# V-Sense/LFBM5D

Measured on AMD Instinct MI355X. Metric: SAI-megapixels/sec (HT+Wiener, sigma=25), higher is better.
Workload: dtype f32; 1 GPU; lf17x17x512x512_sigma25; light_field=17x17x512x512x3, asw=1, color_space=opp, noise=MT19937 seed 1 (utilities.cpp:176-183), window_lanes=2, spatial_bands=1, parallelism=single GPU

## Files before the change

lfbm5d_amd/core.py:

```python
import ctypes as C
import os
import subprocess

from typing import NamedTuple, Optional

import numpy as np

_HERE = os.path.dirname(os.path.abspath(__file__))

YUV, YCBCR, OPP, RGB, ID, DCT, SADCT, BIOR, HADAMARD, HAAR = range(10)
ROWMAJOR, COLMAJOR = 11, 12
TAU = {"id": ID, "dct": DCT, "sadct": SADCT, "bior": BIOR, "hw": HADAMARD, "haar": HAAR}
COLOR_SPACE = {"yuv": YUV, "ycbcr": YCBCR, "opp": OPP, "rgb": RGB}
UNIQUE_ID_BYTES = 128
SR_BICUBIC, SR_GAUSSIAN = 0, 1
SR_UP, SR_DOWN = 0, 1
SR_KERNEL = {"bicubic": SR_BICUBIC, "gaussian": SR_GAUSSIAN}


class LfBm5dError(RuntimeError):
    pass


class Params(C.Structure):
# ... 503 lines not shown


def noise_level_statistic(cov):
    cov = np.ascontiguousarray(cov, np.float64)
    d = cov.shape[0]
    sig, m, lam = C.c_double(), C.c_uint(), np.zeros(d, np.float64)
    dp = C.POINTER(C.c_double)
    if lib().lfbm5d_noise_level_statistic(d, cov.ctypes.data_as(dp), C.byref(sig), C.byref(m), lam.ctypes.data_as(dp)) != 0:
        raise LfBm5dError("lfbm5d_noise_level_statistic: bad arguments (d must be 1..64)")
    return sig.value, m.value, lam


def _quality_result(res, mse, ssim, m, peak):
    pk = 255.0 if peak == 0 else float(peak)
    on = m != 0
    psnr, rmse = np.zeros(m.size, np.float64), np.zeros(m.size, np.float64)
    with np.errstate(divide="ignore"):
        psnr[on] = 10.0 * np.log10(pk * pk / mse[on])
    rmse[on] = np.sqrt(mse[on])
    has = bool(res.has_ssim)
    return Quality(res.psnr_mean, res.psnr_std, res.rmse_mean, res.rmse_std, res.ssim_mean if has else None, res.ssim_std if has else None,
                   res.mse, int(res.count), psnr, rmse, ssim if has else None)


def quality_summary(mse_sai, ssim_sai, mask, peak=255.0):
    m = _u32(mask)
    mse = np.ascontiguousarray(mse_sai, np.float64).copy()
    ssim = None if ssim_sai is None else np.ascontiguousarray(ssim_sai, np.float64).copy()
    if mse.size != m.size or (ssim is not None and ssim.size != m.size):
        raise LfBm5dError("lfbm5d_quality_summary: mse, ssim and mask must hold one entry per SAI")
    dp = C.POINTER(C.c_double)
    res = QualityStruct()
    if lib().lfbm5d_quality_summary(mse.ctypes.data_as(dp), ssim.ctypes.data_as(dp) if ssim is not None else None,
                                    m.ctypes.data_as(C.POINTER(C.c_uint)), m.size, float(peak), C.byref(res)) != 0:
        raise LfBm5dError("lfbm5d_quality_summary: bad arguments (no non-empty SAI, or peak negative or not finite)")
    mse[m == 0] = 0.0
    if ssim is not None:
        ssim[m == 0] = 0.0
    return _quality_result(res, mse, ssim, m, peak)


def pg_fit(hist, sum_m):
    h = np.ascontiguousarray(hist, np.uint64)
    sm = np.ascontiguousarray(sum_m, np.uint64)
    if h.shape != (PG_LEVELS, PG_KEYS) or sm.shape != (PG_LEVELS,):
        raise LfBm5dError("lfbm5d_pg_fit: hist must be [64][322] and sum_m [64]")
    a, b = C.c_double(), C.c_double()
    ullp = C.POINTER(C.c_ulonglong)
    if lib().lfbm5d_pg_fit(h.ctypes.data_as(ullp), sm.ctypes.data_as(ullp), C.byref(a), C.byref(b)) != 0:
        raise LfBm5dError("lfbm5d_pg_fit: no valid level (every level holds fewer than 256 blocks, or its quantile fell into an end bin)")
    return a.value, b.value


def _clip_result(res, chnls):
    return ClipNoiseLevel(res.sigma, tuple(res.sigma_channel[:chnls]), int(res.levels), res.f_max, res.censored, bool(res.heavily_clipped),
                          bool(res.quantised), int(res.blocks), int(res.skipped))


def clip_fit(hist, sum_m, cens, whole, lo=0.0, hi=255.0):
    h = np.ascontiguousarray(hist, np.uint64)
    cz = np.ascontiguousarray(cens, np.uint64)
    wh = np.ascontiguousarray(whole, np.uint64).reshape(-1)
    sm = None if sum_m is None else np.ascontiguousarray(sum_m, np.uint64)
    if h.ndim != 3 or h.shape[0] not in (1, 3) or h.shape[1:] != (PG_LEVELS, PG_KEYS) or cz.shape != h.shape[:2] or wh.shape != h.shape[:1] \
            or (sm is not None and sm.shape != h.shape[:2]):
        raise LfBm5dError("lfbm5d_clip_fit: hist must be [C][64][322], sum_m and cens [C][64], whole [C], C = 1 or 3")
    ullp = C.POINTER(C.c_ulonglong)
    res = ClipEstimateStruct()
    if lib().lfbm5d_clip_fit(h.ctypes.data_as(ullp), sm.ctypes.data_as(ullp) if sm is not None else None, cz.ctypes.data_as(ullp),
                             wh.ctypes.data_as(ullp), h.shape[0], float(lo), float(hi), C.byref(res)) != 0:
        raise LfBm5dError("lfbm5d_clip_fit: fewer than 4 levels are populated (256 blocks, a quantile outside the end bins), or the range "
                          "is bad (lo < hi, both finite)")
    return _clip_result(res, h.shape[0])


def pg_model(a, b, chnls=3):
    a = [float(a)] * chnls if np.isscalar(a) else [float(v) for v in a]
    b = [float(b)] * chnls if np.isscalar(b) else [float(v) for v in b]
    if len(a) != chnls or len(b) != chnls or chnls not in (1, 3):
        raise LfBm5dError("a Poisson-Gaussian model holds one (a, b) per stored channel, 1 or 3 of them")
    m = PgModelStruct()
    for i in range(3):
        j = i if chnls == 3 else 0
        m.a[i], m.b[i] = a[j], b[j]
    return m


def _as_pg_model(model, chnls):
    if model is None or isinstance(model, PgModelStruct):
        return model
    if isinstance(model, PgEstimate):
        return pg_model(model.a, model.b, chnls)
    return pg_model(model[0], model[1], chnls)


def pg_scale(model, chnls=3):
    s = C.c_double()
    try:
        m = _as_pg_model(model, chnls)
    except (TypeError, ValueError) as e:
        raise LfBm5dError(f"lfbm5d_pg_scale: {e}")
    if m is None or lib().lfbm5d_pg_scale(C.byref(m), int(chnls), C.byref(s)) != 0:
        raise LfBm5dError("lfbm5d_pg_scale: bad model (every channel needs a >= 0 and 3/8 a^2 + b > 0, finite; chnls 1 or 3)")
    return s.value


def impulse_scale(hist):
    h = np.ascontiguousarray(hist, dtype=np.uint64)
    if h.shape != (IMPULSE_KEYS,):
        raise LfBm5dError("lfbm5d_impulse_scale: hist must be [386]")
    s = C.c_double()
    if lib().lfbm5d_impulse_scale(h.ctypes.data_as(C.POINTER(C.c_ulonglong)), C.byref(s)) != 0:
        raise LfBm5dError("lfbm5d_impulse_scale: the histogram is empty")
    return s.value


def impulse_params(k=8.0, min_threshold=0.0, threshold=None):
    P = ImpulseParamsStruct()
    lib().lfbm5d_impulse_defaults(C.byref(P))
    P.k, P.min_threshold = float(k), float(min_threshold)
    if threshold is not None:
        t = np.atleast_1d(np.asarray(threshold, np.float64))
        if t.size not in (1, 3):
            raise LfBm5dError("impulse repair: threshold must be a scalar or hold one value per channel")
        for c in range(3):
            P.threshold[c] = float(t[c if t.size == 3 else 0])
    return P


def inpaint_params(iterations=None, sigma_start=None, sigma_end=None, sigma_noise=None):
    P = InpaintParamsStruct()
    lib().lfbm5d_inpaint_defaults(C.byref(P))
    if iterations is not None:
        P.iterations = int(iterations)
    if sigma_start is not None:
        P.sigma_start = float(sigma_start)
    if sigma_end is not None:
        P.sigma_end = float(sigma_end)
    if sigma_noise is not None:
        P.sigma_noise = float(sigma_noise)
    return P


def view_params(max_disparity=None, box_radius=None, ang_radius=None, iterations=None, sigma_start=None, sigma_end=None,
                sigma_noise=None):
    P = ViewParamsStruct()
    lib().lfbm5d_view_defaults(C.byref(P))
    for name, v in (("max_disparity", max_disparity), ("box_radius", box_radius), ("ang_radius", ang_radius), ("iterations", iterations)):
        if v is not None:
            setattr(P, name, int(v))
    for name, v in (("sigma_start", sigma_start), ("sigma_end", sigma_end), ("sigma_noise", sigma_noise)):
        if v is not None:
            setattr(P, name, float(v))
    return P


def consist_params(max_disparity=None, box_radius=None, ang_radius=None, min_sources=None, max_rounds=None, k=None, min_threshold=None,
                   spread=None, sai_factor=None, min_scale=None):
    P = ConsistParamsStruct()
    lib().lfbm5d_consist_defaults(C.byref(P))
    for name, v in (("max_disparity", max_disparity), ("box_radius", box_radius), ("ang_radius", ang_radius), ("min_sources", min_sources),
                    ("max_rounds", max_rounds)):
        if v is not None:
            setattr(P, name, int(v))
    for name, v in (("k", k), ("min_threshold", min_threshold), ("spread", spread), ("sai_factor", sai_factor), ("min_scale", min_scale)):
        if v is not None:
            setattr(P, name, float(v))
    return P


def photo_params(max_disparity=None, box_radius=None, ang_radius=None, steps=None, min_sources=None, max_rounds=None, per_channel=None,
                 anchor=None, min_count=None, tol=None, lo=None, hi=None):
    P = PhotoParamsStruct()
    lib().lfbm5d_photo_defaults(C.byref(P))
    for name, v in (("max_disparity", max_disparity), ("box_radius", box_radius), ("ang_radius", ang_radius), ("steps", steps),
                    ("min_sources", min_sources), ("max_rounds", max_rounds), ("per_channel", per_channel), ("anchor", anchor),
                    ("min_count", min_count)):
        if v is not None:
            setattr(P, name, int(v))
    for name, v in (("tol", tol), ("lo", lo), ("hi", hi)):
        if v is not None:
            setattr(P, name, float(v))
    return P


def photo_edges():
    e = np.zeros(PHOTO_EDGES, np.float32)
    lib().lfbm5d_photo_edges(e.ctypes.data_as(C.POINTER(C.c_float)))
    return e


def photo_ratio(hist, min_count=1):
    h = np.ascontiguousarray(np.asarray(hist, np.uint64).reshape(-1))
    if h.size != PHOTO_KEYS:
        raise LfBm5dError("lfbm5d_photo_ratio: hist must be [1026]")
    r = C.c_double(0.0)
    rc = lib().lfbm5d_photo_ratio(h.ctypes.data_as(C.POINTER(C.c_ulonglong)), int(min_count), C.byref(r))
    return r.value, rc == 0


def photo_solve(r, neighbours, fitted, anchor=None):
    r = np.ascontiguousarray(np.asarray(r, np.float64).reshape(-1))
    A = r.size
    fit = _u32(np.asarray(fitted).reshape(-1) != 0)
    n_src, src = np.zeros(A, np.uint32), np.zeros((A, PHOTO_MAX_SOURCES), np.uint32)
    for m in range(A):
        if not fit[m]:
            continue
        q = [int(v) for v in neighbours[m]]
        if not 1 <= len(q) <= PHOTO_MAX_SOURCES:
            raise LfBm5dError("lfbm5d_photo_solve: a fitted SAI needs 1..24 sources")
        n_src[m] = len(q)
        src[m, :len(q)] = q
    g = np.zeros(A, np.float64)
    up, dp = C.POINTER(C.c_uint), C.POINTER(C.c_double)
    if lib().lfbm5d_photo_solve(A, r.ctypes.data_as(dp), n_src.ctypes.data_as(up), src.ctypes.data_as(up), fit.ctypes.data_as(up),
                                PHOTO_NO_ANCHOR if anchor is None else int(anchor), g.ctypes.data_as(dp)) != 0:
        raise LfBm5dError("lfbm5d_photo_solve: fitted needs [asize] entries, every source and the anchor an index below asize")
    return g


def sr_defaults(scale, /, **changes):
    sr = SrParams()
    if lib().lfbm5d_sr_defaults(int(scale), C.byref(sr)) != 0:
        raise LfBm5dError("lfbm5d_sr_defaults: scale must be 2, 3 or 4")
    for k, v in changes.items():
        if k == "kernel" and isinstance(v, str):
            v = SR_KERNEL[v]
        if k not in dict(SrParams._fields_):
            raise LfBm5dError(f"SrParams has no field {k}")
        setattr(sr, k, v)
    return sr


def sr_taps(op, sr, n_in):
    op = {"up": SR_UP, "down": SR_DOWN}.get(op, op)
    T = C.c_uint(0)
    if lib().lfbm5d_sr_taps(int(op), C.byref(sr), int(n_in), None, None, C.byref(T), 0) != 0:
        raise LfBm5dError("lfbm5d_sr_taps: rejected parameters (scale, kernel, blur_sigma, n_in)")
    n_out = int(n_in) * sr.scale if op == SR_UP else int(n_in) // sr.scale
    first, w = np.zeros(n_out, np.int32), np.zeros((n_out, T.value), np.float32)
    if lib().lfbm5d_sr_taps(int(op), C.byref(sr), int(n_in), first.ctypes.data, w.ctypes.data, C.byref(T), w.size) != 0:
        raise LfBm5dError("lfbm5d_sr_taps failed")
    return first, w


def shard_rows(n_rows, rank, world):
    b, e = C.c_uint(), C.c_uint()
    lib().lfbm5d_shard_rows(n_rows, rank, world, C.byref(b), C.byref(e))
    return b.value, e.value


def make_params(sigma, lam, N, nSim, nDisp, k, p, tau_2D, tau_4D, tau_5D, useSD=0, color_space=OPP):
    t = lambda v: TAU[v] if isinstance(v, str) else int(v)
    cs = COLOR_SPACE[color_space] if isinstance(color_space, str) else int(color_space)
    return Params(float(sigma), float(lam), int(N), int(nSim), int(nDisp), int(k), int(p),
                  int(bool(useSD)), t(tau_2D), t(tau_4D), t(tau_5D), cs)


def make_bm3d_params(sigma, lam, N, nHW, k, p, tau_2D, useSD=0, color_space=OPP):
    cs = COLOR_SPACE[color_space] if isinstance(color_space, str) else int(color_space)
    return Bm3dParams(float(sigma), float(lam), int(N), int(nHW), int(k), int(p), int(bool(useSD)),
                      TAU[tau_2D] if isinstance(tau_2D, str) else int(tau_2D), cs)


def _u32(a):
    return np.ascontiguousarray(np.asarray(a, dtype=np.uint32))


_PLANES = {np.float32: ("device entry points need contiguous float32 CUDA tensors",
                        "per-SAI host buffers must be contiguous float32 numpy arrays"),
           np.uint8: ("flag planes on the device must be contiguous uint8 CUDA tensors",
                      "per-SAI host flag planes must be contiguous uint8 numpy arrays"),
           np.int8: ("disparity planes on the device must be contiguous int8 CUDA tensors",
                     "per-SAI host disparity planes must be contiguous int8 numpy arrays")}


def _dev_ptr(t, dtype=np.float32):
    import torch
    dtype = np.dtype(dtype).type
    if not (isinstance(t, torch.Tensor) and t.is_cuda and t.dtype == getattr(torch, np.dtype(dtype).name) and t.is_contiguous()):
        raise LfBm5dError(_PLANES[dtype][0])
    torch.cuda.current_stream(t.device).synchronize()
    return C.c_void_p(t.data_ptr())


def _sai_ptrs(arrays, mask, dtype=np.float32):
    dtype = np.dtype(dtype).type
    out = (C.c_void_p * len(arrays))()
    for i, a in enumerate(arrays):
        if a is None or not mask[i]:
            continue
        if not (isinstance(a, np.ndarray) and a.dtype == dtype and a.flags.c_contiguous):
            raise LfBm5dError(_PLANES[dtype][1])
        out[i] = a.ctypes.data
    return out


OPTION_ENV = ("LFBM5D_LANES", "LFBM5D_EMULATE_WORLD", "LFBM5D_MAX_WINDOWS", "LFBM5D_FUSED", "LFBM5D_STEP_SHARDING",
              "LFBM5D_DATA_DRIVEN_SCHEDULE", "LFBM5D_HOST_BLOCKING", "LFBM5D_BAND_MB", "LFBM5D_BM3D_LANES", "LFBM5D_SCAN_LDS_CAP",
              "LFBM5D_FORCE_REDO", "LFBM5D_SPATIAL_BANDS", "LFBM5D_BAND_HALO", "LFBM5D_SCAN_V1", "LFBM5D_SCAN_ANY", "LFBM5D_SCAN_FULL_TABLES", "LFBM5D_DCT8W_V2",
              "LFBM5D_GROUP_GENERIC", "LFBM5D_NO_SA_KERNELS", "LFBM5D_NO_SLAB_KERNEL", "LFBM5D_WIDE_NOSPLIT", "LFBM5D_AGG_64BIT",
              "LFBM5D_AGG_SCALAR_SCAN", "LFBM5D_SUBSET_LIST_HOST", "LFBM5D_SUBSET_SCAN_V1", "LFBM5D_FILT_GROUP_MAJOR",
              "LFBM5D_HT_REF_ORDER", "LFBM5D_WINDOW_SUMS_PADDED", "LFBM5D_SELECT_PREFILL")
OPTION_ENV_EMPTY_OFF = ("LFBM5D_WINDOW_SUMS_PADDED",)


class Context:

    def __init__(self, device=0):
        self._L = lib()
        h = C.c_void_p()
        if self._L.lfbm5d_create(C.byref(h), int(device)) != 0:
            raise LfBm5dError(self._L.lfbm5d_last_error(None).decode())
        self._handle = h
        self._env_seen = {k: os.environ.get(k) for k in OPTION_ENV}
        self.device = int(device)

    @property
    def _h(self):
        h = self._handle
        if h and hasattr(self._L, "lfbm5d_set_option"):
            for k in OPTION_ENV:
                v = os.environ.get(k)
                if v != self._env_seen[k]:
                    self._env_seen[k] = v
                    if not v and k in OPTION_ENV_EMPTY_OFF:
                        v = None
                    self._L.lfbm5d_set_option(h, k.encode(), None if v is None else (v or "1").encode())
        return h

    def set_option(self, key, value):
        if self._L.lfbm5d_set_option(self._handle, key.encode(), None if value is None else str(value).encode()) != 0:
            raise LfBm5dError(self._L.lfbm5d_last_error(self._handle).decode())

    def get_option(self, key):
        buf = C.create_string_buffer(64)
        if self._L.lfbm5d_get_option(self._handle, key.encode(), buf, 64) != 0:
            raise LfBm5dError(self._L.lfbm5d_last_error(self._handle).decode())
        return buf.value.decode()

    def close(self):
        if getattr(self, "_handle", None):
            self._L.lfbm5d_destroy(self._handle)
            self._handle = None

    def __del__(self):
        try:
            self.close()
        except Exception:
            pass

    def _ck(self, rc):
        if rc != 0:
            raise LfBm5dError(self._L.lfbm5d_last_error(self._h).decode())

    @staticmethod
    def unique_id():
        buf = (C.c_ubyte * UNIQUE_ID_BYTES)()
        if lib().lfbm5d_comm_unique_id(buf) != 0:
            raise LfBm5dError("ncclGetUniqueId failed")
        return bytes(buf)

    def comm_init(self, unique_id, rank, world):
        buf = (C.c_ubyte * UNIQUE_ID_BYTES).from_buffer_copy(unique_id)
        self._ck(self._L.lfbm5d_comm_init(self._h, buf, rank, world))

    def comm_init_ipc(self, rank, world, rendezvous_dir, timeout_s=30.0):
        self._ck(self._L.lfbm5d_comm_init_ipc(self._h, rank, world, os.fsencode(rendezvous_dir), float(timeout_s)))

    def comm_selftest(self, n=1 << 20):
        self._ck(self._L.lfbm5d_comm_selftest(self._h, n))

    def comm_ranks(self):
        return int(self._L.lfbm5d_comm_ranks(self._h))

    def set_shard(self, rank, world):
        self._ck(self._L.lfbm5d_set_shard(self._h, rank, world))

    def set_tiles(self, nb_tiles):
        self._ck(self._L.lfbm5d_set_tiles(self._h, int(nb_tiles)))

    def reset_stats(self):
        self._L.lfbm5d_reset_stats(self._h)

    def stats(self):
        s = Stats()
        self._L.lfbm5d_get_stats(self._h, C.byref(s))
        return s

    def stream(self):
        return self._L.lfbm5d_stream(self._h)

    def step1(self, P, noisy, mask, basic, ang_major, awidth, aheight, an, W, H, Cc):
        m = _u32(mask)
        mp = m.ctypes.data_as(C.POINTER(C.c_uint))
        tail = (ang_major, awidth, aheight, an, W, H, Cc)
        if isinstance(noisy, (list, tuple)):
            self._ck(self._L.lfbm5d_step1_host_sai(self._h, C.byref(P), _sai_ptrs(noisy, m), mp, _sai_ptrs(basic, m), *tail))
        elif isinstance(noisy, np.ndarray):
            self._ck(self._L.lfbm5d_step1_host(self._h, C.byref(P), noisy.ctypes.data_as(C.c_void_p), mp,
                                               basic.ctypes.data_as(C.c_void_p), *tail))
        else:
            self._ck(self._L.lfbm5d_step1_device(self._h, C.byref(P), _dev_ptr(noisy), mp, _dev_ptr(basic), *tail))

    def step2(self, P, noisy, mask, basic, denoised, ang_major, awidth, aheight, an, W, H, Cc):
        m = _u32(mask)
        mp = m.ctypes.data_as(C.POINTER(C.c_uint))
        tail = (ang_major, awidth, aheight, an, W, H, Cc)
        if isinstance(noisy, (list, tuple)):
            self._ck(self._L.lfbm5d_step2_host_sai(self._h, C.byref(P), _sai_ptrs(noisy, m), mp, _sai_ptrs(basic, m), _sai_ptrs(denoised, m), *tail))
        elif isinstance(noisy, np.ndarray):
            self._ck(self._L.lfbm5d_step2_host(self._h, C.byref(P), noisy.ctypes.data_as(C.c_void_p), mp,
                                               basic.ctypes.data_as(C.c_void_p),
                                               denoised.ctypes.data_as(C.c_void_p), *tail))
        else:
            self._ck(self._L.lfbm5d_step2_device(self._h, C.byref(P), _dev_ptr(noisy), mp, _dev_ptr(basic),
                                                 _dev_ptr(denoised), *tail))

    def denoise(self, P1, P2, noisy, mask, basic, denoised, ang_major, awidth, aheight, an1, an2, W, H, Cc):
        m = _u32(mask)
        mp = m.ctypes.data_as(C.POINTER(C.c_uint))
        tail = (ang_major, awidth, aheight, an1, an2, W, H, Cc)
        if isinstance(noisy, (list, tuple)):
            self._ck(self._L.lfbm5d_denoise_host_sai(self._h, C.byref(P1), C.byref(P2), _sai_ptrs(noisy, m), mp, _sai_ptrs(basic, m),
                                                     _sai_ptrs(denoised, m), *tail))
        elif isinstance(noisy, np.ndarray):
            self._ck(self._L.lfbm5d_denoise_host(self._h, C.byref(P1), C.byref(P2), noisy.ctypes.data_as(C.c_void_p), mp,
                                                 basic.ctypes.data_as(C.c_void_p), denoised.ctypes.data_as(C.c_void_p), *tail))
        else:
            self._ck(self._L.lfbm5d_denoise_device(self._h, C.byref(P1), C.byref(P2), _dev_ptr(noisy), mp, _dev_ptr(basic),
                                                   _dev_ptr(denoised), *tail))

    def core_pass(self, step, P, aw, ah, Wb, Hb, Cc, noisy, basic, num, den, mask, procSAI, cst, pst):
        m, pr = _u32(mask), _u32(procSAI)
        self._ck(self._L.lfbm5d_pass_device(
            self._h, step, C.byref(P), aw, ah, Wb, Hb, Cc, _dev_ptr(noisy),
            _dev_ptr(basic) if basic is not None else None, _dev_ptr(num), _dev_ptr(den),
            m.ctypes.data_as(C.POINTER(C.c_uint)), pr.ctypes.data_as(C.POINTER(C.c_uint)), cst, pst))

    def bm3d_step(self, step, P, Wb, Hb, Cc, noisy, basic, out):
        self._ck(self._L.lfbm5d_bm3d_step_device(self._h, step, C.byref(P), Wb, Hb, Cc, _dev_ptr(noisy),
                                                 _dev_ptr(basic) if basic is not None else None, _dev_ptr(out)))

    def bm3d_lf(self, hard, wien, noisy, mask, basic, denoised, W, H, Cc):
        m = _u32(mask)
        mp = m.ctypes.data_as(C.POINTER(C.c_uint))
        if isinstance(noisy, np.ndarray):
            self._ck(self._L.lfbm5d_bm3d_lf_host(self._h, C.byref(hard), C.byref(wien), noisy.ctypes.data_as(C.c_void_p), mp,
                                                 basic.ctypes.data_as(C.c_void_p), denoised.ctypes.data_as(C.c_void_p),
                                                 m.size, W, H, Cc))
        else:
            self._ck(self._L.lfbm5d_bm3d_lf_device(self._h, C.byref(hard), C.byref(wien), _dev_ptr(noisy), mp, _dev_ptr(basic),
                                                   _dev_ptr(denoised), m.size, W, H, Cc))

    def noise_level(self, LF, LF_SAI_mask, width, height, chnls, patch=8, per_sai=False):
        m = _u32(LF_SAI_mask)
        asize, C_ = m.size, int(chnls)
        res = NoiseLevelStruct()
        d = int(patch) * int(patch) if 4 <= int(patch) <= 8 else 64
        eig = np.zeros(d, np.float64)
        sai = np.zeros(max(asize, 1), np.float64) if per_sai else None
        dp = C.POINTER(C.c_double)
        tail = (m.ctypes.data_as(C.POINTER(C.c_uint)), asize, int(width), int(height), C_, int(patch), C.byref(res),
                sai.ctypes.data_as(dp) if per_sai else None, eig.ctypes.data_as(dp))
        if isinstance(LF, (list, tuple)) or isinstance(LF, np.ndarray):
            arrays = list(LF) if isinstance(LF, (list, tuple)) else [np.ascontiguousarray(a) for a in LF]
            if isinstance(LF, np.ndarray) and LF.dtype != np.float32:
                raise LfBm5dError("host light fields must be float32")
            self._ck(self._L.lfbm5d_noise_level_host_sai(self._h, _sai_ptrs(arrays, m), *tail))
        else:
            self._ck(self._L.lfbm5d_noise_level_device(self._h, _dev_ptr(LF), *tail))
        return NoiseLevel(res.sigma, tuple(res.sigma_channel[:C_]), int(res.components), int(res.patches), eig[:int(res.patch) ** 2],
                          sai[:asize] if per_sai else None)

    def quality(self, ref, test, mask, width, height, chnls, peak=255.0, ssim=True):
        m = _u32(mask)
        asize = m.size
        res = QualityStruct()
        mse, ss = np.zeros(max(asize, 1), np.float64), np.zeros(max(asize, 1), np.float64)
        dp = C.POINTER(C.c_double)
        tail = (m.ctypes.data_as(C.POINTER(C.c_uint)), asize, int(width), int(height), int(chnls), float(peak), 1 if ssim else 0,
                C.byref(res), mse.ctypes.data_as(dp), ss.ctypes.data_as(dp))
        host = [isinstance(x, (list, tuple, np.ndarray)) for x in (ref, test)]
        if host[0] != host[1]:
            raise LfBm5dError("quality: ref and test must both be device tensors or both be host arrays")
        if host[0]:
            arrays = []
            for x in (ref, test):
                if isinstance(x, np.ndarray) and x.dtype != np.float32:
                    raise LfBm5dError("host light fields must be float32")
                arrays.append(list(x) if isinstance(x, (list, tuple)) else [np.ascontiguousarray(a) for a in x])
            self._ck(self._L.lfbm5d_quality_host_sai(self._h, _sai_ptrs(arrays[0], m), _sai_ptrs(arrays[1], m), *tail))
        else:
            self._ck(self._L.lfbm5d_quality_device(self._h, _dev_ptr(ref), _dev_ptr(test), *tail))
        return _quality_result(res, mse[:asize], ss[:asize], m, peak)

    @staticmethod
    def _host_sais(LF):
        if isinstance(LF, np.ndarray) and LF.dtype != np.float32:
            raise LfBm5dError("host light fields must be float32")
        return list(LF) if isinstance(LF, (list, tuple)) else [np.ascontiguousarray(a) for a in LF]

    def _host_out(self, arrays, out, m=None, img=0):
        if out is None:
            out = [(np.zeros(img, np.float32) if img and m[i] else None) if a is None else np.array(a, np.float32, copy=True)
                   for i, a in enumerate(arrays)]
        return out, self._host_sais(out)

    @staticmethod
    def _host_planes(arrays, given, wanted, dtype, n=None):
        if given is not None:
            return list(given)
        if not wanted:
            return None
        return [np.zeros(n, dtype) if n is not None else None if a is None else np.zeros(np.shape(a), dtype) for a in arrays]

    @staticmethod
    def _stacked(noisy, x, like_input=True):
        if not isinstance(noisy, np.ndarray) or x is None or isinstance(x, np.ndarray):
            return x
        return np.stack(x).reshape(noisy.shape) if like_input else np.stack(x)

    @staticmethod
    def _dev_out(noisy, out, m=None):
        import torch
        if out is not None:
            return out
        return torch.empty_like(noisy) if m is not None and m.all() else noisy.clone()

    @staticmethod
    def _dev_planes(noisy, given, wanted, shape, dtype):
        import torch
        if given is None and wanted:
            return torch.zeros(shape, dtype=dtype, device=noisy.device)
        return given

    def pg_histogram(self, LF, LF_SAI_mask, width, height, chnls):
        m = _u32(LF_SAI_mask)
        C_ = int(chnls)
        hist, sm = np.zeros((max(C_, 1), PG_LEVELS, PG_KEYS), np.uint64), np.zeros((max(C_, 1), PG_LEVELS), np.uint64)
        blocks, skipped = C.c_ulonglong(), C.c_ulonglong()
        ullp = C.POINTER(C.c_ulonglong)
        self._ck(self._L.lfbm5d_pg_histogram_device(self._h, _dev_ptr(LF), m.ctypes.data_as(C.POINTER(C.c_uint)), m.size, int(width),
                                                    int(height), C_, hist.ctypes.data_as(ullp), sm.ctypes.data_as(ullp),
                                                    C.byref(blocks), C.byref(skipped)))
        return hist, sm, blocks.value, skipped.value

    def pg_estimate(self, LF, LF_SAI_mask, width, height, chnls):
        m = _u32(LF_SAI_mask)
        C_ = int(chnls)
        res = PgEstimateStruct()
        hist, sm = np.zeros((max(C_, 1), PG_LEVELS, PG_KEYS), np.uint64), np.zeros((max(C_, 1), PG_LEVELS), np.uint64)
        ullp = C.POINTER(C.c_ulonglong)
        tail = (m.ctypes.data_as(C.POINTER(C.c_uint)), m.size, int(width), int(height), C_, C.byref(res), hist.ctypes.data_as(ullp),
                sm.ctypes.data_as(ullp))
        if isinstance(LF, (list, tuple, np.ndarray)):
            self._ck(self._L.lfbm5d_pg_estimate_host_sai(self._h, _sai_ptrs(self._host_sais(LF), m), *tail))
        else:
            self._ck(self._L.lfbm5d_pg_estimate_device(self._h, _dev_ptr(LF), *tail))
        return PgEstimate(res.a, res.b, tuple(res.a_channel[:C_]), tuple(res.b_channel[:C_]), int(res.blocks), int(res.skipped), hist, sm)

    def pg_forward(self, model, LF, mask, out, width, height, chnls):
        mdl = _as_pg_model(model, int(chnls))
        m = _u32(mask)
        self._ck(self._L.lfbm5d_pg_forward_device(self._h, C.byref(mdl), _dev_ptr(LF), m.ctypes.data_as(C.POINTER(C.c_uint)), _dev_ptr(out),
                                                  m.size, int(width), int(height), int(chnls)))
        return pg_scale(mdl, chnls)

    def pg_inverse(self, model, LF, mask, out, width, height, chnls):
        mdl = _as_pg_model(model, int(chnls))
        m = _u32(mask)
        self._ck(self._L.lfbm5d_pg_inverse_device(self._h, C.byref(mdl), _dev_ptr(LF), m.ctypes.data_as(C.POINTER(C.c_uint)), _dev_ptr(out),
                                                  m.size, int(width), int(height), int(chnls)))

    def denoise_pg(self, model, P1, P2, noisy, mask, basic, denoised, ang_major, awidth, aheight, an1, an2, W, H, Cc):
        mdl = _as_pg_model(model, int(Cc))
        used = PgModelStruct()
        m = _u32(mask)
        mp = m.ctypes.data_as(C.POINTER(C.c_uint))
        head = (self._h, C.byref(mdl) if mdl is not None else None, C.byref(used), C.byref(P1), C.byref(P2))
        tail = (ang_major, awidth, aheight, an1, an2, int(W), int(H), int(Cc))
        if isinstance(noisy, (list, tuple, np.ndarray)):
            n, b, d = (self._host_sais(x) for x in (noisy, basic, denoised))
            self._ck(self._L.lfbm5d_denoise_pg_host_sai(*head, _sai_ptrs(n, m), mp, _sai_ptrs(b, m), _sai_ptrs(d, m), *tail))
        else:
            self._ck(self._L.lfbm5d_denoise_pg_device(*head, _dev_ptr(noisy), mp, _dev_ptr(basic), _dev_ptr(denoised), *tail))
        return used

    def clip_histogram(self, LF, LF_SAI_mask, width, height, chnls, lo=0.0, hi=255.0):
        m = _u32(LF_SAI_mask)
        C_ = int(chnls)
        n = max(C_, 1)
        hist, sm, cens = np.zeros((n, PG_LEVELS, PG_KEYS), np.uint64), np.zeros((n, PG_LEVELS), np.uint64), np.zeros((n, PG_LEVELS), np.uint64)
        whole = np.zeros(n, np.uint64)
        blocks, skipped = C.c_ulonglong(), C.c_ulonglong()
        ullp = C.POINTER(C.c_ulonglong)
        self._ck(self._L.lfbm5d_clip_histogram_device(self._h, _dev_ptr(LF), m.ctypes.data_as(C.POINTER(C.c_uint)), m.size, int(width),
                                                      int(height), C_, float(lo), float(hi), hist.ctypes.data_as(ullp),
                                                      sm.ctypes.data_as(ullp), cens.ctypes.data_as(ullp), whole.ctypes.data_as(ullp),
                                                      C.byref(blocks), C.byref(skipped)))
        return hist, sm, cens, whole, blocks.value, skipped.value

    clip_fit = staticmethod(clip_fit)

    def noise_level_clipped(self, LF, LF_SAI_mask, width, height, chnls, lo=0.0, hi=255.0):
        m = _u32(LF_SAI_mask)
        C_ = int(chnls)
# ... 642 lines not shown
```

lfbm5d_amd/csrc/lfbm5d_bm.hip:

```cpp
#include "lfbm5d_kernels.h"

#include <type_traits>
#include <algorithm>
#include <cstdlib>

#pragma clang fp contract(off)

namespace lfbm5d {

namespace {

__device__ __forceinline__ float sq_diff(const float* __restrict__ i1, const float* __restrict__ i2,
                                         int q, int dk) {
    const float d = i2[q + dk] - i1[q];
    return d * d;
}

struct DiffImg {
    const float* i1; const float* i2; int dk; int W, H, b;
    __device__ __forceinline__ float operator()(int y, int x) const {
        if (x < b || x >= W - b || y < b || y >= H - b) return 0.0f;
        return sq_diff(i1, i2, y * W + x, dk);
    }
};
// ... 254 lines not shown
        float F1[FIFO ? K : 1], F2[FIFO ? K : 1];
        if (FIFO) {
#pragma unroll
            for (int m = 0; m < K; m++) {
                const int row = max(m - lane, 0);
                F1[m] = ring[row * CW + lane + K]; F2[m] = ring[row * CW + lane];
            }
        }
        float curS = S0;
        float left_prev = row0_left;
        const int nsteps = (nrows - 1) + last_lane;
        const int lane_eff = col_ok ? lane : 0x40000000;
        const __amdgpu_buffer_rsrc_t rsTb = __builtin_amdgcn_make_buffer_rsrc((void*)table, 0, (int)(tstride * 4), kRsrcFlags);
        int oA = ((K - lane + 64 * RR) % RR) * CW + lane, oB = ((64 * RR - lane) % RR) * CW + lane;
        int wrow = filled % RR;
        int nextF = 0x7fffffff, nextB = 0x7fffffff, offF = -1, offB = -1, incF = 0, incB = 0;
        auto chunk = [&](auto edge_tag, int t0, const int jj,
                         v4f* la1, v4f* la2, float& lb1, float& lb2,
                         const v4f* sa1, const v4f* sa2, float sb1, float sb2) {
            constexpr int FL = decltype(edge_tag)::value;
            constexpr bool FAST = FL == 4;
            constexpr bool TAIL = FL == 3;
            constexpr bool EDGE = FL == 1 || FL == 2;
            constexpr bool REDGE = FL == 2;
            if (!TAIL) load_chunk(std::integral_constant<bool, REDGE>{}, filled + (DEP - 1) * T, la1, la2, lb1, lb2);
            const float* pa = ring + oA;
            const float* pb = ring + oB;
            float d1[T], d2[T], d3[T], d4[T], lc[T], Sout[T];
#pragma unroll
            for (int s = 0; s < T; s++) {
                d1[s] = pa[s * CW + K]; d2[s] = pa[s * CW];
                if (FIFO) {
                    const int slot = (jj * T + s) % K;
                    d3[s] = F1[slot]; d4[s] = F2[slot];
                    F1[slot] = d1[s]; F2[slot] = d2[s];
                } else { d3[s] = pb[s * CW + K]; d4[s] = pb[s * CW]; }
                lc[s] = lcol[(REDGE || TAIL) ? min(1 + t0 + s, nrows + T) : 1 + t0 + s];
            }
            oA += T * CW; oA = oA >= RR * CW ? oA - RR * CW : oA;
            if (!FIFO) { oB += T * CW; oB = oB >= RR * CW ? oB - RR * CW : oB; }
#pragma unroll
            for (int s = 0; s < T; s++) {
                if (EDGE) curS = (lane_eff == t0 + s) ? S0 : curS;
                const float left = __int_as_float(__builtin_amdgcn_update_dpp(__float_as_int(lc[s]), __float_as_int(curS),
                                                                              0x138 , 0xf, 0xf, false));
                float S = left + curS;
                S = S - left_prev;
                S = S + d1[s];
                S = S - d2[s];
                S = S - d3[s];
                S = S + d4[s];
                S = first_col ? left : S;
                Sout[s] = S;
                curS = S;
                left_prev = left;
            }
#pragma unroll
            for (int s = 0; s < T; s++) {
                const int t = t0 + s;
                const bool act = EDGE ? (unsigned)(t - lane_eff) <= (unsigned)(nrows - 2) : col_ok;
                if (stereo) {
                    const bool on = (EDGE || TAIL) ? (unsigned)(t - lane_eff) <= (unsigned)(nrows - 2) : col_ok;
                    __builtin_amdgcn_raw_buffer_store_b32(__builtin_bit_cast(int, Sout[s]), rsTb, on ? lane * 4 : -1, (strip * SR + t + 1) * 256, 0);
                } else if (FAST) {
                    if (t == nextF) { __builtin_amdgcn_raw_buffer_store_b32(__builtin_bit_cast(int, Sout[s]), rsS, offF, 0, 0); offF += incF; nextF += gP; }
                    if (t == nextB) { __builtin_amdgcn_raw_buffer_store_b32(__builtin_bit_cast(int, Sout[s]), rsS, offB, 0, 0); offB += incB; nextB += gP; }
                } else {
                    int v1, v2;
                    if (irregular) {
                        const int q = (b + 1 + t - lane) * W + x;
                        const int r1 = __builtin_amdgcn_raw_buffer_load_b32(rsM, q * 4, 0, 0);
                        const int r2 = (di > 0 && x + djs >= 0 && x + djs < W) ? __builtin_amdgcn_raw_buffer_load_b32(rsM, (q + di * W + djs) * 4, 0, 0) : -1;
                        v1 = (act && r1 >= 0) ? (int)(((unsigned)r1 * (unsigned)ncand + (unsigned)ord_fwd) * 4u) : -1;
                        v2 = (act && r2 >= 0) ? (int)(((unsigned)r2 * (unsigned)ncand + (unsigned)ord_bwd) * 4u) : -1;
                    } else {
                        const slot_t* rp = rs16 + min(max(b + 1 + t0 - lane, 0), H - T);
                        const int r1 = rp[s], r2 = rp[s + di];
                        const bool ok1 = (r1 | base_fwd) >= 0, ok2 = (r2 | base_bwd) >= 0;
                        v1 = (ok1 && (!EDGE || act)) ? r1 * row_bytes + base_fwd : -1;
                        v2 = (ok2 && (!EDGE || act)) ? r2 * row_bytes + base_bwd : -1;
                    }
                    if (__builtin_amdgcn_ballot_w64(v1 != -1)) __builtin_amdgcn_raw_buffer_store_b32(__builtin_bit_cast(int, Sout[s]), rsS, v1, 0, 0);
                    if (__builtin_amdgcn_ballot_w64(v2 != -1)) __builtin_amdgcn_raw_buffer_store_b32(__builtin_bit_cast(int, Sout[s]), rsS, v2, 0, 0);
                }
                const int il = 1 + t - last_lane;
                const float hv = __int_as_float(__builtin_amdgcn_readlane(__float_as_int(Sout[s]), last_lane));
                lcol[(REDGE || TAIL) ? ((il >= 1 && il < nrows) ? il : nrows + T) : FL == 1 ? max(il, 0) : il] = hv;
            }
            if (!TAIL) {
                write_chunk(std::integral_constant<bool, REDGE>{}, filled, wrow, sa1, sa2, sb1, sb2);
                wrow = wrow + T == RR ? 0 : wrow + T;
                filled += T;
            }
        };
        {
            const int band_rows = H - 2 * b;
            constexpr int G = DEP * T;
            int tS0 = ((last_lane + 1 + G - 1) / G) * G;
            int tS1 = min(nrows - 1, band_rows - K - DEP * T);
            tS1 = tS1 > tS0 ? tS0 + ((tS1 - tS0) / G) * G : tS0;
            const bool light_up = tS0 + K + (DEP + 1) * T <= band_rows && tS0 + T < nrows;
            int t0 = 0;
            auto group = [&](auto tag, int tg) {
#pragma unroll
                for (int j = 0; j < DEP; j++)
                    chunk(tag, tg + j * T, j, A1[(j + DEP - 1) % DEP], A2[(j + DEP - 1) % DEP], Bq1[(j + DEP - 1) % DEP], Bq2[(j + DEP - 1) % DEP],
                          A1[j], A2[j], Bq1[j], Bq2[j]);
            };
            SCAN_MARK(2);
            if (light_up) for (; t0 < min(tS0, nsteps); t0 += G) group(std::integral_constant<int, 1>{}, t0);
            else          for (; t0 < min(tS0, nsteps); t0 += G) group(std::integral_constant<int, 2>{}, t0);
            SCAN_MARK(3);
            if (MODE == 0) {
                const bool offpat = (base_fwd >= 0 && (x - gN) % gP != 0) || (base_bwd >= 0 && (x + djs - gN) % gP != 0);
                const unsigned long long mF = __builtin_amdgcn_ballot_w64(base_fwd >= 0), mB = __builtin_amdgcn_ballot_w64(base_bwd >= 0);
                int tF1 = (gR - 1) * gP - 1 - G - di;
                tF1 = tF1 >= t0 ? t0 + ((tF1 - t0) / G + 1) * G : t0;
                tF1 = min(tF1, tS1);
                if (!__builtin_amdgcn_ballot_w64(offpat) && t0 < tF1) {
                    nextF = nextB = 0x7fffffff; offF = offB = -1; incF = incB = 0;
                    if (mF) {
                        const int l1 = (int)__builtin_ctzll(mF);
                        nextF = t0 + (((l1 - 1 - t0) % gP) + gP) % gP;
                        if (base_fwd >= 0) { offF = ((1 + nextF - lane) / gP) * row_bytes + base_fwd; incF = row_bytes; }
                    }
                    if (mB) {
                        const int l2 = (int)__builtin_ctzll(mB);
                        nextB = t0 + (((l2 - 1 - di - t0) % gP) + gP) % gP;
                        if (base_bwd >= 0) { offB = ((1 + nextB - lane + di) / gP) * row_bytes + base_bwd; incB = row_bytes; }
                    }
                    for (; t0 < tF1; t0 += G) group(std::integral_constant<int, 4>{}, t0);
                }
            }
            for (; t0 < tS1; t0 += G) group(std::integral_constant<int, 0>{}, t0);
            SCAN_MARK(4);
            const int t_end = nsteps;
            if (stereo) {
                for (; t0 < t_end && (filled < band_rows || t0 <= last_lane); t0 += G) group(std::integral_constant<int, 2>{}, t0);
                for (; t0 < t_end; t0 += G) group(std::integral_constant<int, 3>{}, t0);
            } else
                for (; t0 < t_end; t0 += G) group(std::integral_constant<int, 2>{}, t0);
        }
        SCAN_MARK(3);
        row0_left = __int_as_float(__builtin_amdgcn_readlane(__float_as_int(S0), last_lane));
        __syncthreads();
    }
#ifdef LFBM5D_PHASE_TIMING
    if (lane == 0 && a.dbg) {
        const int base = stereo ? 0 : 6;
        for (int i = 0; i < 5; i++) atomicAdd(&a.dbg[base + i], (unsigned long long)tk[i]);
        atomicAdd(&a.dbg[base + 5], 1ull);
    }
#endif
}

template <int K, bool WIDE>
__global__ __launch_bounds__(64) __attribute__((amdgpu_waves_per_eu(2, 2))) void k_bm_scan(ScanArgs a) {
    extern __shared__ float lds[];
    if (blockIdx.x >= a.n_self) scan_body<K, 2, WIDE>(a, (int)(blockIdx.x - a.n_self), lds);
    else if (a.refmap) scan_body<K, 1, WIDE>(a, (int)blockIdx.x, lds);
    else scan_body<K, 0, WIDE>(a, (int)blockIdx.x, lds);
}

template <int MODE>
__device__ __forceinline__ void scan_any_body(const ScanArgs& a, const int bid, float* lds) {
    constexpr bool stereo = MODE == 2;
    constexpr bool irregular = MODE == 1;
    const int lane = threadIdx.x;
    const int K = (int)a.k;
    const int half = stereo ? (int)a.nDisp : (int)a.nSim;
    const int trim = stereo ? K - 1 : 0;
    const int W = a.W, H = a.H, b = stereo ? (int)a.nDisp : (int)a.nHW;
    const int Ns = 2 * half + 1, ncand = Ns * Ns;
    const int nrows = H - 2 * b - trim, ncols = W - 2 * b - trim;
    int di, dj;
    DiffImg D;
    const size_t WH = (size_t)W * H;
    if (stereo) {
        const int slot = bid / ncand, ddk = bid % ncand;
        di = ddk / Ns; dj = ddk % Ns;
        D.i1 = a.est + (size_t)a.pst * WH;
        D.i2 = a.est + (size_t)a.st_of_slot[slot] * WH;
        D.dk = di * W + dj - half * (1 + W);
    } else {
        di = bid / Ns; dj = bid % Ns;
        D.i1 = D.i2 = a.est + (size_t)a.pst * WH;
        D.dk = di * W + dj - half;
    }
    D.W = W; D.H = H; D.b = b;
    const size_t tstride = stereo ? stereo_table_stride(a.W, a.H, a.k, a.nDisp) : 0;
    float* table = stereo ? a.tables + (size_t)bid * tstride : nullptr;
    const int SR = nrows + 63;
    const int djs = dj - half;
    const int ord_fwd = dj * Ns + di;
    const int ord_bwd = (-djs + half) * Ns + (half + 1) + (half - di);
    const int gR = a.n_ref_rows, gC = a.n_ref_cols, gP = a.p, gN = a.nHW;
    const int lastR = H - K - gN, lastC = W - K - gN;
    auto emit = [&](int y, int x, float S) {
        if (stereo) { table[((size_t)((x - b) / 64) * SR + (y - b) + (x - b) % 64) * 64 + (x - b) % 64] = S; return; }
        if (irregular) {
            const int r = a.refmap[y * W + x];
            if (r >= 0) a.scores[(size_t)r * ncand + ord_fwd] = S;
            const int yy = y + di, xx = x + djs;
            if (di > 0 && yy < H && xx >= 0 && xx < W) {
                const int r2 = a.refmap[yy * W + xx];
                if (r2 >= 0) a.scores[(size_t)r2 * ncand + ord_bwd] = S;
            }
            return;
        }
        const int cx = grid_index(x, gC, lastC, gN, gP);
        if (cx >= 0) {
            const int ry = grid_index(y, gR, lastR, gN, gP);
            if (ry >= 0) a.scores[(size_t)(ry * gC + cx) * ncand + ord_fwd] = S;
        }
        if (di > 0) {
            const int cx2 = grid_index(x + djs, gC, lastC, gN, gP);
            if (cx2 >= 0) {
                const int ry2 = grid_index(y + di, gR, lastR, gN, gP);
                if (ry2 >= 0) a.scores[(size_t)(ry2 * gC + cx2) * ncand + ord_bwd] = S;
            }
        }
    };
    float* Lprev = lds;
    float* Lnext = lds + nrows;
    float* tbuf = lds + 2 * nrows;

    for (int e = lane; e < K * K; e += 64) tbuf[e] = D(b + e / K, b + e % K);
    __syncthreads();
    float corner = 0.0f;
    for (int e = 0; e < K * K; e++) corner += tbuf[e];
    __syncthreads();
    if (lane == 0) { Lnext[0] = corner; emit(b, b, corner); }
    {
        float carry = corner;
        for (int i0 = 1; i0 < nrows; i0 += 64) {
            const int i = i0 + lane;
            for (int q = 0; q < K; q++) tbuf[lane * K + q] = i < nrows ? D(b + i - 1 + K, b + q) - D(b + i - 1, b + q) : 0.0f;
            __syncthreads();
            const int m = min(64, nrows - i0);
            float mine = 0.0f;
            for (int l = 0; l < m; l++) {
                float cand = carry;
                for (int q = 0; q < K; q++) cand += tbuf[l * K + q];
                carry = cand;
                if (lane == l) mine = carry;
            }
            if (i < nrows) { Lnext[i] = mine; emit(b + i, b, mine); }
            __syncthreads();
        }
    }
    const int nstrips = (ncols - 1 + 63) / 64;
    for (int strip = 0; strip < nstrips; strip++) {
        { float* t = Lprev; Lprev = Lnext; Lnext = t; }
        __syncthreads();
        const int cb = b + 1 + 64 * strip;
        const int x = cb + lane;
        const bool col_ok = x < b + ncols;
        const int last_lane = min(63, ncols - 2 - 64 * strip);
        for (int p = 0; p < K; p++) tbuf[lane * K + p] = col_ok ? D(b + p, x - 1 + K) - D(b + p, x - 1) : 0.0f;
        __syncthreads();
        float S0 = 0.0f;
        {
            float carry = Lprev[0];
            for (int l = 0; l <= last_lane; l++) {
                float cand = carry;
                for (int p = 0; p < K; p++) cand += tbuf[l * K + p];
                carry = cand;
                if (lane == l) S0 = carry;
            }
        }
        if (col_ok) emit(b, x, S0);
        if (lane == last_lane) Lnext[0] = S0;
        float cur = S0, leftprev = Lprev[0];
        const int nsteps = (nrows - 1) + last_lane;
        for (int t = 0; t < nsteps; t++) {
            const int r = 1 + t - lane;
            float nb = __int_as_float(__builtin_amdgcn_update_dpp(0, __float_as_int(cur), 0x138 , 0xf, 0xf, false));
            if (lane == 0) nb = Lprev[min(max(r, 0), nrows - 1)];
            if (col_ok && r >= 1 && r <= nrows - 1) {
                const int y = b + r;
                float S = nb + cur;
                S = S - leftprev;
                S = S + D(y + K - 1, x + K - 1);
                S = S - D(y + K - 1, x - 1);
                S = S - D(y - 1, x + K - 1);
                S = S + D(y - 1, x - 1);
                emit(y, x, S);
                cur = S;
                if (lane == last_lane) Lnext[r] = S;
            }
            leftprev = nb;
        }
        __syncthreads();
    }
}

__global__ __launch_bounds__(64) void k_bm_scan_any(ScanArgs a) {
    extern __shared__ float lds[];
    if (blockIdx.x >= a.n_self) scan_any_body<2>(a, (int)(blockIdx.x - a.n_self), lds);
    else if (a.refmap) scan_any_body<1>(a, (int)blockIdx.x, lds);
    else scan_any_body<0>(a, (int)blockIdx.x, lds);
}

__device__ __forceinline__ unsigned f2ord(float f) {
    const unsigned u = __float_as_uint(f);
    return (u & 0x80000000u) ? ~u : (u | 0x80000000u);
}

__device__ __forceinline__ unsigned long long wave_min(unsigned long long v) {
    auto step = [&](auto ctrl, auto rmask, auto bmask, unsigned long long src) {
        constexpr int C = decltype(ctrl)::value, R = decltype(rmask)::value, B = decltype(bmask)::value;
        const unsigned lo = (unsigned)__builtin_amdgcn_update_dpp((int)(unsigned)v, (int)(unsigned)src, C, R, B, false);
        const unsigned hi = (unsigned)__builtin_amdgcn_update_dpp((int)(unsigned)(v >> 32), (int)(unsigned)(src >> 32), C, R, B, false);
        const unsigned long long oth = ((unsigned long long)hi << 32) | lo;
        v = oth < v ? oth : v;
    };
    using std::integral_constant;
    const unsigned long long v0 = v;
    step(integral_constant<int, 0x111>{}, integral_constant<int, 0xf>{}, integral_constant<int, 0xf>{}, v0);
    step(integral_constant<int, 0x112>{}, integral_constant<int, 0xf>{}, integral_constant<int, 0xf>{}, v0);
    step(integral_constant<int, 0x113>{}, integral_constant<int, 0xf>{}, integral_constant<int, 0xf>{}, v0);
    step(integral_constant<int, 0x114>{}, integral_constant<int, 0xf>{}, integral_constant<int, 0xe>{}, v);
    step(integral_constant<int, 0x118>{}, integral_constant<int, 0xf>{}, integral_constant<int, 0xc>{}, v);
    step(integral_constant<int, 0x142>{}, integral_constant<int, 0xa>{}, integral_constant<int, 0xf>{}, v);
    step(integral_constant<int, 0x143>{}, integral_constant<int, 0xc>{}, integral_constant<int, 0xf>{}, v);
    const unsigned lo = (unsigned)__builtin_amdgcn_readlane((int)(unsigned)v, 63), hi = (unsigned)__builtin_amdgcn_readlane((int)(unsigned)(v >> 32), 63);
    return ((unsigned long long)hi << 32) | lo;
}

__global__ __launch_bounds__(64) void k_self_select(const float* __restrict__ scores,
                                                     const unsigned* __restrict__ refs, unsigned n_refs,
                                                     int W, int nSim, int N, float thr,
                                                     unsigned* __restrict__ self_idx,
                                                     unsigned* __restrict__ self_cnt,
                                                     int grid_cols, int nHW, int p, int last_r, int last_c) {
    extern __shared__ unsigned long long keys[];
    const int lane = threadIdx.x;
    const unsigned ref = blockIdx.x;
    if (ref >= n_refs) return;
    const int Ns = 2 * nSim + 1, ncand = Ns * Ns;
    const unsigned div_m = ((1u << 20) + (unsigned)Ns - 1) / (unsigned)Ns;
    const int k_r = (int)refs[ref];
    size_t row = ref;
    if (grid_cols) {
        const int y = k_r / W, x = k_r - y * W;
        const int gi = y == last_r ? (last_r - nHW + p - 1) / p : (y - nHW) / p;
        const int gj = x == last_c ? (last_c - nHW + p - 1) / p : (x - nHW) / p;
        row = (size_t)gi * grid_cols + gj;
    }
    const float* sc = scores + row * ncand;
    int cnt = 0;
    unsigned long long mine = ~0ull;
    constexpr int kB = 8;
    for (int e0 = 0; e0 < ncand; e0 += 64 * kB) {
        float score[kB], test[kB];
#pragma unroll
        for (int u = 0; u < kB; u++) {
            const int e = e0 + u * 64 + lane;
            score[u] = 0.0f; test[u] = 0.0f;
            if (e < ncand) {
                const int q = (int)(((unsigned)e * div_m) >> 20);
                const int djp = q - nSim, r = e - q * Ns;
                const bool fwd = r <= nSim;
                const int dip = fwd ? r : r - 2 * nSim - 1;
                score[u] = sc[e];
                test[u] = fwd ? score[u] : sc[(-djp + nSim) * Ns + (-dip)];
            }
        }
#pragma unroll
        for (int u = 0; u < kB; u++) {
            const int e = e0 + u * 64 + lane;
            const bool pass = e < ncand && test[u] < thr;
            const unsigned long long bal = __ballot(pass);
            if (pass) {
                const unsigned long long kk = ((unsigned long long)f2ord(score[u]) << 32) | (unsigned)e;
                keys[cnt + __popcll(bal & ((1ull << lane) - 1ull))] = kk;
                mine = kk < mine ? kk : mine;
            }
            cnt += __popcll(bal);
        }
    }
    __syncthreads();
    unsigned nSx;
    if (N > cnt) { nSx = 1; while (nSx * 2 <= (unsigned)cnt) nSx *= 2; } else nSx = N;
    unsigned* out = self_idx + (size_t)ref * N;
    if (cnt == 0) {
        if (lane == 0) { out[0] = k_r; out[1] = k_r; self_cnt[ref] = 2; }
        return;
    }
    auto wave_rank = [&](unsigned long long v) {
        unsigned r = 0;
#pragma unroll
        for (int j = 0; j < 64; j++) {
            const unsigned long long o = ((unsigned long long)(unsigned)__builtin_amdgcn_readlane((int)(unsigned)(v >> 32), j) << 32)
                                       | (unsigned)__builtin_amdgcn_readlane((int)(unsigned)v, j);
            r += (o < v || (o == v && j < lane)) ? 1u : 0u;
        }
        return r;
    };
    if (cnt > 128) {
        const unsigned rk = wave_rank(mine);
        const unsigned long long hb = __ballot(rk == nSx - 1);
        const int src = __ffsll((long long)hb) - 1;
        const unsigned long long bound = ((unsigned long long)(unsigned)__builtin_amdgcn_readlane((int)(unsigned)(mine >> 32), src) << 32)
                                       | (unsigned)__builtin_amdgcn_readlane((int)(unsigned)mine, src);
        int c2 = 0;
        for (int e0 = 0; e0 < cnt; e0 += 64) {
            const int e = e0 + lane;
            const unsigned long long kk = e < cnt ? keys[e] : ~0ull;
            const bool keep = kk <= bound;
            const unsigned long long bal = __ballot(keep);
            if (keep) keys[c2 + __popcll(bal & ((1ull << lane) - 1ull))] = kk;
            c2 += __popcll(bal);
        }
        cnt = c2;
        __builtin_amdgcn_wave_barrier();
    }
    if (cnt <= 64) {
        const unsigned long long kk = lane < cnt ? keys[lane] : ~0ull;
        const unsigned rk = wave_rank(kk);
        if (lane < cnt && rk < nSx) {
            const int e = (int)(kk & 0xffffffffu);
            const int djp = e / Ns - nSim, r = e % Ns;
            const int dip = (r <= nSim) ? r : r - 2 * nSim - 1;
            out[rk] = (unsigned)(k_r + dip * W + djp);
            if (nSx == 1) out[1] = out[0];
        }
        if (lane == 0) self_cnt[ref] = nSx == 1 ? 2 : nSx;
        return;
    }
    unsigned long long last = 0;
    bool first = true;
    for (unsigned n = 0; n < nSx; n++) {
        unsigned long long best = ~0ull;
        for (int e = lane; e < cnt; e += 64) {
            const unsigned long long kk = keys[e];
            if ((first || kk > last) && kk < best) best = kk;
        }
        best = wave_min(best);
        last = best; first = false;
        if (lane == 0) {
            const int e = (int)(best & 0xffffffffu);
            const int djp = e / Ns - nSim, r = e % Ns;
            const int dip = (r <= nSim) ? r : r - 2 * nSim - 1;
            out[n] = (unsigned)(k_r + dip * W + djp);
            if (nSx == 1) out[1] = out[0];
        }
    }
    if (lane == 0) self_cnt[ref] = nSx == 1 ? 2 : nSx;
}

__device__ __forceinline__ bool scan2_writes_backward(int y, int x, int dip, int djp, int W, int nHW) {
    return y + dip >= nHW && (unsigned)(x + djp - nHW) < (unsigned)(W - 2 * nHW);
}

constexpr int kSelWaves = 4;
constexpr int kSelMaxRows = 32;

struct SelectArgs {
    const float* scores; const unsigned* refs; unsigned n_refs;
    int W, nSim, N; float thr;
    unsigned* self_idx; unsigned* self_cnt;
    int grid_cols, nHW, p, last_r, last_c;
    int unfilled;
    float fill;
};

template <int ROWS, int SURE>
__global__ __launch_bounds__(kSelWaves * 64) void k_self_select_regs(SelectArgs a) {
    static_assert(ROWS <= kSelMaxRows && ROWS * 64 <= 2048, "scan indices are 11 bits in the radix select");
    __shared__ float stage[kSelWaves][ROWS * 64];
    __shared__ __attribute__((aligned(16))) unsigned long long skeys[kSelWaves][64];
    const int lane = threadIdx.x & 63, wv = __builtin_amdgcn_readfirstlane(threadIdx.x >> 6);
    const unsigned ref = blockIdx.x * kSelWaves + wv;
    if (ref >= a.n_refs) return;
    const int W = a.W, nSim = a.nSim, N = a.N, nHW = a.nHW;
    const int Ns = 2 * nSim + 1, ncand = Ns * Ns;
    const float thr = a.thr;
    const unsigned div_m = ((1u << 18) + (unsigned)Ns - 1) / (unsigned)Ns;
    const int k_r = __builtin_amdgcn_readfirstlane((int)a.refs[ref]);
    const int y = k_r / W, x = k_r - y * W;
    size_t row = ref;
    if (a.grid_cols) {
        const int gi = y == a.last_r ? (a.last_r - nHW + a.p - 1) / a.p : (y - nHW) / a.p;
        const int gj = x == a.last_c ? (a.last_c - nHW + a.p - 1) / a.p : (x - nHW) / a.p;
        row = (size_t)gi * a.grid_cols + gj;
    }
    const float* sc = a.scores + row * ncand;
    float v[ROWS];
#pragma unroll
    for (int u = 0; u < ROWS; u++) {
        const int e = u * 64 + lane;
        v[u] = (u < SURE || e < ncand) ? sc[e] : 0.0f;
    }
    float* st = stage[wv];
#pragma unroll
    for (int u = 0; u < ROWS; u++) {
        const int e = u * 64 + lane;
        if (u < SURE || e < ncand) st[e] = v[u];
    }
    __builtin_amdgcn_fence(__ATOMIC_RELEASE, "wavefront");
    __builtin_amdgcn_wave_barrier();
    __builtin_amdgcn_fence(__ATOMIC_ACQUIRE, "wavefront");
    unsigned hk[ROWS];
    int cnt = 0;
    unsigned mhi = 0xffffffffu, mlo = 0xffffffffu;
    auto scan_rows = [&](auto edge_tag) {
        constexpr bool EDGE = decltype(edge_tag)::value;
#pragma unroll
        for (int u = 0; u < ROWS; u++) {
            const int e = u * 64 + lane;
            const bool in = u < SURE || e < ncand;
            const int q = (int)(__umul24((unsigned)e, div_m) >> 18);
            const int r = e - (int)__umul24((unsigned)q, (unsigned)Ns);
            const bool fwd = r <= nSim;
            const float t = st[max(ncand - e, 0)];
            float score = v[u];
            if (EDGE) score = (fwd || scan2_writes_backward(y, x, r - Ns, q - nSim, W, nHW)) ? score : a.fill;
            const bool pass = in && (fwd ? v[u] : t) < thr;
            hk[u] = pass ? f2ord(score) : 0xffffffffu;
            cnt += __popcll(__ballot(hk[u] != 0xffffffffu));
            if (hk[u] < mhi) { mhi = hk[u]; mlo = (unsigned)e; }
        }
    };
    if (a.unfilled && !(y - nSim >= nHW && x - nSim >= nHW && x + nSim < W - nHW)) scan_rows(std::true_type{});
    else scan_rows(std::false_type{});
    unsigned nSx;
    if (N > cnt) { nSx = 1; while (nSx * 2 <= (unsigned)cnt) nSx *= 2; } else nSx = N;
    unsigned* out = a.self_idx + (size_t)ref * N;
    if (cnt == 0) {
        if (lane == 0) { out[0] = k_r; out[1] = k_r; a.self_cnt[ref] = 2; }
        return;
    }
    auto place = [&](unsigned long long kk, unsigned n) {
        const int e = (int)(kk & 0xffffffffu);
        const int djp = e / Ns - nSim, r = e % Ns;
        const int dip = (r <= nSim) ? r : r - 2 * nSim - 1;
        out[n] = (unsigned)(k_r + dip * W + djp);
        if (nSx == 1) out[1] = out[0];
    };
    unsigned bhi = 0xffffffffu; int blo = -1;
    if (cnt > 64) {
        unsigned ahi = 0;
        for (int b = 31; b >= 0; b--) {
            const unsigned trial = ahi | (1u << b);
            if ((unsigned)__popcll(__ballot(mhi < trial)) < nSx) ahi = trial;
        }
        if (ahi != 0xffffffffu) {
            const unsigned need = nSx - (unsigned)__popcll(__ballot(mhi < ahi));
            unsigned alo = 0;
            for (int b = 10; b >= 0; b--) {
                const unsigned trial = alo | (1u << b);
                if ((unsigned)__popcll(__ballot(mhi == ahi && mlo < trial)) < need) alo = trial;
            }
            bhi = ahi; blo = (int)alo;
        }
    }
    auto kept = [&](int u) { return hk[u] < bhi || (hk[u] == bhi && u * 64 + lane <= blo); };
    auto key_of = [&](int u) { return ((unsigned long long)hk[u] << 32) | (unsigned)(u * 64 + lane); };
    unsigned long long* keys = skeys[wv];
    int c2 = 0;
#pragma unroll
    for (int u = 0; u < ROWS; u++) {
        const bool keep = kept(u);
        const unsigned long long bal = __ballot(keep);
        if (bal) {
            const int pos = c2 + __popcll(bal & ((1ull << lane) - 1ull));
            if (keep && pos < 64) keys[pos] = key_of(u);
            c2 += __popcll(bal);
        }
    }
    if (c2 <= 64) {
        if (lane >= c2) keys[lane] = ~0ull;
        __builtin_amdgcn_fence(__ATOMIC_RELEASE, "wavefront");
        __builtin_amdgcn_wave_barrier();
        __builtin_amdgcn_fence(__ATOMIC_ACQUIRE, "wavefront");
        const unsigned long long kk = keys[lane];
        unsigned rk = 0;
        for (int j = 0; j < c2; j += 8) {
#pragma unroll
            for (int i = 0; i < 8; i++) rk += keys[j + i] < kk ? 1u : 0u;
        }
        if (lane < c2 && rk < nSx) place(kk, rk);
        if (lane == 0) a.self_cnt[ref] = nSx == 1 ? 2 : nSx;
        return;
    }
    unsigned long long last = 0;
    for (unsigned n = 0; n < nSx; n++) {
        unsigned long long best = ~0ull;
#pragma unroll
        for (int u = 0; u < ROWS; u++) {
            const unsigned long long kk = key_of(u);
            if (kept(u) && (n == 0 || kk > last) && kk < best) best = kk;
        }
        best = wave_min(best);
        last = best;
        if (lane == 0) place(best, n);
    }
    if (lane == 0) a.self_cnt[ref] = nSx == 1 ? 2 : nSx;
}

__global__ __launch_bounds__(256) void k_scores_patch(float* __restrict__ scores, unsigned n_rows, unsigned n_cols, int W, int nSim, int nHW,
                                                       int p, int last_r, int last_c, float fill) {
    const int Ns = 2 * nSim + 1, ncand = Ns * Ns;
    const size_t i = (size_t)blockIdx.x * blockDim.x + threadIdx.x;
    if (i >= (size_t)n_rows * n_cols * ncand) return;
    const unsigned ref = (unsigned)(i / ncand);
    const int e = (int)(i - (size_t)ref * ncand);
    const unsigned gi = ref / n_cols, gj = ref - gi * n_cols;
    const int y = gi == n_rows - 1 ? last_r : nHW + (int)gi * p, x = gj == n_cols - 1 ? last_c : nHW + (int)gj * p;
    const int q = e / Ns, r = e - q * Ns;
// ... 200 lines not shown
```

lfbm5d_amd/csrc/lfbm5d_ctx.h:

```cpp
#ifndef LFBM5D_CTX_H
#define LFBM5D_CTX_H

#include "../../include/lfbm5d.h"
#include "lfbm5d_kernels.h"
#include "lfbm5d_plan.h"
#include "lfbm5d_options.h"

#include <rccl/rccl.h>

#include <algorithm>
#include <chrono>
#include <cmath>
#include <fstream>
#include <thread>
#include <unistd.h>
#include <cstdio>
#include <cstdlib>
#include <cstring>
#include <string>
#include <vector>


namespace lfbm5d_host {

using namespace lfbm5d;



constexpr double kSqrt2 = 1.414213562373095;
constexpr double kSqrt2Inv = 0.7071067811865475;
constexpr double kPi = 3.14159265358979323846;

struct DevBuf {
    void* p = nullptr; size_t cap = 0;
    hipError_t reserve(size_t bytes) {
        if (bytes <= cap) return hipSuccess;
        if (p) { hipError_t e = hipFree(p); p = nullptr; cap = 0; if (e != hipSuccess) return e; }
        hipError_t e = hipMalloc(&p, bytes);
        if (e == hipSuccess) cap = bytes;
        return e;
    }
    void release() { if (p) (void)hipFree(p); p = nullptr; cap = 0; }
    template <class T> T* as() const { return reinterpret_cast<T*>(p); }
};

struct PassEvents { hipEvent_t e[5]; bool comm; };

struct GeomCache {
    DevBuf refs, rslot, tb, scan_wgs;
    std::vector<Scan2Wg> scan_plan; unsigned scan_key[8] = {0, 0, 0, 0, 0, 0, 0, 0}; size_t scan_lds = 0;
    unsigned scan_nwg_slot = 0; int scan_version = 0;
    std::vector<unsigned> last_refs_host;
    unsigned grid_key[5] = {0, 0, 0, 0, 0};
    unsigned rslot_key[5] = {0, 0, 0, 0, 0};
    unsigned tb_key[3] = {0, 0, 0};
    unsigned n_ref_rows = 0, n_ref_cols = 0;
};

}

using lfbm5d_host::DevBuf; using lfbm5d_host::PassEvents; using lfbm5d_host::GeomCache; using lfbm5d::Options;


constexpr int kDefaultLanes = 2;
constexpr size_t kEstLead = 64;

struct HostIO {
    float* const* noisy = nullptr;
    float* const* basic = nullptr;
    float* const* out = nullptr;
};

struct lfbm5d_ctx {
    int device = 0;
    hipStream_t stream = nullptr;
    std::string err;
    int rank = 0, world = 1;
    int tiles = 1;
    ncclComm_t comm = nullptr;
    ncclComm_t comm2 = nullptr;
    hipStream_t cs[2] = {nullptr, nullptr};
    int pass_rank = 0, pass_world = 1;
    bool pass_reduce = false;
    std::vector<unsigned> last_windows;
    lfbm5d_stats stats;
    DevBuf t_noisy, t_basic, t_tnum, t_tden, und_num, und_den;
    DevBuf scan_lcol;
    DevBuf sub_flags, sub_cnt;
    int last_scan_version = 0;
    GeomCache gc[2]; int gslot = 0;
    bool est_ready = false;
    struct DirectSums { bool on = false; float* num = nullptr; float* den = nullptr; size_t lf_stride = 0; lfbm5d::SaiList sai; } direct;
    DevBuf est, refmap, scores, tables, self_idx, self_cnt, best, shape, filt, wgt, aggpos, gpos, gofs, gok, sa_list, gshape, counters, small, t_num, t_den, d_mask;
    DevBuf g_num, g_den, g_num2, g_den2, n2, e_basic, w_noisy, w_basic, w_num, w_den, h2d_noisy, h2d_basic, h2d_out, d_own, gscratch;
    bool ipc = false;
    std::string ipc_dir; double ipc_timeout_s = 30.0; unsigned ipc_epoch = 0;
    std::string ipc_tag;
    DevBuf ipc_flags, ipc_out;
    struct IpcPeer { unsigned char handle[7][64]; void* ptr[7]; };
    std::vector<IpcPeer> ipc_peers;
    DevBuf pristine, pristine_b;
    DevBuf band_noisy, band_basic, band_out, band_src, band_pack, band_gather;
    ncclComm_t team_comm = nullptr, team_comm2 = nullptr; int team_S = 0;
    Options opt_store; Options* opt = &opt_store;
    hipStream_t io_in = nullptr, io_out = nullptr;
    unsigned* h_small = nullptr;
    struct SideBufs { DevBuf sai, lf; std::vector<unsigned> sai_host; } side;
    struct NoiseBufs { DevBuf part, cells, m, pool; } noise;
    struct QualityBufs { DevBuf part, out; } quality;
    struct SrBufs {
        DevBuf tab, lo;
        std::vector<unsigned> host;
        unsigned key[5] = {0, 0, 0, 0, 0}; size_t off[8] = {0, 0, 0, 0, 0, 0, 0, 0}; unsigned T[4] = {0, 0, 0, 0};
    } sr;
    struct PgBufs { DevBuf stats; } pg;
    struct ClipBufs { DevBuf stats; } clip;
    struct ImpulseBufs { DevBuf stats, flags; } imp;
    struct InpaintBufs { DevBuf stats, state[2], flags; } inp;
    struct ViewBufs { DevBuf table, stats, disp, set; } view;
    struct ConsistBufs { DevBuf table, stats, pred, disp, flags; } consist;
    struct PhotoBufs { DevBuf table, sweep_table, stats, pred, disp, x; std::vector<unsigned> planes_host; std::vector<float> factors_host; } photo;
    std::vector<lfbm5d_ctx*> lanes;
    unsigned* h_counts = nullptr; size_t h_counts_cap = 0;
    std::vector<hipEvent_t> ev_pool; size_t ev_used = 0;
    std::vector<PassEvents> pending;
    unsigned last_n_refs = 0, last_N = 0, last_A = 0; size_t last_plane = 0; int last_gslot = 0;
    struct UnfilledScores { bool pending = false; unsigned n_rows = 0, n_cols = 0, W = 0, nSim = 0, nHW = 0, p = 0, last_r = 0, last_c = 0; float fill = 0; } unfilled;
};

namespace lfbm5d_host {


#define HIPCK(ctx, call)                                                                         \
    do {                                                                                         \
        hipError_t e_ = (call);                                                                  \
        if (e_ != hipSuccess) {                                                                  \
            (ctx)->err = std::string(#call) + ": " + hipGetErrorString(e_);                      \
            return 1;                                                                            \
        }                                                                                        \
    } while (0)

inline int fail(lfbm5d_ctx* c, const std::string& m) { c->err = m; return 1; }

lfbm5d_ctx* new_ctx(int device, std::string& err);
hipEvent_t get_event(lfbm5d_ctx* c);
void drain_events(lfbm5d_ctx* c);
int sigma_table(float sigma, unsigned C, unsigned cs, float* out);
void ind_init(std::vector<unsigned>& v, unsigned max_size, unsigned N, unsigned step);
void build_tables(GroupTables& t, unsigned k, unsigned aw, unsigned ah);
bool is_pow2(unsigned n);
int validate(lfbm5d_ctx* c, int step, const lfbm5d_params* P, unsigned aw, unsigned ah, unsigned C, bool bm3d = false);
int fold_counters(lfbm5d_ctx* c, const lfbm5d_params* P, unsigned A, unsigned C, int step, int slot = 0);
inline void add_stats(lfbm5d_stats& dst, const lfbm5d_stats& src) {
    static_assert(sizeof(lfbm5d_stats) == 15 * 8, "lfbm5d_stats has a new field: add it below or name it above");
    dst.passes += src.passes; dst.groups += src.groups; dst.stack_patches += src.stack_patches; dst.sadct_groups += src.sadct_groups;
    dst.algorithmic_bytes += src.algorithmic_bytes;
    dst.ms_bm += src.ms_bm; dst.ms_group += src.ms_group; dst.ms_aggregate += src.ms_aggregate;
    dst.launches_group += src.launches_group; dst.launches_aggregate += src.launches_aggregate;
}
int pass_impl(lfbm5d_ctx* c, int step, const lfbm5d_params* P, unsigned aw, unsigned ah, unsigned Wb,
              unsigned Hb, unsigned C, const float* d_noisy, const float* d_basic, float* d_num,
              float* d_den, const unsigned* h_mask, const unsigned* h_proc, unsigned cst, unsigned pst,
              bool bm3d = false);
int io_upload_all(lfbm5d_ctx* c, const HostIO* io, const unsigned* h_mask, unsigned asize, size_t img, float* d_noisy, float* d_basic_in);
int io_download_all(lfbm5d_ctx* c, const HostIO* io, const unsigned* h_mask, unsigned asize, size_t img, const float* d_noisy,
                    const float* d_basic, const float* d_out);
constexpr unsigned kIpcMaxMsgs = 4096;
int auto_bands(unsigned awidth, unsigned aheight, unsigned height, unsigned halo, int world);
int ipc_allgather(lfbm5d_ctx* c, const char* tag, int mine, std::vector<int>& all);
bool ipc_put(const std::string& dir, const std::string& name, const void* data, size_t bytes);
bool ipc_get(const std::string& dir, const std::string& name, void* data, size_t bytes, double timeout_s);
int run_step(lfbm5d_ctx* c, int step, const lfbm5d_params* P, float* d_noisy, const unsigned* h_mask,
             float* d_basic, float* d_out, unsigned ang_major, unsigned awidth, unsigned aheight,
             unsigned an, unsigned W, unsigned H, unsigned C, const HostIO* io = nullptr);
int run_denoise(lfbm5d_ctx* c, const lfbm5d_params* P1, const lfbm5d_params* P2, float* d_noisy, const unsigned* h_mask, float* d_basic,
                float* d_out, unsigned ang_major, unsigned awidth, unsigned aheight, unsigned an1, unsigned an2, unsigned W, unsigned H,
                unsigned C, const HostIO* io = nullptr);

constexpr int kViewTabStride = 2 + 3 * 24;
int view_sweep_launch(lfbm5d_ctx* c, const int* d_table, unsigned n_sai, const float* d_in, float* d_out, signed char* d_disp, unsigned W,
                      unsigned H, unsigned C, int D, int r, unsigned long long* d_cnt, unsigned steps, unsigned max_sources);

}
#endif
```

lfbm5d_amd/csrc/lfbm5d_kernels.h:

```cpp
#ifndef LFBM5D_KERNELS_H
#define LFBM5D_KERNELS_H

#include <hip/hip_runtime.h>
#include <vector>

#include "lfbm5d_options.h"

constexpr int kFiltStoreAux = 2;
constexpr int kFiltLoadAux = 0;

#if defined(__HIPCC__)
typedef float filt_v4f __attribute__((ext_vector_type(4)));
typedef float filt_v2f __attribute__((ext_vector_type(2)));
__device__ __forceinline__ void filt_put(float* p, const float v) { *p = v; }
__device__ __forceinline__ void filt_put2(filt_v2f* p, const filt_v2f v) { *p = v; }
__device__ __forceinline__ void filt_put4(filt_v4f* p, const filt_v4f v) { *p = v; }
__device__ __forceinline__ void filt_put4(float4* p, const float4 v) { *p = v; }
__device__ __forceinline__ void filt_put4_nt(filt_v4f* p, const filt_v4f v) { __builtin_nontemporal_store(v, p); }
#endif

namespace lfbm5d {

constexpr int kMaxK = 32;
constexpr int kMaxA = 49;
constexpr int kA3 = 9;
constexpr int kMaxAw = 7;
constexpr int kBigAw = 17;
constexpr int kBigA = kBigAw * kBigAw;
constexpr int kMaskWords = (kBigA + 63) / 64;
struct SaiMask {
    unsigned long long w[kMaskWords];
    __host__ __device__ bool test(unsigned i) const { return (w[i >> 6] >> (i & 63)) & 1ull; }
    __host__ __device__ void set(unsigned i) { w[i >> 6] |= 1ull << (i & 63); }
    __host__ __device__ unsigned count() const { unsigned n = 0; for (int i = 0; i < kMaskWords; i++) n += (unsigned)__builtin_popcountll(w[i]); return n; }
    __host__ __device__ bool holds_all(unsigned n) const { for (unsigned i = 0; i < n; i++) if (!test(i)) return false; return true; }
};
inline SaiMask sai_mask_none() { SaiMask m; for (int i = 0; i < kMaskWords; i++) m.w[i] = 0; return m; }
constexpr int kMaxN = 16;
constexpr int kMaxN3 = 32;

struct GroupTables {
    float kaiser[kMaxK * kMaxK];
    float cn2[kMaxK * kMaxK];
    float cni2[kMaxK * kMaxK];
    float cos2[kMaxK * kMaxK];
    float cn4[kBigA];
    float cni4[kBigA];
    float cos3[9];
    float cosw[kBigA];
    float cos1[kBigAw + 1][kBigA];
    float cn1[kBigAw + 1][kBigAw];
    float cni1[kBigAw + 1][kBigAw];
    float c1inv[kBigAw + 1];
    float cos5[5][256];
    float cos5x[1024];
    float cn5_0[6], cn5[6];
    float c5inv[6];
    float lpd[10], hpd[10], lpr[10], hpr[10];
    float coef2inv;
    float coef4inv;
    float ht3_f[9];
    float ht3_gf[9];
};

constexpr float kHtGuardAbs[9][4] = {
    {1.5e-7f, 8.1e-6f, 1.7e-5f, 3.5e-5f}, {5.6e-7f, 1.4e-6f, 1.9e-6f, 3.5e-6f}, {7.8e-7f, 2.3e-6f, 2.8e-6f, 3.7e-6f},
    {2.1e-6f, 3.6e-6f, 5.4e-6f, 6.4e-6f}, {4.1e-7f, 1.1e-6f, 1.6e-6f, 2.4e-6f}, {5.3e-7f, 1.8e-6f, 2.3e-6f, 4.0e-6f},
    {3.8e-6f, 6.6e-6f, 9.4e-6f, 1.4e-5f}, {7.6e-7f, 1.7e-6f, 2.5e-6f, 4.2e-6f}, {1.0e-6f, 3.0e-6f, 3.9e-6f, 6.5e-6f}};

constexpr unsigned kShapeInfoBytes = (5 * kMaxA + 2 * kMaxAw + 1) * 4;
constexpr unsigned kShapeInfoBigBytes = (5 * kBigA + 2 * kBigAw + 1) * 4;

struct GroupArgs {
    const float* noisy;
    const float* basic;
    float* num;
    float* den;
    const unsigned* refs;
    const unsigned* self_idx;
    const unsigned* self_cnt;
    const unsigned* best;
    const unsigned char* shape;
    const GroupTables* tb;
    float* filt;
    float* wgt;
    unsigned* aggpos;
    unsigned* gpos;
    unsigned* sa_list;
    unsigned* gofs;
    unsigned* gok;
    void* gshape;
    unsigned n_refs_total;
    unsigned long long* counters;
    unsigned ref_begin, n_groups;
    unsigned Wb, Hb, C, A, k, N, pst;
    SaiMask mask_bits, proc_bits;
    unsigned tau2, tau4, tau5, useSD;
    unsigned fill_quirk;
    int step;
    float lambda;
    float sigma[3];
    float ht3_T[3][9][4];
    float ht3_K[3][9];
    float* scratch;
    unsigned long long scratch_floats;
    unsigned opt;
    unsigned long long filt_sai_stride;
    unsigned bm3d;
};

constexpr unsigned kSaiMajorMinA = 121;
__device__ __forceinline__ size_t filt_patch(const GroupArgs& a, unsigned g, unsigned n, unsigned st, unsigned k2) {
    return a.filt_sai_stride ? (size_t)st * a.filt_sai_stride + ((size_t)g * a.N + n) * a.C * k2
                             : (((size_t)g * a.N + n) * a.A + st) * a.C * k2;
}


struct SaiList { unsigned st[kBigA]; unsigned n; };

struct AggArgs {
    float* num;
    float* den;
    const float* filt;
    unsigned long long filt_sai_stride;
    unsigned long long filt_bytes;
    const float* wgt;
    const unsigned* aggpos;
    unsigned n_refs_total;
    const unsigned* refs;
    const unsigned* self_idx;
    const unsigned* self_cnt;
    const unsigned* best;
    const unsigned char* shape;
    const GroupTables* tb;
    unsigned ref_begin, n_groups;
    unsigned n_ref_rows, n_ref_cols;
    unsigned Wb, Hb, C, A, k, N, pst, p, nHW, nSim, nDisp;
    SaiMask mask_bits, proc_bits; unsigned tau4;
    unsigned irregular;
    unsigned opt;
    unsigned wchan0;
    unsigned direct;
    unsigned long long lf_stride;
    SaiList sai;
};

__host__ __device__ inline size_t stereo_table_stride(unsigned W, unsigned H, unsigned k, unsigned nDisp) {
    const unsigned ncols = W - 2 * nDisp - (k - 1), nrows = H - 2 * nDisp - (k - 1);
    return (size_t)((ncols + 63) / 64) * 64 * (nrows + 63);
}

__host__ __device__ inline unsigned stereo_table_srq(unsigned H, unsigned k, unsigned nDisp) {
    const unsigned nrows = H - 2 * nDisp - (k - 1);
    return ((nrows - 1 + 63 + 15) / 16) * 4 + 1;
}
__host__ __device__ inline size_t stereo_table_stride2(unsigned W, unsigned H, unsigned k, unsigned nDisp) {
    const unsigned ncols = W - 2 * nDisp - (k - 1);
    return (size_t)((ncols - 1 + 63) / 64) * stereo_table_srq(H, k, nDisp) * 256 + stereo_table_srq(H, k, nDisp) * 4;
}

__host__ __device__ inline unsigned stereo_part_chunks(unsigned H, unsigned k, unsigned nDisp) {
    const unsigned nrows = H - 2 * nDisp - (k - 1);
    return ((nrows - 1 + 63 + 15) / 16) * 2;
}
__host__ __device__ inline size_t stereo_part_stride(unsigned W, unsigned H, unsigned k, unsigned nDisp) {
    const unsigned ncols = W - 2 * nDisp - (k - 1);
    return (size_t)((ncols - 1 + 63) / 64) * stereo_part_chunks(H, k, nDisp) * 512;
}
__host__ __device__ inline size_t stereo_edge_stride(unsigned W, unsigned H, unsigned k, unsigned nDisp) {
    const unsigned ncols = W - 2 * nDisp - (k - 1), nrows = H - 2 * nDisp - (k - 1);
    return ((size_t)nrows + (ncols - 1 + 63) / 64 + 3) & ~(size_t)3;
}

struct Scan2Wg {
    short tab[16];
    short slot;
    short r2lo, c2lo;
    short rh, ch;
    short wgj;
    short pad[2];
    short ord[16];
};

struct ScanArgs {
    const float* est;
    unsigned W, H, k;
    unsigned nSim, nDisp, nHW;
    unsigned pst;
    unsigned n_self;
    unsigned n_stereo;
    unsigned n_ref_rows, n_ref_cols, p;
    const int* rslot;
    const int* refmap;
    float* scores;
    unsigned scores_bytes;
    unsigned long long* dbg;
    unsigned opt;
    unsigned lds_cap;
    float* tables;
    unsigned st_of_slot[kBigA];
    unsigned est_planes;
    const Scan2Wg* wgs;
    unsigned n_wgs;
    float* lcol;
    unsigned lcol_stride;
    unsigned nwg_slot;
};

hipError_t launch_color(hipStream_t s, float* img, unsigned cs, unsigned n_px, int forward);
hipError_t launch_color_lf(hipStream_t s, float* lf, size_t sai_stride, unsigned n_sai, const unsigned* d_mask, unsigned cs,
                           unsigned n_px, int forward);
hipError_t launch_color_roundtrip_lf(hipStream_t s, const float* in, float* out, size_t sai_stride, unsigned n_sai, const unsigned* d_mask,
                                     unsigned cs, unsigned n_px);
hipError_t launch_estimate_lf(hipStream_t s, const float* num, const float* den, const float* sub, float* est, size_t seg,
                              unsigned n_sai, const unsigned* d_mask);
hipError_t launch_symetrize(hipStream_t s, const float* src, float* dst, unsigned W, unsigned H,
                            unsigned C, unsigned N);
hipError_t launch_unsymetrize(hipStream_t s, float* dst, const float* src, unsigned W, unsigned H,
                              unsigned C, unsigned N);
hipError_t launch_crop(hipStream_t s, float* dst, const float* src, unsigned W, unsigned H, unsigned C, unsigned N, unsigned off);
hipError_t launch_estimate(hipStream_t s, const float* num, const float* den, const float* sub,
                           float* est, size_t n);
hipError_t launch_finalize_multi(hipStream_t s, const float* num, const float* den, const float* sub, float* basic, size_t sai_stride,
                                 const SaiList& L, unsigned cs, unsigned n_px, int colour);
hipError_t launch_output_multi(hipStream_t s, const float* num, const float* den, const float* sub, float* out, float* basic,
                               const float* noisy_src, float* noisy_dst, size_t sai_stride, const SaiList& L, unsigned cs, unsigned n_px,
                               int colour);
hipError_t launch_ipc_set(hipStream_t s, unsigned* p, unsigned v);
hipError_t launch_ipc_wait(hipStream_t s, const unsigned* p, unsigned want, unsigned* err, double timeout_s);
hipError_t launch_symetrize_multi(hipStream_t s, const float* src, size_t src_stride, float* dst, size_t dst_stride,
                                  const SaiList& L, unsigned W, unsigned H, unsigned C, unsigned N);
hipError_t launch_unsymetrize_multi(hipStream_t s, float* dst, size_t dst_stride, const float* src, size_t src_stride,
                                    const SaiList& L, unsigned W, unsigned H, unsigned C, unsigned N);
constexpr unsigned kWinCounters = 32;
hipError_t launch_window_begin(hipStream_t s, const float* noisy, const float* basic, const float* num, const float* den, size_t lf_stride,
                               float* w_noisy, float* w_basic, float* w_num, float* w_den, float* est, size_t w_stride, const SaiList& L,
                               unsigned W, unsigned H, unsigned C, unsigned N, unsigned* zero);
hipError_t launch_window_end(hipStream_t s, float* num, float* den, size_t lf_stride, const float* w_num, const float* w_den, size_t w_stride,
                             const SaiList& L, unsigned W, unsigned H, unsigned C, unsigned N, unsigned k, unsigned* count);
hipError_t launch_estimate_multi(hipStream_t s, const float* num, const float* den, const float* sub, float* est,
                                 size_t plane, unsigned C, unsigned A, const SaiMask& mask_bits);
hipError_t launch_copy_rect(hipStream_t s, float* dst, size_t dst_stride, unsigned dW, unsigned dH, unsigned dx0, unsigned dy0,
                            const float* src, size_t src_stride, unsigned sW, unsigned sH, unsigned sx0, unsigned sy0,
                            unsigned w, unsigned h, unsigned C, unsigned n_slots, const SaiMask& mask_bits);
hipError_t launch_copy_rows(hipStream_t s, const float* src, unsigned src_H, unsigned src_row0, float* dst, unsigned dst_H, unsigned dst_row0,
                            unsigned n_rows, unsigned W, unsigned planes);
hipError_t launch_fill_f32(hipStream_t s, float* p, float v, size_t n);
hipError_t launch_fill_i32(hipStream_t s, int* p, int v, size_t n);
hipError_t launch_add(hipStream_t s, float* dst, const float* src, size_t n);
hipError_t launch_count_zeros(hipStream_t s, const float* den, size_t seg, unsigned n_seg,
                              unsigned* counts);
hipError_t launch_count_denoised(hipStream_t s, const float* den, size_t sai_stride, unsigned n_slots, const SaiMask& mask_bits,
                                 unsigned W, unsigned H, unsigned C, unsigned N, unsigned k, unsigned* count);
hipError_t launch_refmap(hipStream_t s, const unsigned* refs, unsigned n_refs, int* refmap);
hipError_t launch_subset_list(hipStream_t s, const float* den0, unsigned Wb, unsigned k, unsigned nHW, unsigned p, unsigned n_rows,
                              unsigned n_cols, unsigned last_r, unsigned last_c, unsigned char* flags, unsigned* refs, unsigned* count);
hipError_t launch_bm_scan(hipStream_t s, const ScanArgs& a);
int bm_scan_version(const ScanArgs& a);
bool scan2_plan(const ScanArgs& a, std::vector<Scan2Wg>& wgs, size_t* lds_bytes, unsigned* nwg_slot = nullptr);
size_t scan_tables_floats(const ScanArgs& a, int version, unsigned n_slots, unsigned nwg_slot);
unsigned scan2_lcol_stride(const ScanArgs& a);
hipError_t prepare_scan2_kernels();
hipError_t launch_bm_scan2(hipStream_t s, const ScanArgs& a, size_t lds_bytes, bool combined);
hipError_t launch_stereo_argmin3(hipStream_t s, const float* tables, const unsigned* st_of_slot, unsigned n_slots, unsigned nwg_slot,
                                 unsigned W, unsigned H, unsigned k, unsigned nDisp, float thr,
                                 unsigned* best, unsigned char* shape);
hipError_t launch_stereo_argmin2(hipStream_t s, const float* tables, const unsigned* st_of_slot, unsigned n_slots,
                                 unsigned W, unsigned H, unsigned k, unsigned nDisp, float thr,
                                 unsigned* best, unsigned char* shape);
hipError_t launch_self_select(hipStream_t s, const float* scores, const unsigned* refs, unsigned n_refs,
                              unsigned W, unsigned nSim, unsigned N, float thr, unsigned* self_idx,
                              unsigned* self_cnt,
                              unsigned grid_cols = 0, unsigned nHW = 0, unsigned p = 1, unsigned last_r = 0, unsigned last_c = 0);
bool self_select_regs_covers(unsigned nSim);
hipError_t launch_self_select_regs(hipStream_t s, const float* scores, const unsigned* refs, unsigned n_refs,
                                   unsigned W, unsigned nSim, unsigned N, float thr, unsigned* self_idx, unsigned* self_cnt,
                                   unsigned grid_cols, unsigned nHW, unsigned p, unsigned last_r, unsigned last_c, bool unfilled);
hipError_t launch_scores_patch(hipStream_t s, float* scores, unsigned n_rows, unsigned n_cols, unsigned W, unsigned nSim, unsigned nHW,
                               unsigned p, unsigned last_r, unsigned last_c, float fill);
hipError_t launch_self_trivial(hipStream_t s, const unsigned* refs, unsigned n_refs, unsigned* self_idx,
                               unsigned* self_cnt);
hipError_t launch_stereo_argmin(hipStream_t s, const float* tables, const unsigned* st_of_slot, unsigned n_slots,
                                unsigned W, unsigned H, unsigned k, unsigned nDisp, float thr,
                                unsigned* best, unsigned char* shape);
hipError_t prepare_group_kernels();
hipError_t launch_group(hipStream_t s, const GroupArgs& a);
size_t group_lds_bytes(const GroupArgs& a);
size_t group_scratch_bytes(const GroupArgs& a);
hipError_t launch_aggregate(hipStream_t s, const AggArgs& a);

}
#endif
```

lfbm5d_amd/csrc/lfbm5d_options.h:

```cpp
#ifndef LFBM5D_OPTIONS_H
#define LFBM5D_OPTIONS_H

#include <cstddef>
#include <cstdlib>
#include <cstring>
#include <string>

namespace lfbm5d {

enum : unsigned {
    kOptScanV1 = 1u << 0,
    kOptScanAny = 1u << 1,
    kOptScanFullTables = 1u << 2,
    kOptDct8wV2 = 1u << 3,
    kOptGroupGeneric = 1u << 4,
    kOptNoSaKernels = 1u << 5,
    kOptNoSlabKernel = 1u << 6,
    kOptWideNoSplit = 1u << 7,
    kOptAgg64Bit = 1u << 8,
    kOptAggScalarScan = 1u << 9,
    kOptSubsetListHost = 1u << 10,
    kOptSubsetScanV1 = 1u << 11,
    kOptFiltGroupMajor = 1u << 12,
    kOptHtReferenceOrder = 1u << 13,
    kOptSelectPrefill = 1u << 14,
};

struct Options {
    int lanes = 2;
    int emulate_world = 0;
    int max_windows = 0;
    int fused = 1;
    int step_sharding = 0;
    int data_driven_schedule = 0;
    int host_blocking = 0;
    int band_mb = 0;
    int bm3d_lanes = 3;
    int scan_lds_cap = 0;
    int force_redo = 0;
    int spatial_bands = 1;
    int band_halo = 0;
    int window_sums_padded = 0;
    unsigned kernels = 0;
};

struct OptionKey { const char* key; const char* env; int Options::* field; unsigned bit; };

inline const OptionKey* option_keys(size_t* n) {
    static const OptionKey keys[] = {
        {"lanes", "LFBM5D_LANES", &Options::lanes, 0}, {"emulate_world", "LFBM5D_EMULATE_WORLD", &Options::emulate_world, 0},
        {"max_windows", "LFBM5D_MAX_WINDOWS", &Options::max_windows, 0}, {"fused", "LFBM5D_FUSED", &Options::fused, 0},
        {"step_sharding", "LFBM5D_STEP_SHARDING", &Options::step_sharding, 0},
        {"data_driven_schedule", "LFBM5D_DATA_DRIVEN_SCHEDULE", &Options::data_driven_schedule, 0},
        {"host_blocking", "LFBM5D_HOST_BLOCKING", &Options::host_blocking, 0}, {"band_mb", "LFBM5D_BAND_MB", &Options::band_mb, 0},
        {"bm3d_lanes", "LFBM5D_BM3D_LANES", &Options::bm3d_lanes, 0}, {"scan_lds_cap", "LFBM5D_SCAN_LDS_CAP", &Options::scan_lds_cap, 0},
        {"force_redo", "LFBM5D_FORCE_REDO", &Options::force_redo, 0}, {"spatial_bands", "LFBM5D_SPATIAL_BANDS", &Options::spatial_bands, 0},
        {"band_halo", "LFBM5D_BAND_HALO", &Options::band_halo, 0},
        {"window_sums_padded", "LFBM5D_WINDOW_SUMS_PADDED", &Options::window_sums_padded, 0},
        {"scan_v1", "LFBM5D_SCAN_V1", nullptr, kOptScanV1}, {"scan_any", "LFBM5D_SCAN_ANY", nullptr, kOptScanAny},
        {"scan_full_tables", "LFBM5D_SCAN_FULL_TABLES", nullptr, kOptScanFullTables}, {"dct8w_v2", "LFBM5D_DCT8W_V2", nullptr, kOptDct8wV2},
        {"group_generic", "LFBM5D_GROUP_GENERIC", nullptr, kOptGroupGeneric}, {"no_sa_kernels", "LFBM5D_NO_SA_KERNELS", nullptr, kOptNoSaKernels},
        {"no_slab_kernel", "LFBM5D_NO_SLAB_KERNEL", nullptr, kOptNoSlabKernel}, {"wide_nosplit", "LFBM5D_WIDE_NOSPLIT", nullptr, kOptWideNoSplit},
        {"agg_64bit", "LFBM5D_AGG_64BIT", nullptr, kOptAgg64Bit}, {"agg_scalar_scan", "LFBM5D_AGG_SCALAR_SCAN", nullptr, kOptAggScalarScan},
        {"subset_list_host", "LFBM5D_SUBSET_LIST_HOST", nullptr, kOptSubsetListHost}, {"subset_scan_v1", "LFBM5D_SUBSET_SCAN_V1", nullptr, kOptSubsetScanV1},
        {"filt_group_major", "LFBM5D_FILT_GROUP_MAJOR", nullptr, kOptFiltGroupMajor},
        {"ht_reference_order", "LFBM5D_HT_REF_ORDER", nullptr, kOptHtReferenceOrder},
        {"select_prefill", "LFBM5D_SELECT_PREFILL", nullptr, kOptSelectPrefill},
    };
    *n = sizeof(keys) / sizeof(keys[0]);
    return keys;
}

inline bool option_set(Options& o, const char* key, const char* value) {
    size_t n; const OptionKey* keys = option_keys(&n);
    static const Options defaults;
    for (size_t i = 0; i < n; i++) {
        if (std::strcmp(key, keys[i].key) != 0 && std::strcmp(key, keys[i].env) != 0) continue;
        const bool unset = value == nullptr || value[0] == 0;
        if (keys[i].field) {
            int v = defaults.*(keys[i].field);
            if (!unset) {
                if (keys[i].field == &Options::step_sharding) v = std::strcmp(value, "rows") == 0 ? 1 : std::strcmp(value, "blocks") == 0 ? 2 : std::atoi(value);
                else if (keys[i].field == &Options::data_driven_schedule || keys[i].field == &Options::host_blocking || keys[i].field == &Options::force_redo)
                    v = std::strcmp(value, "0") != 0;
                else v = std::atoi(value);
            }
            o.*(keys[i].field) = v;
        } else {
            if (!unset && std::strcmp(value, "0") != 0) o.kernels |= keys[i].bit; else o.kernels &= ~keys[i].bit;
        }
        return true;
    }
    return false;
}
inline bool option_get(const Options& o, const char* key, std::string& out) {
    size_t n; const OptionKey* keys = option_keys(&n);
    for (size_t i = 0; i < n; i++) {
        if (std::strcmp(key, keys[i].key) != 0 && std::strcmp(key, keys[i].env) != 0) continue;
        if (keys[i].field == &Options::step_sharding) out = o.step_sharding == 1 ? "rows" : o.step_sharding == 2 ? "blocks" : "0";
        else if (keys[i].field) out = std::to_string(o.*(keys[i].field));
        else out = (o.kernels & keys[i].bit) ? "1" : "0";
        return true;
    }
    return false;
}
inline void options_from_env(Options& o) {
    size_t n; const OptionKey* keys = option_keys(&n);
    for (size_t i = 0; i < n; i++)
        if (const char* e = std::getenv(keys[i].env)) {
            const bool flag = !keys[i].field || keys[i].field == &Options::data_driven_schedule || keys[i].field == &Options::host_blocking ||
                              keys[i].field == &Options::force_redo;
            if (e[0]) (void)option_set(o, keys[i].key, e); else if (flag) (void)option_set(o, keys[i].key, "1");
        }
}

}
#endif
```

lfbm5d_amd/csrc/lfbm5d_pass.hip:

```cpp
#include "lfbm5d_ctx.h"

namespace lfbm5d_host {

lfbm5d_ctx* new_ctx(int device, std::string& err) {
    hipError_t e;
    lfbm5d_ctx* c = new lfbm5d_ctx();
    c->device = device;
    std::memset(&c->stats, 0, sizeof(c->stats));
    if ((e = hipStreamCreateWithFlags(&c->stream, hipStreamNonBlocking)) != hipSuccess) { err = hipGetErrorString(e); delete c; return nullptr; }
    if ((e = prepare_group_kernels()) != hipSuccess || (e = prepare_scan2_kernels()) != hipSuccess) { err = std::string("kernel LDS limits: ") + hipGetErrorString(e); (void)hipStreamDestroy(c->stream); delete c; return nullptr; }
    if ((e = hipHostMalloc((void**)&c->h_small, 64 * sizeof(unsigned))) != hipSuccess) { err = hipGetErrorString(e); (void)hipStreamDestroy(c->stream); delete c; return nullptr; }
    return c;
}


hipEvent_t get_event(lfbm5d_ctx* c) {
    if (c->ev_used == c->ev_pool.size()) {
        hipEvent_t e; (void)hipEventCreate(&e); c->ev_pool.push_back(e);
    }
    return c->ev_pool[c->ev_used++];
}

void drain_events(lfbm5d_ctx* c) {
    for (const PassEvents& pe : c->pending) {
// ... 30 lines not shown
void ind_init(std::vector<unsigned>& v, unsigned max_size, unsigned N, unsigned step) {
    v.clear();
    unsigned ind = N;
    while (ind < max_size - N) { v.push_back(ind); ind += step; }
    if (v.back() < max_size - N - 1) v.push_back(max_size - N - 1);
}

void build_tables(GroupTables& t, unsigned k, unsigned aw, unsigned ah) {
    std::memset(&t, 0, sizeof(t));
    static const float q8[4][4] = {{0.1924f, 0.2989f, 0.3846f, 0.4325f}, {0.2989f, 0.4642f, 0.5974f, 0.6717f},
                                   {0.3846f, 0.5974f, 0.7688f, 0.8644f}, {0.4325f, 0.6717f, 0.8644f, 0.9718f}};
    static const float q12[6][6] = {{0.1924f, 0.2615f, 0.3251f, 0.3782f, 0.4163f, 0.4362f},
                                    {0.2615f, 0.3554f, 0.4419f, 0.5139f, 0.5657f, 0.5927f},
                                    {0.3251f, 0.4419f, 0.5494f, 0.6390f, 0.7033f, 0.7369f},
                                    {0.3782f, 0.5139f, 0.6390f, 0.7433f, 0.8181f, 0.8572f},
                                    {0.4163f, 0.5657f, 0.7033f, 0.8181f, 0.9005f, 0.9435f},
                                    {0.4362f, 0.5927f, 0.7369f, 0.8572f, 0.9435f, 0.9885f}};
    const float coef = 0.5f / (float)k;
    for (unsigned i = 0; i < k; i++)
        for (unsigned j = 0; j < k; j++) {
            const unsigned h = k / 2, a = i < h ? i : k - 1 - i, b = j < h ? j : k - 1 - j;
            t.kaiser[i * k + j] = k == 8 ? q8[a][b] : (k == 12 ? q12[a][b] : 1.0f);
            if (i == 0 && j == 0) { t.cn2[0] = 0.5f * coef; t.cni2[0] = 2.0f; }
            else if (i * j == 0)  { t.cn2[i * k + j] = (float)(kSqrt2Inv * coef); t.cni2[i * k + j] = (float)kSqrt2; }
            else                  { t.cn2[i * k + j] = coef; t.cni2[i * k + j] = 1.0f; }
            t.cos2[i * k + j] = (float)std::cos(kPi * (j + 0.5) * i / k);
        }
    const float c4 = 0.5f / (std::sqrt((float)aw) * std::sqrt((float)ah));
    for (unsigned i = 0; i < ah; i++)
        for (unsigned j = 0; j < aw; j++) {
            if (i == 0 && j == 0) { t.cn4[0] = (float)(0.5f * c4); t.cni4[0] = 2.0f; }
            else if (i * j == 0)  { t.cn4[i * aw + j] = (float)(kSqrt2Inv * c4); t.cni4[i * aw + j] = (float)kSqrt2; }
            else                  { t.cn4[i * aw + j] = c4; t.cni4[i * aw + j] = 1.0f; }
        }
    for (unsigned u = 0; u < 3; u++)
        for (unsigned j = 0; j < 3; j++) t.cos3[u * 3 + j] = (float)std::cos(kPi * (j + 0.5) * u / 3.0);
    for (unsigned u = 0; u < aw && aw <= (unsigned)kBigAw; u++)
        for (unsigned j = 0; j < aw; j++) t.cosw[u * aw + j] = (float)std::cos(kPi * (j + 0.5) * u / (double)aw);
    for (unsigned n = 1; n <= (unsigned)kBigAw; n++) {
        for (unsigned u = 0; u < n; u++)
            for (unsigned j = 0; j < n; j++) t.cos1[n][u * n + j] = (float)std::cos(kPi * (j + 0.5) * u / n);
        const float c1 = (float)((float)kSqrt2 / std::sqrt((double)n));
        t.cn1[n][0] = (float)(kSqrt2Inv * c1); t.cni1[n][0] = (float)kSqrt2;
        for (unsigned i = 1; i < n; i++) { t.cn1[n][i] = c1; t.cni1[n][i] = 1.0f; }
        t.c1inv[n] = 0.5f * (float)kSqrt2Inv / std::sqrt((float)n);
    }
    for (unsigned l = 0; l < 6; l++) {
        const unsigned n = 1u << l;
        float* ct = l < 5 ? t.cos5[l] : t.cos5x;
        for (unsigned uu = 0; uu < n; uu++)
            for (unsigned j = 0; j < n; j++) ct[uu * n + j] = (float)std::cos(kPi * (j + 0.5) * uu / n);
        const float c5 = (float)((float)kSqrt2 / std::sqrt((double)n));
        t.cn5_0[l] = (float)(kSqrt2Inv * c5); t.cn5[l] = c5;
        t.c5inv[l] = 0.5f * (float)kSqrt2Inv / std::sqrt((float)n);
    }
    const float cn = 1.f / (std::sqrt(2.f) * 128.f), s = 1.f / std::sqrt(2.f);
    const float a1[10] = {3.f, -3.f, -22.f, 22.f, 128.f, 128.f, 22.f, -22.f, -3.f, 3.f};
    const float b1[10] = {3.f, 3.f, -22.f, -22.f, 128.f, -128.f, 22.f, 22.f, -3.f, -3.f};
    for (int i = 0; i < 10; i++) { t.lpd[i] = a1[i] * cn; t.hpr[i] = b1[i] * cn; }
    t.hpd[4] = -s; t.hpd[5] = s; t.lpr[4] = s; t.lpr[5] = s;
    t.coef2inv = 1.0f / (float)(k * 2);
    t.coef4inv = 1.0f / (std::sqrt((float)aw) * std::sqrt((float)ah) * 2.0f);
    if (aw == 3 && ah == 3) {
        const double r3 = std::sqrt(3.0), alpha[3] = {2.0, r3, 1.0}, gamma[3] = {1.0, r3, 1.0};
        for (unsigned v = 0; v < 3; v++)
            for (unsigned u = 0; u < 3; u++) {
                const double F = alpha[v] * alpha[u] * (double)t.cn4[v * 3 + u];
                t.ht3_f[v * 3 + u] = (float)F;
                t.ht3_gf[v * 3 + u] = (float)(F * (double)t.cni4[v * 3 + u] * (double)t.coef4inv * gamma[v] * gamma[u]);
            }
    }
}

bool is_pow2(unsigned n) { return n && !(n & (n - 1)); }

int validate(lfbm5d_ctx* c, int step, const lfbm5d_params* P, unsigned aw, unsigned ah, unsigned C, bool bm3d) {
    if (bm3d) {
        if (aw != 1 || ah != 1) return fail(c, "BM3D works on single images");
        if (C != 1 && C != 3) return fail(c, "unsupported: chnls must be 1 or 3");
        if (P->k < 2 || P->k > (unsigned)kMaxK) return fail(c, "unsupported: patch size k outside 2..32");
        if (P->tau_2D != LFBM5D_DCT && P->tau_2D != LFBM5D_BIOR) return fail(c, "BM3D: tau_2D must be dct or bior");
        if (P->tau_2D == LFBM5D_BIOR && !is_pow2(P->k)) return fail(c, "bior1.5 needs a power-of-two patch size");
        if (!is_pow2(P->N) || P->N < 2 || P->N > (unsigned)kMaxN3) return fail(c, "unsupported: BM3D N must be a power of two in 2..32");
        if (P->nSim < 1 || P->nSim > 48 || P->p < 1) return fail(c, "bad search window / step");
        return 0;
    }
    if (aw != ah || aw < 3 || !(aw & 1) || aw > (unsigned)kBigAw) return fail(c, "unsupported: angular search window must be a square of 3 .. 17 SAIs a side (aswSize 1 to 8)");
    if (C != 1 && C != 3) return fail(c, "unsupported: chnls must be 1 or 3");
    if (P->k < 2 || P->k > (unsigned)kMaxK) return fail(c, "unsupported: patch size k outside 2..32");
    if (P->tau_2D == LFBM5D_BIOR && !is_pow2(P->k)) return fail(c, "bior1.5 needs a power-of-two patch size");
    if (P->tau_2D != LFBM5D_ID && P->tau_2D != LFBM5D_DCT && P->tau_2D != LFBM5D_BIOR) return fail(c, "bad tau_2D");
    if (P->tau_4D != LFBM5D_ID && P->tau_4D != LFBM5D_DCT && P->tau_4D != LFBM5D_SADCT) return fail(c, "bad tau_4D");
    if (P->tau_5D != LFBM5D_HAAR && P->tau_5D != LFBM5D_HADAMARD && P->tau_5D != LFBM5D_DCT) return fail(c, "bad tau_5D");
    if (!is_pow2(P->N) || P->N > (unsigned)kMaxN3) return fail(c, "unsupported: N must be a power of two <= 32");
    if (P->nSim < 1 || P->nDisp < 1 || P->p < 1) return fail(c, "bad search window / step");
    if (P->nSim > 48 || P->nDisp > 24) return fail(c, "unsupported: nSim > 48 or nDisp > 24");
    (void)step;
    return 0;
}

int pass_impl(lfbm5d_ctx* c, int step, const lfbm5d_params* P, unsigned aw, unsigned ah, unsigned Wb,
              unsigned Hb, unsigned C, const float* d_noisy, const float* d_basic, float* d_num,
              float* d_den, const unsigned* h_mask, const unsigned* h_proc, unsigned cst, unsigned pst,
              bool bm3d) {
    const bool est_ready = c->est_ready;
    c->est_ready = false;
    const bool direct = c->direct.on;
    c->direct.on = false;
    if (validate(c, step, P, aw, ah, C, bm3d)) return 1;
    if (step == 2 && !d_basic) return fail(c, "step 2 needs the basic estimate");
    const unsigned A = aw * ah, k = P->k, k2 = k * k, N = P->N, nHW = P->nSim + P->nDisp;
    const size_t plane = (size_t)Wb * Hb;
    hipStream_t s = c->stream;
    GeomCache& gc = c->gc[c->gslot];
    if (Hb < 2 * nHW + k + 1 || Wb < 2 * nHW + k + 1) return fail(c, "window smaller than the search range");
    if (Hb > 65535 || Wb > 65535) return fail(c, "unsupported: window larger than 65535 pixels a side");

    float sig[3] = {0, 0, 0};
    if (sigma_table(P->sigma, C, P->color_space, sig)) return fail(c, "bad color space");
    const float tauMatch = bm3d ? (step == 1 ? (C == 1 ? 3.f : 1.f) * (sig[0] < 35.0f ? 2500 : 5000)
                                             : (sig[0] < 35.0f ? 400.f : 3500.f))
                                : (C == 1 ? 3.f : 1.f) * (sig[0] < 35.0f ? (step == 1 ? 3000 : 2000) : 5000);
    const float thr = tauMatch * k * k;
    float lambda = P->lambda;
    if (!bm3d && step == 1 && P->tau_2D == LFBM5D_ID && P->tau_4D == LFBM5D_DCT) lambda /= (float)kSqrt2;
    SaiMask mask_bits = sai_mask_none(), proc_bits = sai_mask_none();
    for (unsigned st = 0; st < A; st++) { if (h_mask[st]) mask_bits.set(st); if (h_proc[st]) proc_bits.set(st); }
    if (pst >= A || cst >= A) return fail(c, "cst / pst outside the angular window");
    if (!mask_bits.test(pst)) return fail(c, "processed SAI is empty");

    const bool centre = pst == cst;
    if (direct && (!centre || !est_ready || bm3d || c->pass_world != 1 || c->pass_reduce)) return fail(c, "direct sums: not a single-pass window of the graph form");
    const unsigned key[5] = {Wb, Hb, k, nHW, P->p};
    if (centre && (std::memcmp(key, gc.grid_key, sizeof(key)) != 0 || gc.last_refs_host.empty())) {
        std::vector<unsigned> rows, cols;
        ind_init(rows, Hb - k + 1, nHW, P->p);
        ind_init(cols, Wb - k + 1, nHW, P->p);
        gc.n_ref_rows = (unsigned)rows.size(); gc.n_ref_cols = (unsigned)cols.size();
        gc.last_refs_host.resize(rows.size() * cols.size());
        for (size_t i = 0; i < rows.size(); i++)
            for (size_t j = 0; j < cols.size(); j++) gc.last_refs_host[i * cols.size() + j] = rows[i] * Wb + cols[j];
        std::vector<int> rslot(Hb + 64, -1);
        for (size_t i = 0; i < rows.size(); i++) rslot[rows[i]] = (int)i;
        HIPCK(c, gc.rslot.reserve(rslot.size() * sizeof(int)));
        HIPCK(c, hipMemcpyAsync(gc.rslot.p, rslot.data(), rslot.size() * sizeof(int), hipMemcpyHostToDevice, s));
        HIPCK(c, gc.refs.reserve(gc.last_refs_host.size() * sizeof(unsigned)));
        HIPCK(c, hipMemcpyAsync(gc.refs.p, gc.last_refs_host.data(), gc.last_refs_host.size() * sizeof(unsigned), hipMemcpyHostToDevice, s));
        HIPCK(c, hipStreamSynchronize(s));
        std::memcpy(gc.grid_key, key, sizeof(key));
        std::memcpy(gc.rslot_key, key, sizeof(key));
    }
    unsigned R = gc.n_ref_rows * gc.n_ref_cols;
    const unsigned R_full = R;
    std::vector<unsigned> row_start;
    const bool dev_list = !centre && c->pass_world == 1 && std::memcmp(key, gc.rslot_key, sizeof(key)) == 0 && !(c->opt->kernels & kOptSubsetListHost);
    if (dev_list) {
        HIPCK(c, c->sub_flags.reserve((size_t)R_full));
        HIPCK(c, c->sub_cnt.reserve(sizeof(unsigned)));
        HIPCK(c, gc.refs.reserve((size_t)R_full * sizeof(unsigned)));
        unsigned* const d_cnt = c->sub_cnt.as<unsigned>();
        HIPCK(c, launch_subset_list(s, d_den + (size_t)pst * C * plane, Wb, k, nHW, P->p, gc.n_ref_rows, gc.n_ref_cols, Hb - k - nHW, Wb - k - nHW,
                                    reinterpret_cast<unsigned char*>(c->sub_flags.p), gc.refs.as<unsigned>(), d_cnt));
        HIPCK(c, hipMemcpyAsync(&R, d_cnt, sizeof(unsigned), hipMemcpyDeviceToHost, s));
        HIPCK(c, hipStreamSynchronize(s));
        std::memset(gc.grid_key, 0, sizeof(gc.grid_key));
        gc.last_refs_host.resize(R);
        if (R == 0) { c->last_n_refs = 0; return 0; }
        HIPCK(c, hipMemcpyAsync(gc.last_refs_host.data(), gc.refs.p, R * sizeof(unsigned), hipMemcpyDeviceToHost, s));
        HIPCK(c, hipStreamSynchronize(s));
        row_start.assign({0u, R});
        if (N > 1 && (c->opt->kernels & kOptSubsetScanV1)) {
            HIPCK(c, c->refmap.reserve(plane * sizeof(int)));
            HIPCK(c, launch_fill_i32(s, c->refmap.as<int>(), -1, plane));
            HIPCK(c, launch_refmap(s, gc.refs.as<unsigned>(), R, c->refmap.as<int>()));
        }
    } else
    if (!centre) {
        std::vector<float> den0(plane);
        HIPCK(c, hipMemcpyAsync(den0.data(), d_den + (size_t)pst * C * plane, plane * sizeof(float), hipMemcpyDeviceToHost, s));
        HIPCK(c, hipStreamSynchronize(s));
        auto denoised = [&](unsigned p_idx) {
            for (unsigned pp = 0; pp < k; pp++)
                for (unsigned q = 0; q < k; q++)
                    if (den0[p_idx + pp * Wb + q] == 0.0f) return false;
            return true;
        };
        const unsigned max_h = Hb - k + 1, max_w = Wb - k + 1;
        std::vector<unsigned> refs, tmp;
        row_start.clear();
        auto scan_row = [&](unsigned i) {
            tmp.clear();
            for (unsigned j = nHW; j < max_w - nHW; j += P->p)
                if (!denoised(i * Wb + j)) tmp.push_back(j);
            const bool border = tmp.empty() ? true : (tmp.back() < max_w - nHW - 1);
            if (border && !denoised(i * Wb + max_w - nHW - 1)) tmp.push_back(max_w - nHW - 1);
            if (!tmp.empty()) { row_start.push_back((unsigned)refs.size()); for (unsigned j : tmp) refs.push_back(i * Wb + j); return true; }
            return false;
        };
        unsigned last_row = 0; bool any = false;
        for (unsigned i = nHW; i < max_h - nHW; i += P->p) if (scan_row(i)) { last_row = i; any = true; }
        if (!any || last_row < max_h - nHW - 1) scan_row(max_h - nHW - 1);
        row_start.push_back((unsigned)refs.size());
        gc.last_refs_host = refs;
        std::memset(gc.grid_key, 0, sizeof(gc.grid_key));
        R = (unsigned)refs.size();
        if (R == 0) { c->last_n_refs = 0; return 0; }
        HIPCK(c, gc.refs.reserve(R * sizeof(unsigned)));
        HIPCK(c, hipMemcpyAsync(gc.refs.p, refs.data(), R * sizeof(unsigned), hipMemcpyHostToDevice, s));
        HIPCK(c, c->refmap.reserve(plane * sizeof(int)));
        HIPCK(c, launch_fill_i32(s, c->refmap.as<int>(), -1, plane));
        HIPCK(c, launch_refmap(s, gc.refs.as<unsigned>(), R, c->refmap.as<int>()));
        HIPCK(c, hipStreamSynchronize(s));
    }

    const unsigned NsS = 2 * P->nSim + 1, NsD = 2 * P->nDisp + 1;
    unsigned slots[kBigA]; unsigned n_slots = 0;
    for (unsigned st = 0; st < A; st++) if (st != pst && mask_bits.test(st)) slots[n_slots++] = st;
    const unsigned Nst = N > 1 ? N : 1;
    HIPCK(c, c->est.reserve((kEstLead + A * plane + 256) * sizeof(float)));
    float* const est = c->est.as<float>() + kEstLead;
    const bool full_scan = !centre && N > 1 && std::memcmp(key, gc.rslot_key, sizeof(key)) == 0 && !(c->opt->kernels & kOptSubsetScanV1);
    const unsigned R_sc = full_scan ? R_full : R;
    if (N > 1 && (size_t)R_sc * NsS * NsS * sizeof(float) > 0x7fffffffull) return fail(c, "unsupported: candidate score table of 2 GiB or more (reference patches x (2 nSim + 1)^2 x 4 B)");
    if (N > 1) HIPCK(c, c->scores.reserve((size_t)R_sc * NsS * NsS * sizeof(float)));
    HIPCK(c, c->self_idx.reserve((size_t)R * Nst * sizeof(unsigned)));
    HIPCK(c, c->self_cnt.reserve((size_t)R * sizeof(unsigned)));
    HIPCK(c, c->best.reserve(A * plane * sizeof(unsigned)));
    HIPCK(c, c->shape.reserve(A * plane));
    const size_t per_group = (size_t)Nst * A * C * k2;
    unsigned band_groups = R;
    {
        constexpr size_t kFiltCapBytes = (size_t)12 << 30;
        size_t cap = std::min<size_t>(kFiltCapBytes, (size_t)0xfff00000ull * sizeof(float));
        if (c->opt->band_mb > 0) cap = std::min<size_t>(cap, (size_t)c->opt->band_mb << 20);
        const size_t row_groups = centre ? gc.n_ref_cols : 1;
        if ((size_t)R * per_group * sizeof(float) > cap) {
            const size_t rows_fit = std::max<size_t>(1, cap / (per_group * sizeof(float) * row_groups));
            band_groups = (unsigned)std::min<size_t>(R, rows_fit * row_groups);
        }
    }
    HIPCK(c, c->filt.reserve((size_t)band_groups * per_group * sizeof(float)));
    HIPCK(c, c->wgt.reserve((size_t)R * C * sizeof(float)));
    HIPCK(c, c->aggpos.reserve((size_t)A * R * Nst * sizeof(unsigned)));
    HIPCK(c, c->gpos.reserve((size_t)A * R * Nst * sizeof(unsigned)));
    HIPCK(c, c->gofs.reserve((size_t)A * R * Nst * sizeof(unsigned)));
    HIPCK(c, c->gok.reserve((size_t)R * Nst * sizeof(unsigned)));
    HIPCK(c, c->sa_list.reserve((size_t)(4 * (size_t)R + 1) * sizeof(unsigned)));
    HIPCK(c, c->gshape.reserve((size_t)R * (A > (unsigned)kMaxA ? kShapeInfoBigBytes : kShapeInfoBytes)));
    HIPCK(c, gc.tb.reserve(sizeof(GroupTables)));
    if (!c->counters.p) {
        HIPCK(c, c->counters.reserve(32 * sizeof(unsigned long long)));
        HIPCK(c, hipMemsetAsync(c->counters.p, 0, 32 * sizeof(unsigned long long), s));
    }
    unsigned long long* const d_counters = c->counters.as<unsigned long long>() + 16 * c->gslot;
    if (gc.tb_key[0] != k || gc.tb_key[1] != aw || gc.tb_key[2] != ah) {
        GroupTables tb;
        build_tables(tb, k, aw, ah);
        HIPCK(c, hipMemcpyAsync(gc.tb.p, &tb, sizeof(tb), hipMemcpyHostToDevice, s));
        HIPCK(c, hipStreamSynchronize(s));
        gc.tb_key[0] = k; gc.tb_key[1] = aw; gc.tb_key[2] = ah;
    }

    PassEvents pe; pe.comm = false;
    for (int i = 0; i < 5; i++) pe.e[i] = get_event(c);

    const float* sub = step == 1 ? d_noisy : d_basic;
    if (!est_ready) HIPCK(c, launch_estimate_multi(s, d_num, d_den, sub, est, plane, C, A, mask_bits));
    if (c->pass_world > 1 && c->pass_rank > 0) {
        HIPCK(c, hipMemsetAsync(d_num, 0, A * C * plane * sizeof(float), s));
        HIPCK(c, hipMemsetAsync(d_den, 0, A * C * plane * sizeof(float), s));
    }

    HIPCK(c, hipEventRecord(pe.e[0], s));
    ScanArgs sa;
    std::memset(&sa, 0, sizeof(sa));
    sa.dbg = d_counters + 4;
    sa.est = est; sa.W = Wb; sa.H = Hb; sa.k = k; sa.pst = pst;
    sa.nSim = P->nSim; sa.nDisp = P->nDisp; sa.nHW = nHW;
    sa.n_ref_rows = gc.n_ref_rows; sa.n_ref_cols = gc.n_ref_cols; sa.p = P->p;
    sa.scores = c->scores.as<float>(); sa.tables = c->tables.as<float>(); sa.rslot = gc.rslot.as<int>(); sa.refmap = (centre || full_scan) ? nullptr : c->refmap.as<int>(); sa.scores_bytes = (unsigned)((size_t)R_sc * NsS * NsS * sizeof(float));
    sa.n_self = N > 1 ? (P->nSim + 1) * NsS : 0;
    sa.n_stereo = n_slots * NsD * NsD;
    for (unsigned i = 0; i < n_slots; i++) sa.st_of_slot[i] = slots[i];
    sa.est_planes = A;
    sa.opt = c->opt->kernels; sa.lds_cap = (unsigned)std::max(0, c->opt->scan_lds_cap);
    const bool opt_v1 = (sa.opt & (kOptScanV1 | kOptScanAny)) != 0, opt_ft = (sa.opt & kOptScanFullTables) != 0;
    const unsigned skey[8] = {sa.n_self, sa.n_stereo, sa.nSim, sa.nDisp, sa.k, Hb, Wb,
                              1u | ((centre || full_scan) ? 0u : 2u) | (opt_v1 ? 4u : 0u) | (opt_ft ? 8u : 0u) | ((sa.opt & kOptScanAny) ? 16u : 0u)};
    const bool scan_changed = std::memcmp(skey, gc.scan_key, sizeof(skey)) != 0;
    if (scan_changed) gc.scan_version = bm_scan_version(sa);
    const int scan_version = gc.scan_version;
    c->last_scan_version = scan_version;
    const bool select_regs = N > 1 && (centre || full_scan) && self_select_regs_covers(P->nSim) && !(c->opt->kernels & kOptSelectPrefill);
    const bool unfilled = select_regs && scan_version >= 2 && sa.refmap == nullptr && !bm3d;
    if (N > 1 && !unfilled) HIPCK(c, launch_fill_f32(s, c->scores.as<float>(), 2 * thr, (size_t)R_sc * NsS * NsS));
    c->unfilled.pending = unfilled;
    if (unfilled) {
        c->unfilled.n_rows = gc.n_ref_rows; c->unfilled.n_cols = gc.n_ref_cols; c->unfilled.W = Wb; c->unfilled.nSim = P->nSim; c->unfilled.nHW = nHW;
        c->unfilled.p = P->p; c->unfilled.last_r = Hb - k - nHW; c->unfilled.last_c = Wb - k - nHW; c->unfilled.fill = 2 * thr;
    }
    if (scan_version == 1) {
        HIPCK(c, c->tables.reserve(std::max<size_t>(1, scan_tables_floats(sa, 1, n_slots, 0)) * sizeof(float)));
        sa.tables = c->tables.as<float>();
    }
    if (scan_version >= 2) {
        if (scan_changed) {
            if (!scan2_plan(sa, gc.scan_plan, &gc.scan_lds, &gc.scan_nwg_slot)) return fail(c, "scan plan");
            HIPCK(c, gc.scan_wgs.reserve(gc.scan_plan.size() * sizeof(Scan2Wg)));
            HIPCK(c, hipMemcpyAsync(gc.scan_wgs.p, gc.scan_plan.data(), gc.scan_plan.size() * sizeof(Scan2Wg), hipMemcpyHostToDevice, s));
            HIPCK(c, hipStreamSynchronize(s));
        }
        sa.wgs = gc.scan_wgs.as<Scan2Wg>(); sa.n_wgs = (unsigned)gc.scan_plan.size();
        sa.lcol_stride = scan2_lcol_stride(sa);
        HIPCK(c, c->scan_lcol.reserve((size_t)(sa.n_self + sa.n_stereo) * sa.lcol_stride * sizeof(float)));
        sa.lcol = c->scan_lcol.as<float>();
        sa.nwg_slot = gc.scan_nwg_slot;
        HIPCK(c, c->tables.reserve(std::max<size_t>(1, scan_tables_floats(sa, scan_version, n_slots, sa.nwg_slot)) * sizeof(float)));
        sa.tables = c->tables.as<float>();
        HIPCK(c, launch_bm_scan2(s, sa, gc.scan_lds, scan_version == 3));
    } else
        HIPCK(c, launch_bm_scan(s, sa));
    std::memcpy(gc.scan_key, skey, sizeof(skey));
    if (select_regs)
        HIPCK(c, launch_self_select_regs(s, c->scores.as<float>(), gc.refs.as<unsigned>(), R, Wb, P->nSim, N, thr,
                                         c->self_idx.as<unsigned>(), c->self_cnt.as<unsigned>(),
                                         full_scan ? gc.n_ref_cols : 0u, nHW, P->p, Hb - k - nHW, Wb - k - nHW, unfilled));
    else if (N > 1)
        HIPCK(c, launch_self_select(s, c->scores.as<float>(), gc.refs.as<unsigned>(), R, Wb, P->nSim, N, thr,
                                    c->self_idx.as<unsigned>(), c->self_cnt.as<unsigned>(),
                                    full_scan ? gc.n_ref_cols : 0u, nHW, P->p, Hb - k - nHW, Wb - k - nHW));
    else
        HIPCK(c, launch_self_trivial(s, gc.refs.as<unsigned>(), R, c->self_idx.as<unsigned>(), c->self_cnt.as<unsigned>()));
    if (n_slots && scan_version == 3)
        HIPCK(c, launch_stereo_argmin3(s, c->tables.as<float>(), slots, n_slots, sa.nwg_slot, Wb, Hb, k, P->nDisp, thr,
                                       c->best.as<unsigned>(), c->shape.as<unsigned char>()));
    else if (n_slots && scan_version == 2)
        HIPCK(c, launch_stereo_argmin2(s, c->tables.as<float>(), slots, n_slots, Wb, Hb, k, P->nDisp, thr,
                                       c->best.as<unsigned>(), c->shape.as<unsigned char>()));
    else if (n_slots)
        HIPCK(c, launch_stereo_argmin(s, c->tables.as<float>(), slots, n_slots, Wb, Hb, k, P->nDisp, thr,
                                      c->best.as<unsigned>(), c->shape.as<unsigned char>()));
    HIPCK(c, hipEventRecord(pe.e[1], s));

    unsigned ref_begin, n_groups;
    if (centre) {
        unsigned rb = 0, re = gc.n_ref_rows;
        lfbm5d_shard_rows(gc.n_ref_rows, c->pass_rank, c->pass_world, &rb, &re);
        ref_begin = rb * gc.n_ref_cols; n_groups = (re - rb) * gc.n_ref_cols;
    } else {
        unsigned rb = 0, re = (unsigned)row_start.size() - 1;
        lfbm5d_shard_rows((unsigned)row_start.size() - 1, c->pass_rank, c->pass_world, &rb, &re);
        ref_begin = row_start[rb]; n_groups = row_start[re] - row_start[rb];
    }

    GroupArgs ga;
    std::memset(&ga, 0, sizeof(ga));
    ga.noisy = d_noisy; ga.basic = d_basic; ga.num = d_num; ga.den = d_den;
    ga.refs = gc.refs.as<unsigned>(); ga.self_idx = c->self_idx.as<unsigned>(); ga.self_cnt = c->self_cnt.as<unsigned>();
    ga.best = c->best.as<unsigned>(); ga.shape = c->shape.as<unsigned char>(); ga.tb = gc.tb.as<GroupTables>();
    ga.wgt = c->wgt.as<float>(); ga.aggpos = c->aggpos.as<unsigned>(); ga.gpos = c->gpos.as<unsigned>(); ga.gofs = c->gofs.as<unsigned>(); ga.gok = c->gok.as<unsigned>(); ga.sa_list = c->sa_list.as<unsigned>(); ga.gshape = c->gshape.p; ga.n_refs_total = R; ga.counters = d_counters;
    ga.ref_begin = ref_begin; ga.n_groups = n_groups;
    ga.Wb = Wb; ga.Hb = Hb; ga.C = C; ga.A = A; ga.k = k; ga.N = Nst; ga.pst = pst;
    ga.mask_bits = mask_bits; ga.proc_bits = proc_bits;
    ga.tau2 = P->tau_2D; ga.tau4 = P->tau_4D; ga.tau5 = P->tau_5D; ga.useSD = P->useSD;
    ga.step = step; ga.lambda = lambda; ga.fill_quirk = centre ? 1u : 0u;
    for (int i = 0; i < 3; i++) ga.sigma[i] = sig[i];
    if (A == 9 && step == 1) {
        GroupTables ht;
        build_tables(ht, k, 3, 3);
        for (int ch = 0; ch < 3; ch++) {
            const float T = lambda * sig[ch] * 1.41421356237309505f;
            for (int st = 0; st < 9; st++)
                for (int l = 0; l < 4; l++) ga.ht3_T[ch][st][l] = (float)((double)T / ((double)ht.ht3_f[st] * std::pow(2.0, -0.5 * l)));
            for (int st = 0; st < 9; st++) {
                double K = 0.0;
                for (int l = 0; l < 4; l++) K = std::max(K, (double)kHtGuardAbs[st][l] / (double)ga.ht3_T[ch][st][l]);
                ga.ht3_K[ch][st] = std::nextafter((float)std::min(K, 1e30), INFINITY);
            }
        }
    }
    ga.bm3d = bm3d ? 1u : 0u;
    ga.opt = c->opt->kernels;
    if (const size_t sb = group_scratch_bytes(ga)) {
        HIPCK(c, c->gscratch.reserve(sb));
        ga.scratch = c->gscratch.as<float>(); ga.scratch_floats = sb / sizeof(float);
    }
    AggArgs aa;
    std::memset(&aa, 0, sizeof(aa));
    aa.num = d_num; aa.den = d_den; aa.wgt = ga.wgt; aa.aggpos = ga.aggpos; aa.n_refs_total = R; aa.refs = ga.refs;
    aa.self_idx = ga.self_idx; aa.self_cnt = ga.self_cnt; aa.best = ga.best; aa.shape = ga.shape; aa.tb = ga.tb;
    aa.ref_begin = ref_begin; aa.n_groups = n_groups; aa.n_ref_rows = gc.n_ref_rows; aa.n_ref_cols = gc.n_ref_cols;
    aa.Wb = Wb; aa.Hb = Hb; aa.C = C; aa.A = A; aa.k = k; aa.N = Nst; aa.pst = pst; aa.p = P->p;
    aa.nHW = nHW; aa.nSim = P->nSim; aa.nDisp = P->nDisp;
    aa.mask_bits = mask_bits; aa.proc_bits = proc_bits; aa.tau4 = P->tau_4D; aa.irregular = centre ? 0u : 1u;
    aa.wchan0 = (bm3d && P->useSD) ? 1u : 0u;
    aa.opt = c->opt->kernels;
    if (direct) {
        aa.num = c->direct.num; aa.den = c->direct.den; aa.direct = 1u; aa.lf_stride = c->direct.lf_stride; aa.sai = c->direct.sai;
    }
    const bool sai_major = A >= kSaiMajorMinA && !(c->opt->kernels & kOptFiltGroupMajor);
    const size_t per_group_bias = sai_major ? per_group / A : per_group;
    if (n_groups <= band_groups) {
        ga.filt_sai_stride = aa.filt_sai_stride = sai_major ? (unsigned long long)n_groups * (per_group / A) : 0ull;
        ga.filt = c->filt.as<float>() - (size_t)ref_begin * per_group_bias;
        aa.filt = c->filt.as<float>(); aa.filt_bytes = (unsigned long long)n_groups * per_group * sizeof(float);
        if (n_groups) HIPCK(c, launch_group(s, ga));
        HIPCK(c, hipEventRecord(pe.e[2], s));
        if (n_groups) HIPCK(c, launch_aggregate(s, aa));
        HIPCK(c, hipEventRecord(pe.e[3], s));
    } else {
        bool first = true;
        for (unsigned b0 = ref_begin; b0 < ref_begin + n_groups; b0 += band_groups) {
            const unsigned nb = std::min(band_groups, ref_begin + n_groups - b0);
            ga.filt_sai_stride = aa.filt_sai_stride = sai_major ? (unsigned long long)nb * (per_group / A) : 0ull;
            ga.ref_begin = b0; ga.n_groups = nb; ga.filt = c->filt.as<float>() - (size_t)b0 * per_group_bias;
            aa.ref_begin = b0; aa.n_groups = nb; aa.filt = c->filt.as<float>(); aa.filt_bytes = (unsigned long long)nb * per_group * sizeof(float);
            HIPCK(c, launch_group(s, ga));
            if (first) HIPCK(c, hipEventRecord(pe.e[2], s));
            first = false;
            HIPCK(c, launch_aggregate(s, aa));
            c->stats.launches_group += 1; c->stats.launches_aggregate += 1;
        }
        c->stats.launches_group -= 1; c->stats.launches_aggregate -= 1;
        HIPCK(c, hipEventRecord(pe.e[3], s));
    }

    if (c->comm && c->pass_reduce) {
        const size_t cnt = (size_t)A * C * plane;
        if (ncclAllReduce(d_num, d_num, cnt, ncclFloat, ncclSum, c->comm, s) != ncclSuccess) return fail(c, "ncclAllReduce(num) failed");
        if (ncclAllReduce(d_den, d_den, cnt, ncclFloat, ncclSum, c->comm, s) != ncclSuccess) return fail(c, "ncclAllReduce(den) failed");
        HIPCK(c, hipEventRecord(pe.e[4], s));
        pe.comm = true;
    }
    c->pending.push_back(pe);

    c->stats.passes += 1;
    c->stats.groups += n_groups;
    c->stats.launches_group += n_groups ? 1 : 0;
    c->stats.launches_aggregate += n_groups ? 1 : 0;
    c->last_n_refs = R; c->last_N = Nst; c->last_A = A; c->last_plane = plane; c->last_gslot = c->gslot;
    return 0;
}

int fold_counters(lfbm5d_ctx* c, const lfbm5d_params* P, unsigned A, unsigned C, int step, int slot) {
    unsigned long long h[4] = {0, 0, 0, 0};
    if (!c->counters.p) return 0;
    unsigned long long* const d_counters = c->counters.as<unsigned long long>() + 16 * slot;
    HIPCK(c, hipMemcpyAsync(h, d_counters, sizeof(h), hipMemcpyDeviceToHost, c->stream));
    HIPCK(c, hipStreamSynchronize(c->stream));
    HIPCK(c, hipMemsetAsync(d_counters, 0, sizeof(h), c->stream));
    c->stats.stack_patches += h[0];
    c->stats.sadct_groups += h[1];
#ifdef LFBM5D_PHASE_TIMING
    {
        unsigned long long ph[12];
        (void)hipMemcpy(ph, d_counters + 4, sizeof(ph), hipMemcpyDeviceToHost);
        (void)hipMemset(d_counters + 4, 0, sizeof(ph));
        std::fprintf(stderr, "[phases step %d]", step);
        for (int i = 0; i < 12; i++) std::fprintf(stderr, " %.3g", (double)ph[i]);
        std::fprintf(stderr, "\n");
    }
#endif
    c->stats.algorithmic_bytes += (double)h[0] * A * P->k * P->k * C * (4.0 * (step == 2 ? 2 : 1) + 16.0);
    return 0;
}

}
```

lfbm5d_amd/csrc/lfbm5d_scan2.hip:

```cpp
#include "lfbm5d_kernels.h"

#include <algorithm>
#include <cstdlib>
#include <cstring>
#include <type_traits>
#include <vector>

#pragma clang fp contract(off)

namespace lfbm5d {

namespace {

typedef float v4f __attribute__((ext_vector_type(4)));
typedef int v4i __attribute__((ext_vector_type(4)));

constexpr unsigned kRsrcFlags = 0x00020000u;
constexpr int kPairStoreAux = 2;
constexpr int kS2HandAux = 17;
constexpr int kLeadBytes = 32;

template <int K> struct S2Geom {
    static constexpr int CW1 = 64 + K;
    static constexpr int LAG = (63 - K + 7) / 8;
    static constexpr int LEAD1 = (K + 7) / 8;
    static constexpr int RR1 = 8 * (LAG + LEAD1 + 2);
    static constexpr int RRp1 = RR1 + 13;
    __host__ __device__ static int lead2(int rh) { return (7 + K + rh) / 8; }
    __host__ __device__ static int rr2(int rh) { return 8 * (LAG + lead2(rh) + 2); }
    __host__ __device__ static int cw2(int ch) { return (64 + K + ch + 3) & ~3; }
};

__device__ __forceinline__ int s2_grid_index(int v, int n, int last, int nHW, int p) {
    if (v == last) return n - 1;
    const int d = v - nHW;
    if (d < 0 || d % p) return -1;
    const int i = d / p;
    return i < n - 1 ? i : -1;
}

__device__ __forceinline__ void lds_barrier() {
    asm volatile("s_waitcnt lgkmcnt(0)\n\ts_barrier" ::: "memory");
}

constexpr int kS2NW = 11;
constexpr int kS2NL = 1;
constexpr int kS2NI = 6;
constexpr int kS2LD = 2;

template <int K, bool STEREO, int NW, int NL>
__device__ __forceinline__ void scan2_loader(const ScanArgs& a, const Scan2Wg& g, float* lds, int r0, const int lw) {
    static_assert(NL == 1, "one loader wave");
    __builtin_amdgcn_s_setprio(3);
    typedef S2Geom<K> G;
    constexpr int CW1 = G::CW1, RR1 = G::RR1, RRp1 = G::RRp1, LEAD1 = G::LEAD1;
    const int lane = threadIdx.x & 63;
    const int W = a.W, H = a.H;
    const int half = STEREO ? (int)a.nDisp : (int)a.nSim;
    const int b = STEREO ? (int)a.nDisp : (int)a.nHW;
    const int trim = STEREO ? K - 1 : 0;
    const int Ns = 2 * half + 1, ncand = Ns * Ns;
    const int nrows = H - 2 * b - trim, ncols = W - 2 * b - trim;
    const size_t WH = (size_t)W * H;
    const int CW2 = G::cw2(g.ch), LEAD2 = G::lead2(g.rh), RR2 = G::rr2(g.rh), RRp2 = RR2 + 13;
    const int LEADM = LEAD2 > LEAD1 ? LEAD2 : LEAD1;
    float* ring1 = lds;
    float* ring2 = lds + CW1 * RRp1;
    float* lcst = ring2 + CW2 * RRp2;
    const unsigned pl1 = a.pst, pl2 = STEREO ? a.st_of_slot[g.slot] : a.pst;
    const __amdgpu_buffer_rsrc_t rE = __builtin_amdgcn_make_buffer_rsrc((void*)(a.est - kLeadBytes / 4), 0, (int)(a.est_planes * WH * 4 + kLeadBytes + 1024), kRsrcFlags);
    const __amdgpu_buffer_rsrc_t rLA = __builtin_amdgcn_make_buffer_rsrc((void*)a.lcol, 0, (int)((a.n_self + a.n_stereo) * a.lcol_stride * 4), kRsrcFlags);
    const int n1 = 2 * CW1, nit = n1 + 2 * CW2;
    bool pv[kS2NI], p1[kS2NI];
    int py0[kS2NI], pgo[kS2NI], pslot[kS2NI];
    float* pdst[kS2NI];
#pragma unroll
    for (int k = 0; k < kS2NI; k++) {
        const int item = k * 64 + lane;
        pv[k] = item < nit; p1[k] = item < n1;
        const int it = p1[k] ? item : item - n1;
        const int r = it & 7, quad = it >> 3;
        py0[k] = (p1[k] ? b : b + g.r2lo) + r;
        pgo[k] = (int)((p1[k] ? pl1 : pl2) * WH) * 4 + kLeadBytes + ((p1[k] ? 0 : g.c2lo) + 4 * quad - 1) * 4;
        pdst[k] = (p1[k] ? ring1 : ring2) + 4 * quad * (p1[k] ? RRp1 : RRp2);
        pslot[k] = (r + (p1[k] ? 0 : r0)) % (p1[k] ? RR1 : RR2);
    }
    static_assert(NW <= 16, "two hand-off values per loader lane");
    (void)lw;
    const int he = lane & 7;
    int hbase[2];
    float* hdst[2];
#pragma unroll
    for (int q = 0; q < 2; q++) {
        const int hw = (q * 64 + lane) >> 3;
        hbase[q] = -1;
        if (hw < NW) {
            const int tw = g.tab[hw];
            if (tw >= 0) hbase[q] = ((STEREO ? (int)a.n_self + g.slot * ncand + tw : tw) * (int)a.lcol_stride + 65 + he) * 4;
        }
        hdst[q] = lcst + (hw < NW ? hw : 0) * 8 + he;
    }
    const bool hok[2] = {(lane >> 3) < NW, ((64 + lane) >> 3) < NW};

    const int nstrips = (ncols - 1 + 63) / 64;
    for (int strip = 0; strip < nstrips; strip++) {
        const int cb = b + 1 + 64 * strip;
        const int last_lane = min(63, ncols - 2 - 64 * strip);
        const int nchunks = (((nrows - 1) + last_lane + 15) >> 4) * 2;
        lds_barrier();
        int ws[kS2NI];
#pragma unroll
        for (int k = 0; k < kS2NI; k++) ws[k] = pslot[k];
        auto piece_load = [&](int k, int j) -> v4f {
            const int y = min(max(py0[k] + 8 * j, 0), H - 1);
            return __builtin_bit_cast(v4f, __builtin_amdgcn_raw_buffer_load_b128(rE, pv[k] ? pgo[k] + (y * W + cb) * 4 : -1, 0, 0));
        };
        auto piece_write = [&](int k, const v4f v) {
            if (pv[k]) {
                const int RRk = p1[k] ? RR1 : RR2, RRpk = p1[k] ? RRp1 : RRp2;
                const int slot = ws[k];
                ws[k] += 8; ws[k] = ws[k] >= RRk ? ws[k] - RRk : ws[k];
                float* d = pdst[k] + slot;
                d[0] = v[0]; d[RRpk] = v[1]; d[2 * RRpk] = v[2]; d[3 * RRpk] = v[3];
                if (slot < 7) { d += RRk; d[0] = v[0]; d[RRpk] = v[1]; d[2 * RRpk] = v[2]; d[3 * RRpk] = v[3]; }
            }
        };
        auto hand_load = [&](int q, int c) -> float {
            return __builtin_bit_cast(float, __builtin_amdgcn_raw_buffer_load_b32(rLA, hbase[q] >= 0 ? hbase[q] + 32 * c : -1, 0, kS2HandAux));
        };
        for (int j = 0; j <= LEADM; j++) {
            v4f v[kS2NI];
#pragma unroll
            for (int k = 0; k < kS2NI; k++) v[k] = piece_load(k, j);
#pragma unroll
            for (int k = 0; k < kS2NI; k++) if (j <= (p1[k] ? LEAD1 : LEAD2)) piece_write(k, v[k]);
        }
        v4f stg[kS2LD][kS2NI];
#pragma unroll
        for (int d = 0; d < kS2LD; d++)
#pragma unroll
            for (int k = 0; k < kS2NI; k++) stg[d][k] = piece_load(k, (p1[k] ? LEAD1 : LEAD2) + 1 + d);
#pragma unroll
        for (int q = 0; q < 2; q++) { const float h0 = hand_load(q, 0); if (hok[q]) hdst[q][0] = h0; }
        float hv[kS2LD][2];
#pragma unroll
        for (int d = 0; d < kS2LD; d++)
#pragma unroll
            for (int q = 0; q < 2; q++) hv[d][q] = hand_load(q, 1 + d);
        lds_barrier();
#ifdef LFBM5D_PHASE_TIMING
        long long lk[2] = {0, 0};
        long long llast = (long long)__builtin_readcyclecounter();
#endif
        auto chunk = [&](const int d, const int cc) {
#pragma unroll
            for (int k = 0; k < kS2NI; k++) {
                piece_write(k, stg[d][k]);
                stg[d][k] = piece_load(k, cc + (p1[k] ? LEAD1 : LEAD2) + 1 + kS2LD);
            }
#pragma unroll
            for (int q = 0; q < 2; q++) {
                if (hok[q]) hdst[q][((cc + 1) & 1) * NW * 8] = hv[d][q];
                hv[d][q] = hand_load(q, cc + 1 + kS2LD);
            }
#ifdef LFBM5D_PHASE_TIMING
            { const long long tn = (long long)__builtin_readcyclecounter(); lk[0] += tn - llast; llast = tn; }
#endif
            lds_barrier();
#ifdef LFBM5D_PHASE_TIMING
            { const long long tn = (long long)__builtin_readcyclecounter(); lk[1] += tn - llast; llast = tn; }
#endif
        };
        static_assert(kS2LD == 2, "the chunk count is even");
        for (int c = 0; c < nchunks; c += 2) { chunk(0, c); chunk(1, c + 1); }
#ifdef LFBM5D_PHASE_TIMING
        if (lane == 0 && a.dbg && STEREO) { atomicAdd(&a.dbg[5], (unsigned long long)lk[0]); atomicAdd(&a.dbg[11], (unsigned long long)lk[1]); }
#endif
    }
    lds_barrier();
}

template <int K, bool STEREO, int NW, bool COMB>
__device__ __forceinline__ void scan2_table(const ScanArgs& a, const Scan2Wg& g, float* lds, const int w, const int r0) {
    typedef S2Geom<K> G;
    constexpr int CW1 = G::CW1, RR1 = G::RR1, RRp1 = G::RRp1;
    const int lane = threadIdx.x & 63;
    const int W = a.W, H = a.H;
    const int half = STEREO ? (int)a.nDisp : (int)a.nSim;
    const int b = STEREO ? (int)a.nDisp : (int)a.nHW;
    const int trim = STEREO ? K - 1 : 0;
    const int Ns = 2 * half + 1, ncand = Ns * Ns;
    const int nrows = H - 2 * b - trim, ncols = W - 2 * b - trim, band_rows = H - 2 * b;
    const size_t WH = (size_t)W * H;
    const int tab_w = g.tab[w];
    const bool live = tab_w >= 0;
    const int tb = live ? tab_w : g.tab[0];
    const int di = tb / Ns, dj = tb % Ns;
    const int dioff = STEREO ? di - half : di, djoff = dj - half;
    const int r2lo = g.r2lo, c2lo = g.c2lo;
    const int CW2 = G::cw2(g.ch), RR2 = G::rr2(g.rh), RRp2 = RR2 + 13;
    float* ring1 = lds;
    float* ring2 = lds + CW1 * RRp1;
    const float* lcst = ring2 + CW2 * RRp2;
    const short* rs = reinterpret_cast<const short*>(lcst + 2 * NW * 8);
    float* const xch = const_cast<float*>(lcst) + 2 * NW * 8;
    if (STEREO && COMB && !live) {
        const v4f inf4 = {__builtin_inff(), __builtin_inff(), __builtin_inff(), __builtin_inff()};
#pragma unroll
        for (int ch = 0; ch < 2; ch++) {
            *reinterpret_cast<v4f*>(xch + (ch * NW + w) * 512 + lane * 8) = inf4;
            *reinterpret_cast<v4f*>(xch + (ch * NW + w) * 512 + lane * 8 + 4) = inf4;
        }
    }

    const unsigned pl1 = a.pst, pl2 = STEREO ? a.st_of_slot[g.slot] : a.pst;
    const float* img1 = a.est + (size_t)pl1 * WH;
    const float* img2 = a.est + (size_t)pl2 * WH;
    const int dk = dioff * W + djoff;
    const __amdgpu_buffer_rsrc_t rs1 = __builtin_amdgcn_make_buffer_rsrc((void*)img1, 0, (int)(WH * 4 + 1024), kRsrcFlags);
    const __amdgpu_buffer_rsrc_t rs2 = __builtin_amdgcn_make_buffer_rsrc((void*)(img2 + dk), 0, (int)(WH * 4 + 1024), kRsrcFlags);
    const int tglob = STEREO ? (int)a.n_self + g.slot * ncand + tb : tb;
    float* lcolT = a.lcol + (size_t)tglob * a.lcol_stride;
    const __amdgpu_buffer_rsrc_t rL = __builtin_amdgcn_make_buffer_rsrc((void*)lcolT, 0, live ? (int)(a.lcol_stride * 4) : 0, kRsrcFlags);
    const size_t tstride = (STEREO && !COMB) ? stereo_table_stride2(a.W, a.H, a.k, a.nDisp) : 0;
    float* table = (STEREO && !COMB) ? a.tables + (size_t)(g.slot * ncand + tb) * tstride : nullptr;
    const __amdgpu_buffer_rsrc_t rT = __builtin_amdgcn_make_buffer_rsrc((void*)table, 0, (STEREO && !COMB && live) ? (int)(tstride * 4) : 0, kRsrcFlags);
    const unsigned NCH = stereo_part_chunks(a.H, a.k, a.nDisp);
    const size_t pstride = COMB ? stereo_part_stride(a.W, a.H, a.k, a.nDisp) : 0;
    const size_t estride = COMB ? stereo_edge_stride(a.W, a.H, a.k, a.nDisp) : 0;
    const unsigned n_slots = STEREO ? a.n_stereo / (unsigned)ncand : 0;
    float* part = COMB ? a.tables + ((size_t)g.slot * a.nwg_slot + g.wgj) * pstride * 2 : nullptr;
    float* edge = COMB ? a.tables + (size_t)n_slots * a.nwg_slot * pstride * 2 + (size_t)(g.slot * ncand + tb) * estride : nullptr;
    const __amdgpu_buffer_rsrc_t rP = __builtin_amdgcn_make_buffer_rsrc((void*)part, 0, COMB ? (int)(pstride * 8) : 0, kRsrcFlags);
    const __amdgpu_buffer_rsrc_t rEd = __builtin_amdgcn_make_buffer_rsrc((void*)edge, 0, (COMB && live) ? (int)(estride * 4) : 0, kRsrcFlags);
    const __amdgpu_buffer_rsrc_t rS = __builtin_amdgcn_make_buffer_rsrc((void*)a.scores, 0, (!STEREO && live) ? (int)a.scores_bytes : 0, kRsrcFlags);
    const int SRq = (int)stereo_table_srq(a.H, a.k, a.nDisp);
    const int nstrips = (ncols - 1 + 63) / 64;
    const int col0_off = nstrips * SRq * 256;

    const int gR = a.n_ref_rows, gC = a.n_ref_cols, gP = a.p, gN = a.nHW;
    const int lastR = H - K - gN, lastC = W - K - gN;
    const int djs = dj - half;
    const int ord_fwd = dj * Ns + di;
    const int ord_bwd = (-djs + half) * Ns + (half + 1) + (half - di);
    const int row_bytes = gC * ncand * 4;

    float corner = 0.0f;
    {
        float* scr = ring1 + w * 256;
        for (int e = lane; e < K * K; e += 64) {
            const int q = (b + e / K) * W + b + e % K;
            const float d = img2[q + dk] - img1[q];
            scr[e] = d * d;
        }
        __builtin_amdgcn_fence(__ATOMIC_RELEASE, "wavefront");
        __builtin_amdgcn_wave_barrier();
        __builtin_amdgcn_fence(__ATOMIC_ACQUIRE, "wavefront");
        for (int e = 0; e < K * K; e++) corner += scr[e];
        auto emit0 = [&](int i, float v, bool on) {
            __builtin_amdgcn_raw_buffer_store_b32(__builtin_bit_cast(int, v), rL, on ? (64 + i) * 4 : -1, 0, 0);
            if (STEREO && COMB) {
                __builtin_amdgcn_raw_buffer_store_b32(__builtin_bit_cast(int, v), rEd, on ? i * 4 : -1, 0, 0);
            } else if (STEREO) {
                __builtin_amdgcn_raw_buffer_store_b32(__builtin_bit_cast(int, v), rT, on ? (col0_off + i) * 4 : -1, 0, 0);
            } else {
                const int cxa = s2_grid_index(b, gC, lastC, gN, gP);
                const int cxb = di > 0 ? s2_grid_index(b + djs, gC, lastC, gN, gP) : -1;
                const int yy = min(b + i, H - 1);
                const int ra = a.rslot[yy], rb = a.rslot[yy + di];
                __builtin_amdgcn_raw_buffer_store_b32(__builtin_bit_cast(int, v), rS, (on && (ra | cxa) >= 0) ? ((ra * gC + cxa) * ncand + ord_fwd) * 4 : -1, 0, 0);
                __builtin_amdgcn_raw_buffer_store_b32(__builtin_bit_cast(int, v), rS, (on && (rb | cxb) >= 0) ? ((rb * gC + cxb) * ncand + ord_bwd) * 4 : -1, 0, 0);
            }
        };
        emit0(0, corner, lane == 0);
        constexpr int K4 = K / 4;
        auto load_e = [&](int i, v4f* lo1, v4f* lo2, v4f* hi1, v4f* hi2) {
            const int ra = min(b + i - 1, H - 1), rb = min(b + i - 1 + K, H - 1);
#pragma unroll
            for (int j = 0; j < K4; j++) {
                lo1[j] = __builtin_bit_cast(v4f, __builtin_amdgcn_raw_buffer_load_b128(rs1, (ra * W + b + 4 * j) * 4, 0, 0));
                lo2[j] = __builtin_bit_cast(v4f, __builtin_amdgcn_raw_buffer_load_b128(rs2, (ra * W + b + 4 * j) * 4, 0, 0));
                hi1[j] = __builtin_bit_cast(v4f, __builtin_amdgcn_raw_buffer_load_b128(rs1, (rb * W + b + 4 * j) * 4, 0, 0));
                hi2[j] = __builtin_bit_cast(v4f, __builtin_amdgcn_raw_buffer_load_b128(rs2, (rb * W + b + 4 * j) * 4, 0, 0));
            }
        };
        float carry = corner;
        for (int i0 = 1; i0 < nrows; i0 += 64) {
            const int i = i0 + lane;
            v4f lo1[K4], lo2[K4], hi1[K4], hi2[K4];
            load_e(i, lo1, lo2, hi1, hi2);
            float e[K];
            const bool lo_in = b + i - 1 < H - b, hi_in = b + i - 1 + K < H - b;
#pragma unroll
            for (int j = 0; j < K4; j++)
#pragma unroll
                for (int q = 0; q < 4; q++) {
                    const float dl = lo2[j][q] - lo1[j][q], dh = hi2[j][q] - hi1[j][q];
                    e[4 * j + q] = i < nrows ? (hi_in ? dh * dh : 0.0f) - (lo_in ? dl * dl : 0.0f) : 0.0f;
                }
            const int m = min(64, nrows - i0);
            float mine = 0.0f;
            for (int l = 0; l < m; l++) {
                float cand = carry;
#pragma unroll
                for (int q = 0; q < K; q++) cand += e[q];
                carry = __int_as_float(__builtin_amdgcn_readlane(__float_as_int(cand), l));
                if (lane == l) mine = carry;
            }
            emit0(i, mine, i < nrows);
        }
    }

    float row0_left = corner;
    for (int strip = 0; strip < nstrips; strip++) {
        const int cb = b + 1 + 64 * strip;
        const int x = cb + lane;
        const bool col_ok = x < b + ncols;
        const int last_lane = min(63, ncols - 2 - 64 * strip);
        const int lane_eff = col_ok ? lane : 0x40000000;
        const int cm1 = (STEREO || x + K - 1 < W - b) ? -1 : 0;

        asm volatile("s_waitcnt vmcnt(0)" ::: "memory");
        lds_barrier();
        lds_barrier();

        auto Draw = [&](int rho, int c) -> float {
            const float i1 = ring1[c * RRp1 + rho];
            const float i2 = ring2[(c + djoff - c2lo) * RRp2 + rho + dioff - r2lo + r0];
            const float d = i2 - i1;
            return d * d;
        };

        float S0 = 0.0f;
        {
            float e[K];
#pragma unroll
            for (int p = 0; p < K; p++) {
                float dr = Draw(p, lane + K);
                if (!STEREO) dr = __int_as_float(__float_as_int(dr) & cm1);
                e[p] = dr - Draw(p, lane);
            }
            float carry = row0_left;
            for (int l = 0; l <= last_lane; l++) {
                float cand = carry;
#pragma unroll
                for (int p = 0; p < K; p++) cand += e[p];
                carry = __int_as_float(__builtin_amdgcn_readlane(__float_as_int(cand), l));
                if (lane == l) S0 = carry;
            }
        }
        const int cx = STEREO ? -1 : s2_grid_index(x, gC, lastC, gN, gP);
        const int cx2 = (STEREO || di == 0) ? -1 : s2_grid_index(x + djs, gC, lastC, gN, gP);
        const int base_fwd = (col_ok && cx >= 0) ? (cx * ncand + ord_fwd) * 4 : -1;
        const int base_bwd = (col_ok && cx2 >= 0 && di > 0) ? (cx2 * ncand + ord_bwd) * 4 : -1;
        if (STEREO && COMB) {
            __builtin_amdgcn_raw_buffer_store_b32(__builtin_bit_cast(int, S0), rEd, lane == 0 ? (nrows + strip) * 4 : -1, 0, 0);
        } else if (STEREO) {
            __builtin_amdgcn_raw_buffer_store_b32(__builtin_bit_cast(int, S0), rT, lane == 0 ? (strip * SRq * 256 + 3) * 4 : -1, 0, 0);
        } else {
            const int ry = s2_grid_index(b, gR, lastR, gN, gP);
            __builtin_amdgcn_raw_buffer_store_b32(__builtin_bit_cast(int, S0), rS, (ry >= 0 && base_fwd >= 0) ? ry * row_bytes + base_fwd : -1, 0, 0);
            const int ry2 = di > 0 ? s2_grid_index(b + di, gR, lastR, gN, gP) : -1;
            __builtin_amdgcn_raw_buffer_store_b32(__builtin_bit_cast(int, S0), rS, (ry2 >= 0 && base_bwd >= 0) ? ry2 * row_bytes + base_bwd : -1, 0, 0);
        }
        bool fast = false;
        int nfF = 0x40000000, nfB = 0x40000000, offF = -1, offB = -1, incF = 0, incB = 0;
        unsigned boundF = 0, boundB = 0;
        if (!STEREO) {
            const bool offpat = (base_fwd >= 0 && (x - gN) % gP != 0) || (base_bwd >= 0 && (x + djs - gN) % gP != 0);
            fast = !__builtin_amdgcn_ballot_w64(offpat) && (lastR - gN) % gP == 0;
            if (fast) {
                const int tF0 = ((-(2 + 64 * strip)) % gP + gP) % gP;
                const int tB0 = ((-(2 + 64 * strip + djs + di)) % gP + gP) % gP;
                nfF = tF0; nfB = di > 0 ? tB0 : 0x40000000;
                if (base_fwd >= 0) { offF = ((1 + tF0 - lane) / gP) * row_bytes + base_fwd; incF = row_bytes; }
                if (base_bwd >= 0) { offB = ((1 + tB0 - lane + di) / gP) * row_bytes + base_bwd; incB = row_bytes; }
                boundF = (unsigned)max(min(nrows - 2, lastR - b - 1), -1);
                boundB = (unsigned)max(min(nrows - 2, lastR - b - 1 - di), -1);
            }
        }

        float F1[K], F2[K];
#pragma unroll
        for (int m = 0; m < K; m++) {
            const int row = max(m - lane, 0);
            float dr = Draw(row, lane + K);
            if (!STEREO) dr = __int_as_float(__float_as_int(dr) & cm1);
            F1[m] = dr; F2[m] = Draw(row, lane);
        }
        float curS = S0;
        float left_prev = row0_left;
        unsigned slot1 = (unsigned)((K - lane + RR1) % RR1);
        unsigned slot2 = (unsigned)(((K - lane + dioff - r2lo + r0) % RR2 + RR2) % RR2);
        const float* const colA = ring1 + (lane + K) * RRp1;
        const float* const colB = ring2 + (lane + K + djoff - c2lo) * RRp2;
        const int KB2 = K * RRp2;
        int voffT = ((strip * SRq + 1) * 64 + lane) * 16;
        int voffL = lane == 63 ? (64 + 1 - 63) * 4 : 0x70000000;
        const float* const lcw = lcst + w * 8;
        constexpr int kShare = (512 + NW - 1) / NW;
        const int ordv = (int)g.ord[lane & 15];
        const int rp = w * kShare + lane;
        const bool rok = lane < kShare && rp < 512;
        auto reduce_chunk = [&](const int cprev) {
            const float* src = xch + (cprev & 1) * NW * 512 + (rok ? rp : 0);
            float v[NW];
#pragma unroll
            for (int q = 0; q < NW; q++) v[q] = src[q * 512];
            float best = v[0];
#pragma unroll
            for (int q = 1; q + 1 < NW; q += 2) best = __builtin_fminf(__builtin_fminf(best, v[q]), v[q + 1]);
            if ((NW & 1) == 0) best = __builtin_fminf(best, v[NW - 1]);
            int bq = NW - 1;
#pragma unroll
            for (int q = NW - 2; q >= 0; q--) bq = v[q] == best ? q : bq;
            const int bo = __builtin_amdgcn_ds_bpermute(bq << 2, ordv);
            typedef int v2i __attribute__((ext_vector_type(2)));
            const v2i pr = {__float_as_int(best), bo};
            __builtin_amdgcn_raw_buffer_store_b64(pr, rP, rok ? (int)(((strip * NCH + cprev) * 512 + rp) * 8) : -1, 0, kPairStoreAux);
        };

#ifdef LFBM5D_PHASE_TIMING
        long long tk[4] = {0, 0, 0, 0};
        long long tlast = (long long)__builtin_readcyclecounter();
#define S2_MARK(i) do { const long long tn = (long long)__builtin_readcyclecounter(); tk[i] += tn - tlast; tlast = tn; } while (0)
#else
#define S2_MARK(i) do {} while (0)
#endif
#if defined(LFBM5D_PHASE_TIMING) && LFBM5D_PHASE_TIMING >= 2
        long long tq[4] = {0, 0, 0, 0};
        long long qlast = 0;
#define S2_Q0() do { asm volatile("" ::: "memory"); qlast = (long long)__builtin_readcyclecounter(); } while (0)
#define S2_QMARK(i) do { asm volatile("" ::: "memory"); const long long tn = (long long)__builtin_readcyclecounter(); tq[i] += tn - qlast; qlast = tn; } while (0)
#else
#define S2_Q0() do {} while (0)
#define S2_QMARK(i) do {} while (0)
#endif
        auto body16 = [&](auto fl_tag, const int t0) {
            constexpr bool EDGE = decltype(fl_tag)::value;
            const int rel_start = lane_eff - t0;
            const int rel_band = band_rows - K + lane - t0;
#pragma unroll
            for (int ch = 0; ch < 2; ch++) {
                const int tc = t0 + 8 * ch;
                const v4f lc[2] = {*reinterpret_cast<const v4f*>(lcw + ch * NW * 8), *reinterpret_cast<const v4f*>(lcw + ch * NW * 8 + 4)};
                if (!EDGE) S2_Q0();
                if (COMB && tc > 0) reduce_chunk((tc >> 3) - 1);
                if (!EDGE) S2_QMARK(0);
                const float* pA = colA + slot1;
                const float* pB = colB + slot2;
#pragma unroll
                for (int gq = 0; gq < 2; gq++) {
                    const int tg = tc + 4 * gq;
                    const v4f a1 = *reinterpret_cast<const v4f*>(pA + 4 * gq);
                    const v4f a2 = *reinterpret_cast<const v4f*>(pA - K * RRp1 + 4 * gq);
                    const v4f b1 = *reinterpret_cast<const v4f*>(pB + 4 * gq);
                    const v4f b2 = *reinterpret_cast<const v4f*>(pB - KB2 + 4 * gq);
                    v4f e1 = b1 - a1, e2 = b2 - a2;
                    e1 = e1 * e1; e2 = e2 * e2;
                    if (!STEREO) {
#pragma unroll
                        for (int s = 0; s < 4; s++) {
                            int m = cm1;
                            if (EDGE) m = (8 * ch + 4 * gq + s < rel_band) ? m : 0;
                            e1[s] = __int_as_float(__float_as_int(e1[s]) & m);
                            if (EDGE) e2[s] = (8 * ch + 4 * gq + s < rel_band) ? e2[s] : 0.0f;
                        }
                    }
                    v4f out;
#pragma unroll
                    for (int s = 0; s < 4; s++) {
                        const int fs = (8 * ch + 4 * gq + s) % K;
                        const float left = __int_as_float(__builtin_amdgcn_update_dpp(__float_as_int(lc[gq][s]), __float_as_int(curS),
                                                                                      0x138 , 0xf, 0xf, false));
                        float S = left + curS;
                        S = S - left_prev;
                        S = S + e1[s];
                        S = S - e2[s];
                        S = S - F1[fs];
                        S = S + F2[fs];
                        F1[fs] = e1[s]; F2[fs] = e2[s];
                        if (EDGE) S = (rel_start == 8 * ch + 4 * gq + s + 1) ? S0 : S;
                        out[s] = S;
                        curS = S;
                        left_prev = left;
                    }
                    if (STEREO && COMB) {
                        if (live) *reinterpret_cast<v4f*>(xch + (ch * NW + w) * 512 + lane * 8 + 4 * gq) = out;
                    } else if (STEREO) {
                        __builtin_amdgcn_raw_buffer_store_b128(__builtin_bit_cast(v4i, out), rT, voffT, 0, 0);
                        voffT += 1024;
                    } else if (fast) {
#pragma unroll
                        for (int s = 0; s < 4; s++) {
                            const int u = 8 * ch + 4 * gq + s;
                            const float ov = out[s];
                            if (u == nfF) {
                                __builtin_amdgcn_raw_buffer_store_b32(__float_as_int(ov), rS, (unsigned)(u - rel_start) <= boundF ? offF : -1, 0, 0);
                                offF += incF; nfF += gP;
                            }
                            if (u == nfB) {
                                __builtin_amdgcn_raw_buffer_store_b32(__float_as_int(ov), rS, (unsigned)(u - rel_start) <= boundB ? offB : -1, 0, 0);
                                offB += incB; nfB += gP;
                            }
                        }
                    } else {
#pragma unroll
                        for (int s = 0; s < 4; s++) {
                            const float ov = out[s];
                            {
                                const int t = tg + s;
                                const bool act = (unsigned)(t - lane_eff) <= (unsigned)(nrows - 2);
                                const int y = min(max(b + 1 + t - lane, 0), H - 1);
                                const int r1 = rs[y], r2 = rs[y + di];
                                const int v1 = (act && (r1 | base_fwd) >= 0) ? r1 * row_bytes + base_fwd : -1;
                                const int v2 = (act && (r2 | base_bwd) >= 0) ? r2 * row_bytes + base_bwd : -1;
                                if (__builtin_amdgcn_ballot_w64(v1 != -1)) __builtin_amdgcn_raw_buffer_store_b32(__float_as_int(ov), rS, v1, 0, 0);
                                if (__builtin_amdgcn_ballot_w64(v2 != -1)) __builtin_amdgcn_raw_buffer_store_b32(__float_as_int(ov), rS, v2, 0, 0);
                            }
                        }
                    }
                    __builtin_amdgcn_raw_buffer_store_b128(__builtin_bit_cast(v4i, out), rL, voffL, 0, 0);
                    voffL += 16;
                    if (!EDGE) S2_QMARK(1 + gq);
                }
                slot1 += 8; slot1 = min(slot1, slot1 - (unsigned)RR1);
                slot2 += 8; slot2 = min(slot2, slot2 - (unsigned)RR2);
                S2_MARK(EDGE ? 1 : 0);
                lds_barrier();
                S2_MARK(2);
            }
            if (!STEREO) { nfF -= 16; nfB -= 16; }
        };

        const int nsteps = (nrows - 1) + last_lane;
        const int tS1 = (min(nrows - 1, band_rows - K) / 16) * 16;
        auto run = [&]() {
            int t0 = 0;
            for (; t0 < nsteps && t0 < 64; t0 += 16) body16(std::true_type{}, t0);
            for (; t0 < tS1; t0 += 16) body16(std::false_type{}, t0);
            for (; t0 < nsteps; t0 += 16) body16(std::true_type{}, t0);
        };
        S2_MARK(3);
        run();
        if (COMB && nsteps > 0) reduce_chunk(((nsteps + 15) >> 4) * 2 - 1);
        row0_left = __int_as_float(__builtin_amdgcn_readlane(__float_as_int(S0), last_lane));
#if defined(LFBM5D_PHASE_TIMING) && LFBM5D_PHASE_TIMING >= 2
        if (lane == 0 && a.dbg && live && STEREO) {
            for (int i = 0; i < 4; i++) atomicAdd(&a.dbg[i], (unsigned long long)tk[i]);
            atomicAdd(&a.dbg[4], 1ull);
            for (int i = 0; i < 3; i++) atomicAdd(&a.dbg[6 + i], (unsigned long long)tq[i]);
        }
#elif defined(LFBM5D_PHASE_TIMING)
        if (lane == 0 && a.dbg && live) {
            const int base = STEREO ? 0 : 6;
            for (int i = 0; i < 4; i++) atomicAdd(&a.dbg[base + i], (unsigned long long)tk[i]);
            atomicAdd(&a.dbg[base + 4], 1ull);
        }
#endif
    }
    asm volatile("s_waitcnt vmcnt(0)" ::: "memory");
    lds_barrier();
}

template <int K, bool STEREO, int NW, int NL, bool COMB>
__device__ __forceinline__ void scan2_body(const ScanArgs& a, const Scan2Wg& g, float* lds) {
    typedef S2Geom<K> G;
    const int tid = threadIdx.x;
    const int w = __builtin_amdgcn_readfirstlane(tid >> 6);
    const int half = STEREO ? (int)a.nDisp : (int)a.nSim;
    const int Ns = 2 * half + 1;
    int r0;
    {
        const int t0 = g.tab[0], di0 = t0 / Ns, dj0 = t0 % Ns;
        r0 = (4 - (((dj0 - half) - g.c2lo + (STEREO ? di0 - half : di0) - g.r2lo) & 3)) & 3;
    }
    if (!STEREO) {
        float* ring2 = lds + G::CW1 * G::RRp1;
        short* rs = reinterpret_cast<short*>(ring2 + G::cw2(g.ch) * (G::rr2(g.rh) + 13) + 2 * NW * 8);
        for (int i = tid; i < (int)a.H + 64; i += blockDim.x) rs[i] = (short)a.rslot[i];
    }
    if (w >= NW) scan2_loader<K, STEREO, NW, NL>(a, g, lds, r0, w - NW);
    else scan2_table<K, STEREO, NW, COMB>(a, g, lds, w, r0);
}

template <int K, bool COMB>
__global__ __launch_bounds__((kS2NW + kS2NL) * 64) void k_bm_scan2(ScanArgs a) {
    extern __shared__ __attribute__((aligned(16))) float lds2[];
    const Scan2Wg& g = a.wgs[blockIdx.x];
    if (g.slot >= 0) scan2_body<K, true, kS2NW, kS2NL, COMB>(a, g, lds2);
    else scan2_body<K, false, kS2NW, kS2NL, false>(a, g, lds2);
}

struct Argmin2Args { const float* tables; size_t tstride; unsigned st_of_slot[kBigA]; int W, H, k, nDisp, SRq; float thr; unsigned* best; unsigned char* shape; };
__global__ __launch_bounds__(256) void k_stereo_argmin2(Argmin2Args a) {
    const int W = a.W, H = a.H, nDisp = a.nDisp;
    const int span_c = W - 2 * nDisp - a.k + 1, span_r = H - 2 * nDisp - a.k + 1;
    const int nstrips = (span_c - 1 + 63) / 64;
    const int i = blockIdx.x * blockDim.x + threadIdx.x;
    const int n_strip_items = nstrips * a.SRq * 64;
    if (i >= n_strip_items + a.SRq) return;
    const unsigned slot = blockIdx.y, st = a.st_of_slot[slot];
    int r0, col;
    if (i < n_strip_items) {
        const int l = i & 63, qg = (i >> 6) % a.SRq, strip = (i >> 6) / a.SRq;
        r0 = 4 * qg - l - 3; col = 1 + 64 * strip + l;
    } else { r0 = 4 * (i - n_strip_items); col = 0; }
    if (r0 + 3 < 0 || r0 >= span_r || col >= span_c) return;
    const int Ns = 2 * nDisp + 1, ncand = Ns * Ns;
    const size_t WH = (size_t)W * H;
    const float* t = a.tables + (size_t)slot * ncand * a.tstride + (size_t)i * 4;
    float bv[4]; int bo[4], bd[4];
    {
        const v4f v0 = *reinterpret_cast<const v4f*>(t);
#pragma unroll
        for (int e = 0; e < 4; e++) { bv[e] = v0[e]; bo[e] = 0; bd[e] = 0; }
    }
    for (int d0 = 0; d0 < ncand; d0 += 8) {
        v4f v[8];
#pragma unroll
        for (int u = 0; u < 8; u++) v[u] = *reinterpret_cast<const v4f*>(t + (size_t)min(d0 + u, ncand - 1) * a.tstride);
#pragma unroll
        for (int u = 0; u < 8; u++) {
            const int ddk = d0 + u;
            if (ddk < ncand) {
                const int di = ddk / Ns, dj = ddk - di * Ns;
                const int order = dj * Ns + di;
#pragma unroll
                for (int e = 0; e < 4; e++)
                    if (v[u][e] < bv[e] || (v[u][e] == bv[e] && order < bo[e])) { bv[e] = v[u][e]; bo[e] = order; bd[e] = ddk; }
            }
        }
    }
#pragma unroll
    for (int e = 0; e < 4; e++) {
        const int r = r0 + e;
        if (r < 0 || r >= span_r) continue;
        const int pos = (nDisp + r) * W + nDisp + col;
        const int di = bd[e] / Ns, dj = bd[e] % Ns;
        a.best[(size_t)st * WH + pos] = (unsigned)(pos + (di - nDisp) * W + (dj - nDisp));
        a.shape[(size_t)st * WH + pos] = bv[e] < a.thr ? 1 : 0;
    }
}

template <int K> size_t scan2_lds_bytes(const ScanArgs& a, int rh_max, int ch_max) {
    typedef S2Geom<K> G;
    const int RRp2 = G::rr2(rh_max) + 13;
    const size_t tail = std::max<size_t>(a.n_self ? (size_t)(a.H + 64) * sizeof(short) : 0, a.n_stereo ? (size_t)2 * kS2NW * 512 * sizeof(float) : 0);
    return (size_t)(G::CW1 * G::RRp1 + G::cw2(ch_max) * RRp2 + 2 * kS2NW * 8) * sizeof(float) + tail + 16;
}

}

int bm_scan_version(const ScanArgs& a) {
    if (a.opt & (kOptScanV1 | kOptScanAny)) return 1;
    if (a.k != 8 && a.k != 16) return 1;
    if (a.n_self && a.refmap) return 1;
    if ((size_t)a.est_planes * a.W * a.H * 4 + kLeadBytes + 1024 > 0x7fffffffull) return 1;
    std::vector<Scan2Wg> wgs; size_t lds = 0;
    if (!scan2_plan(a, wgs, &lds)) return 1;
    if (a.opt & kOptScanFullTables) return 2;
    return 3;
}

size_t scan_tables_floats(const ScanArgs& a, int version, unsigned n_slots, unsigned nwg_slot) {
    const size_t ncand = (size_t)(2 * a.nDisp + 1) * (2 * a.nDisp + 1);
    if (version == 1) return (size_t)n_slots * ncand * stereo_table_stride(a.W, a.H, a.k, a.nDisp);
    if (version == 2) return (size_t)n_slots * ncand * stereo_table_stride2(a.W, a.H, a.k, a.nDisp);
    return (size_t)n_slots * nwg_slot * stereo_part_stride(a.W, a.H, a.k, a.nDisp) * 2 + (size_t)n_slots * ncand * stereo_edge_stride(a.W, a.H, a.k, a.nDisp);
}

bool scan2_plan(const ScanArgs& a, std::vector<Scan2Wg>& wgs, size_t* lds_bytes, unsigned* nwg_slot) {
    wgs.clear();
    int rh_max = 0, ch_max = 0;
    int wgj = 0;
    auto add = [&](int slot, const std::vector<int>& tabs, int r2lo, int c2lo, int rh, int ch) {
        for (size_t i = 0; i < tabs.size(); i += kS2NW) {
            Scan2Wg g;
            std::memset(&g, 0, sizeof(g));
            for (int w = 0; w < 16; w++) g.tab[w] = (w < kS2NW && i + w < tabs.size()) ? (short)tabs[i + w] : (short)-1;
            if (slot >= 0) { const int Ns = 2 * (int)a.nDisp + 1; for (int w = 0; w < 16; w++) g.ord[w] = g.tab[w] >= 0 ? (short)((g.tab[w] % Ns) * Ns + g.tab[w] / Ns) : (short)0; }
            g.slot = (short)slot; g.r2lo = (short)r2lo; g.c2lo = (short)c2lo; g.rh = (short)rh; g.ch = (short)ch; g.wgj = (short)wgj++;
            wgs.push_back(g);
        }
        rh_max = std::max(rh_max, rh); ch_max = std::max(ch_max, ch);
    };
    if (nwg_slot) *nwg_slot = 0;
    if (a.n_self) {
        const int nSim = (int)a.nSim, Ns = 2 * nSim + 1;
        for (int d0 = 0; d0 <= nSim; d0 += 4)
            for (int j0 = 0; j0 < Ns; j0 += kS2NW)
                for (int cls = 0; cls < 4; cls++) {
                    std::vector<int> tabs;
                    for (int di = d0; di < std::min(d0 + 4, nSim + 1); di++)
                        for (int dj = j0; dj < std::min(j0 + kS2NW, Ns); dj++)
                            if (((di + dj) & 3) == cls) tabs.push_back(di * Ns + dj);
                    if (!tabs.empty()) add(-1, tabs, d0, j0 - nSim, 3, kS2NW - 1);
                }
    }
    if (a.n_stereo) {
        const int nD = (int)a.nDisp, Ns = 2 * nD + 1, ncand = Ns * Ns;
        const int n_slots = (int)a.n_stereo / ncand;
        for (int slot = 0; slot < n_slots; slot++) {
            wgj = 0;
            for (int cls = 0; cls < 4; cls++) {
                std::vector<int> tabs;
                for (int ord = 0; ord < ncand; ord++) {
                    const int dj = ord / Ns, di = ord % Ns;
                    if (((di + dj) & 3) == cls) tabs.push_back(di * Ns + dj);
                }
                if (!tabs.empty()) add(slot, tabs, -nD, -nD, 2 * nD, 2 * nD);
            }
            if (nwg_slot) *nwg_slot = (unsigned)wgj;
        }
    }
    size_t lds = a.k == 8 ? scan2_lds_bytes<8>(a, rh_max, ch_max) : scan2_lds_bytes<16>(a, rh_max, ch_max);
    if (lds_bytes) *lds_bytes = lds;
    const int n1 = 2 * (64 + (int)a.k), n2 = 2 * ((64 + (int)a.k + ch_max + 3) & ~3);
    if (n1 + n2 > 64 * kS2NI || lds > 160 * 1024) return false;
    return !wgs.empty();
}

unsigned scan2_lcol_stride(const ScanArgs& a) {
    const unsigned rows_self = a.n_self ? a.H - 2 * a.nHW : 0, rows_st = a.n_stereo ? a.H - 2 * a.nDisp - (a.k - 1) : 0;
    return ((std::max(rows_self, rows_st) + 64 + 160 + 63) / 64) * 64;
}

hipError_t prepare_scan2_kernels() {
    const void* fns[] = {reinterpret_cast<const void*>(&k_bm_scan2<8, false>), reinterpret_cast<const void*>(&k_bm_scan2<16, false>),
                         reinterpret_cast<const void*>(&k_bm_scan2<8, true>), reinterpret_cast<const void*>(&k_bm_scan2<16, true>)};
    for (const void* f : fns) {
        const hipError_t e = hipFuncSetAttribute(f, hipFuncAttributeMaxDynamicSharedMemorySize, 160 * 1024);
        if (e != hipSuccess) return e;
    }
    return hipSuccess;
}

hipError_t launch_bm_scan2(hipStream_t s, const ScanArgs& a, size_t lds, bool combined) {
    if (!a.n_wgs) return hipSuccess;
    const dim3 blk((kS2NW + kS2NL) * 64);
    if (a.k == 8 && combined) hipLaunchKernelGGL((k_bm_scan2<8, true>), dim3(a.n_wgs), blk, lds, s, a);
    else if (a.k == 8) hipLaunchKernelGGL((k_bm_scan2<8, false>), dim3(a.n_wgs), blk, lds, s, a);
    else if (a.k == 16 && combined) hipLaunchKernelGGL((k_bm_scan2<16, true>), dim3(a.n_wgs), blk, lds, s, a);
    else if (a.k == 16) hipLaunchKernelGGL((k_bm_scan2<16, false>), dim3(a.n_wgs), blk, lds, s, a);
    else return hipErrorInvalidValue;
    return hipGetLastError();
}

struct Argmin3Args { const float* tables; unsigned st_of_slot[kBigA]; int W, H, k, nDisp, n_slots, nwg_slot; float thr; unsigned* best; unsigned char* shape; };
__global__ __launch_bounds__(256) void k_stereo_argmin3(Argmin3Args a) {
    const int W = a.W, H = a.H, nDisp = a.nDisp;
    const int span_c = W - 2 * nDisp - a.k + 1, span_r = H - 2 * nDisp - a.k + 1;
    const int nstrips = (span_c - 1 + 63) / 64;
    const int NCH = (int)stereo_part_chunks(H, a.k, nDisp);
    const size_t pstride = stereo_part_stride(W, H, a.k, nDisp), estride = stereo_edge_stride(W, H, a.k, nDisp);
    const int Ns = 2 * nDisp + 1, ncand = Ns * Ns;
    const unsigned slot = blockIdx.y, st = a.st_of_slot[slot];
    const size_t WH = (size_t)W * H;
    const int i = blockIdx.x * blockDim.x + threadIdx.x;
    const int n_main = nstrips * NCH * 256, n_edge = span_r + nstrips;
    if (i >= n_main + 16 * n_edge) return;
    auto put = [&](int row, int col, float bv, int bo) {
        const int pos = (nDisp + row) * W + nDisp + col;
        const int dj = bo / Ns, di = bo % Ns;
        a.best[(size_t)st * WH + pos] = (unsigned)(pos + (di - nDisp) * W + (dj - nDisp));
        a.shape[(size_t)st * WH + pos] = bv < a.thr ? 1 : 0;
    };
    if (i < n_main) {
        const int p = 2 * (i & 255), c = (i >> 8) % NCH, strip = (i >> 8) / NCH;
        const int l = p >> 3, t = 8 * c + (p & 7);
        const int row = 1 + t - l, col = 1 + 64 * strip + l;
        if (row + 1 < 0 || row >= span_r || col >= span_c) return;
        const v4f* src = reinterpret_cast<const v4f*>(a.tables) + ((size_t)slot * a.nwg_slot * pstride >> 1) + i;
        float bv0 = __builtin_inff(), bv1 = __builtin_inff(); int bo0 = 0x7fffffff, bo1 = 0x7fffffff;
        for (int j0 = 0; j0 < a.nwg_slot; j0 += 16) {
            v4f w8[16];
#pragma unroll
            for (int u = 0; u < 16; u++) {
                w8[u] = __builtin_nontemporal_load(src + (size_t)min(j0 + u, a.nwg_slot - 1) * (pstride >> 1));
            }
#pragma unroll
            for (int u = 0; u < 16; u++) {
                const int o0 = __float_as_int(w8[u][1]), o1 = __float_as_int(w8[u][3]);
                if (w8[u][0] < bv0 || (w8[u][0] == bv0 && o0 < bo0)) { bv0 = w8[u][0]; bo0 = o0; }
                if (w8[u][2] < bv1 || (w8[u][2] == bv1 && o1 < bo1)) { bv1 = w8[u][2]; bo1 = o1; }
            }
        }
        if (row >= 0 && !(row == 0 && l == 0)) put(row, col, bv0, bo0);
        if (row + 1 < span_r && row + 1 >= 0 && !(row + 1 == 0 && l == 0)) put(row + 1, col, bv1, bo1);
    } else {
        const int e = (i - n_main) >> 4, sub = (i - n_main) & 15;
        int row, col;
        if (e < span_r) { row = e; col = 0; } else { row = 0; col = 1 + 64 * (e - span_r); }
        const bool ok = e < n_edge && col < span_c;
        const float* ed = a.tables + (size_t)a.n_slots * a.nwg_slot * pstride * 2 + (size_t)slot * ncand * estride + (ok ? e : 0);
        float bv = __builtin_inff(); int bo = 0x7fffffff;
        for (int d0 = sub; d0 < ncand; d0 += 16 * 8) {
            float v[8];
#pragma unroll
            for (int u = 0; u < 8; u++) v[u] = ed[(size_t)min(d0 + 16 * u, ncand - 1) * estride];
#pragma unroll
            for (int u = 0; u < 8; u++) {
                const int ddk = d0 + 16 * u;
                const int o = (ddk % Ns) * Ns + ddk / Ns;
                if (ddk < ncand && (v[u] < bv || (v[u] == bv && o < bo))) { bv = v[u]; bo = o; }
            }
        }
#pragma unroll
        for (int m = 8; m > 0; m >>= 1) {
            const float ov = __shfl_xor(bv, m, 16); const int oo = __shfl_xor(bo, m, 16);
            if (ov < bv || (ov == bv && oo < bo)) { bv = ov; bo = oo; }
        }
        if (ok && sub == 0) put(row, col, bv, bo);
    }
}

hipError_t launch_stereo_argmin3(hipStream_t s, const float* tables, const unsigned* st_of_slot, unsigned n_slots, unsigned nwg_slot,
                                 unsigned W, unsigned H, unsigned k, unsigned nDisp, float thr,
                                 unsigned* best, unsigned char* shape) {
    Argmin3Args a;
    a.tables = tables; a.W = (int)W; a.H = (int)H; a.k = (int)k; a.nDisp = (int)nDisp; a.n_slots = (int)n_slots; a.nwg_slot = (int)nwg_slot; a.thr = thr; a.best = best; a.shape = shape;
    for (unsigned i = 0; i < n_slots && i < (unsigned)kBigA; i++) a.st_of_slot[i] = st_of_slot[i];
    const unsigned span_c = W - 2 * nDisp - k + 1, span_r = H - 2 * nDisp - k + 1;
    const unsigned nstrips = (span_c - 1 + 63) / 64;
    const unsigned n = nstrips * stereo_part_chunks(H, k, nDisp) * 256 + 16 * (span_r + nstrips);
    hipLaunchKernelGGL(k_stereo_argmin3, dim3((n + 255) / 256, n_slots), dim3(256), 0, s, a);
    return hipGetLastError();
}

hipError_t launch_stereo_argmin2(hipStream_t s, const float* tables, const unsigned* st_of_slot, unsigned n_slots,
                                 unsigned W, unsigned H, unsigned k, unsigned nDisp, float thr,
                                 unsigned* best, unsigned char* shape) {
    const unsigned span_c = W - 2 * nDisp - k + 1;
    Argmin2Args a;
    a.tables = tables; a.tstride = stereo_table_stride2(W, H, k, nDisp); a.W = (int)W; a.H = (int)H; a.k = (int)k; a.nDisp = (int)nDisp; a.thr = thr; a.best = best; a.shape = shape;
    a.SRq = (int)stereo_table_srq(H, k, nDisp);
    const unsigned n = ((span_c - 1 + 63) / 64) * a.SRq * 64 + a.SRq;
    for (unsigned i = 0; i < n_slots && i < (unsigned)kBigA; i++) a.st_of_slot[i] = st_of_slot[i];
    hipLaunchKernelGGL(k_stereo_argmin2, dim3((n + 255) / 256, n_slots), dim3(256), 0, s, a);
    return hipGetLastError();
}

}
```

Measured before the change: 256.3 SAI-megapixels/s.

## Merge per-workgroup stereo argmin partials via 64-bit atomic-min keys

Stereo scan workgroups no longer write separate (score, offset) pairs into a per-workgroup table for a later reduction. Each one now does an atomic min on a packed 64-bit key (order-preserving float bits, then offset) in a single array per slot. The argmin kernel reads one key, resets it to all-ones for the next call, and skips the loop over nwg_slot partial tables. This removes a large write and read of partial-table traffic, at the cost of global atomics and a one-time 0xFF memset whose clean state is tracked across calls. The old pair form stays available behind LFBM5D_ARGMIN_PAIRS.

```diff
diff --git a/lfbm5d_amd/core.py b/lfbm5d_amd/core.py
--- a/lfbm5d_amd/core.py
+++ b/lfbm5d_amd/core.py
@@ -829,8 +829,8 @@
               "LFBM5D_FORCE_REDO", "LFBM5D_SPATIAL_BANDS", "LFBM5D_BAND_HALO", "LFBM5D_SCAN_V1", "LFBM5D_SCAN_ANY", "LFBM5D_SCAN_FULL_TABLES", "LFBM5D_DCT8W_V2",
               "LFBM5D_GROUP_GENERIC", "LFBM5D_NO_SA_KERNELS", "LFBM5D_NO_SLAB_KERNEL", "LFBM5D_WIDE_NOSPLIT", "LFBM5D_AGG_64BIT",
               "LFBM5D_AGG_SCALAR_SCAN", "LFBM5D_SUBSET_LIST_HOST", "LFBM5D_SUBSET_SCAN_V1", "LFBM5D_FILT_GROUP_MAJOR",
-              "LFBM5D_HT_REF_ORDER", "LFBM5D_WINDOW_SUMS_PADDED", "LFBM5D_SELECT_PREFILL")
-OPTION_ENV_EMPTY_OFF = ("LFBM5D_WINDOW_SUMS_PADDED",)
+              "LFBM5D_HT_REF_ORDER", "LFBM5D_WINDOW_SUMS_PADDED", "LFBM5D_SELECT_PREFILL", "LFBM5D_ARGMIN_PAIRS")
+OPTION_ENV_EMPTY_OFF = ("LFBM5D_WINDOW_SUMS_PADDED", "LFBM5D_ARGMIN_PAIRS")
 
 
 class Context:
diff --git a/lfbm5d_amd/csrc/lfbm5d_bm.hip b/lfbm5d_amd/csrc/lfbm5d_bm.hip
--- a/lfbm5d_amd/csrc/lfbm5d_bm.hip
+++ b/lfbm5d_amd/csrc/lfbm5d_bm.hip
@@ -580,11 +580,6 @@
     else scan_any_body<0>(a, (int)blockIdx.x, lds);
 }
 
-__device__ __forceinline__ unsigned f2ord(float f) {
-    const unsigned u = __float_as_uint(f);
-    return (u & 0x80000000u) ? ~u : (u | 0x80000000u);
-}
-
 __device__ __forceinline__ unsigned long long wave_min(unsigned long long v) {
     auto step = [&](auto ctrl, auto rmask, auto bmask, unsigned long long src) {
         constexpr int C = decltype(ctrl)::value, R = decltype(rmask)::value, B = decltype(bmask)::value;
diff --git a/lfbm5d_amd/csrc/lfbm5d_ctx.h b/lfbm5d_amd/csrc/lfbm5d_ctx.h
--- a/lfbm5d_amd/csrc/lfbm5d_ctx.h
+++ b/lfbm5d_amd/csrc/lfbm5d_ctx.h
@@ -125,6 +125,7 @@
     std::vector<hipEvent_t> ev_pool; size_t ev_used = 0;
     std::vector<PassEvents> pending;
     unsigned last_n_refs = 0, last_N = 0, last_A = 0; size_t last_plane = 0; int last_gslot = 0;
+    size_t keys_clean = 0;
     struct UnfilledScores { bool pending = false; unsigned n_rows = 0, n_cols = 0, W = 0, nSim = 0, nHW = 0, p = 0, last_r = 0, last_c = 0; float fill = 0; } unfilled;
 };
 
diff --git a/lfbm5d_amd/csrc/lfbm5d_kernels.h b/lfbm5d_amd/csrc/lfbm5d_kernels.h
--- a/lfbm5d_amd/csrc/lfbm5d_kernels.h
+++ b/lfbm5d_amd/csrc/lfbm5d_kernels.h
@@ -20,6 +20,16 @@
 #endif
 
 namespace lfbm5d {
+
+#if defined(__HIPCC__)
+__device__ __forceinline__ unsigned f2ord(float f) {
+    const unsigned u = __float_as_uint(f);
+    return (u & 0x80000000u) ? ~u : (u | 0x80000000u);
+}
+__device__ __forceinline__ float ord2f(unsigned o) {
+    return __uint_as_float((o & 0x80000000u) ? (o & 0x7fffffffu) : ~o);
+}
+#endif
 
 constexpr int kMaxK = 32;
 constexpr int kMaxA = 49;
@@ -159,6 +169,8 @@
     return (size_t)((ncols - 1 + 63) / 64) * stereo_table_srq(H, k, nDisp) * 256 + stereo_table_srq(H, k, nDisp) * 4;
 }
 
+constexpr int kCombKeys = 1, kCombPairs = 2;
+constexpr unsigned kStereoKeyArrays = 1;
 __host__ __device__ inline unsigned stereo_part_chunks(unsigned H, unsigned k, unsigned nDisp) {
     const unsigned nrows = H - 2 * nDisp - (k - 1);
     return ((nrows - 1 + 63 + 15) / 16) * 2;
@@ -205,6 +217,7 @@
     float* lcol;
     unsigned lcol_stride;
     unsigned nwg_slot;
+    unsigned edge_off;
 };
 
 hipError_t launch_color(hipStream_t s, float* img, unsigned cs, unsigned n_px, int forward);
@@ -259,12 +272,16 @@
 int bm_scan_version(const ScanArgs& a);
 bool scan2_plan(const ScanArgs& a, std::vector<Scan2Wg>& wgs, size_t* lds_bytes, unsigned* nwg_slot = nullptr);
 size_t scan_tables_floats(const ScanArgs& a, int version, unsigned n_slots, unsigned nwg_slot);
+size_t scan_keys_floats(const ScanArgs& a, unsigned n_slots, unsigned nwg_slot);
 unsigned scan2_lcol_stride(const ScanArgs& a);
 hipError_t prepare_scan2_kernels();
-hipError_t launch_bm_scan2(hipStream_t s, const ScanArgs& a, size_t lds_bytes, bool combined);
-hipError_t launch_stereo_argmin3(hipStream_t s, const float* tables, const unsigned* st_of_slot, unsigned n_slots, unsigned nwg_slot,
+hipError_t launch_bm_scan2(hipStream_t s, const ScanArgs& a, size_t lds_bytes, int form);
+hipError_t launch_stereo_argmin3(hipStream_t s, const float* tables, size_t edge_off, const unsigned* st_of_slot, unsigned n_slots, unsigned nwg_slot,
                                  unsigned W, unsigned H, unsigned k, unsigned nDisp, float thr,
                                  unsigned* best, unsigned char* shape);
+hipError_t launch_stereo_argmin_keys(hipStream_t s, float* tables, size_t edge_off, const unsigned* st_of_slot, unsigned n_slots,
+                                     unsigned W, unsigned H, unsigned k, unsigned nDisp, float thr,
+                                     unsigned* best, unsigned char* shape);
 hipError_t launch_stereo_argmin2(hipStream_t s, const float* tables, const unsigned* st_of_slot, unsigned n_slots,
                                  unsigned W, unsigned H, unsigned k, unsigned nDisp, float thr,
                                  unsigned* best, unsigned char* shape);
diff --git a/lfbm5d_amd/csrc/lfbm5d_options.h b/lfbm5d_amd/csrc/lfbm5d_options.h
--- a/lfbm5d_amd/csrc/lfbm5d_options.h
+++ b/lfbm5d_amd/csrc/lfbm5d_options.h
@@ -24,6 +24,7 @@
     kOptFiltGroupMajor = 1u << 12,
     kOptHtReferenceOrder = 1u << 13,
     kOptSelectPrefill = 1u << 14,
+    kOptArgminPairs = 1u << 15,
 };
 
 struct Options {
@@ -66,6 +67,7 @@
         {"filt_group_major", "LFBM5D_FILT_GROUP_MAJOR", nullptr, kOptFiltGroupMajor},
         {"ht_reference_order", "LFBM5D_HT_REF_ORDER", nullptr, kOptHtReferenceOrder},
         {"select_prefill", "LFBM5D_SELECT_PREFILL", nullptr, kOptSelectPrefill},
+        {"argmin_pairs", "LFBM5D_ARGMIN_PAIRS", nullptr, kOptArgminPairs},
     };
     *n = sizeof(keys) / sizeof(keys[0]);
     return keys;
@@ -108,7 +110,7 @@
     size_t n; const OptionKey* keys = option_keys(&n);
     for (size_t i = 0; i < n; i++)
         if (const char* e = std::getenv(keys[i].env)) {
-            const bool flag = !keys[i].field || keys[i].field == &Options::data_driven_schedule || keys[i].field == &Options::host_blocking ||
+            const bool flag = (!keys[i].field && keys[i].bit != kOptArgminPairs) || keys[i].field == &Options::data_driven_schedule || keys[i].field == &Options::host_blocking ||
                               keys[i].field == &Options::force_redo;
             if (e[0]) (void)option_set(o, keys[i].key, e); else if (flag) (void)option_set(o, keys[i].key, "1");
         }
diff --git a/lfbm5d_amd/csrc/lfbm5d_pass.hip b/lfbm5d_amd/csrc/lfbm5d_pass.hip
--- a/lfbm5d_amd/csrc/lfbm5d_pass.hip
+++ b/lfbm5d_amd/csrc/lfbm5d_pass.hip
@@ -356,7 +356,10 @@
     if (scan_version == 1) {
         HIPCK(c, c->tables.reserve(std::max<size_t>(1, scan_tables_floats(sa, 1, n_slots, 0)) * sizeof(float)));
         sa.tables = c->tables.as<float>();
-    }
+        if (n_slots) c->keys_clean = 0;
+    }
+    const bool merged = scan_version == 3 && n_slots && !(sa.opt & kOptArgminPairs);
+    size_t keys_clean = 0;
     if (scan_version >= 2) {
         if (scan_changed) {
             if (!scan2_plan(sa, gc.scan_plan, &gc.scan_lds, &gc.scan_nwg_slot)) return fail(c, "scan plan");
@@ -369,9 +372,28 @@
         HIPCK(c, c->scan_lcol.reserve((size_t)(sa.n_self + sa.n_stereo) * sa.lcol_stride * sizeof(float)));
         sa.lcol = c->scan_lcol.as<float>();
         sa.nwg_slot = gc.scan_nwg_slot;
-        HIPCK(c, c->tables.reserve(std::max<size_t>(1, scan_tables_floats(sa, scan_version, n_slots, sa.nwg_slot)) * sizeof(float)));
+        if (merged) {
+            const size_t kb = scan_keys_floats(sa, n_slots, 0) * sizeof(float);
+            const size_t edge_bytes = (scan_tables_floats(sa, 3, n_slots, 0) - scan_keys_floats(sa, n_slots, 0)) * sizeof(float);
+            const size_t cap_before = c->tables.cap;
+            HIPCK(c, c->tables.reserve(std::max(kb, c->keys_clean) + edge_bytes));
+            keys_clean = c->tables.cap == cap_before ? c->keys_clean : 0;
+            if (keys_clean < kb) {
+                HIPCK(c, hipMemsetAsync(static_cast<char*>(c->tables.p) + keys_clean, 0xFF, kb - keys_clean, s));
+                keys_clean = kb;
+            }
+            if (keys_clean / sizeof(float) > 0xffffffffull) return fail(c, "disparity keys beyond 32-bit offsets");
+            sa.edge_off = (unsigned)(keys_clean / sizeof(float));
+            c->keys_clean = 0;
+        } else {
+            const size_t pairs = scan_version == 3 ? scan_keys_floats(sa, n_slots, sa.nwg_slot) : 0;
+            if (pairs > 0xffffffffull) return fail(c, "disparity pairs beyond 32-bit offsets");
+            HIPCK(c, c->tables.reserve(std::max<size_t>(1, scan_tables_floats(sa, scan_version, n_slots, sa.nwg_slot)) * sizeof(float)));
+            sa.edge_off = (unsigned)pairs;
+            if (n_slots) c->keys_clean = 0;
+        }
         sa.tables = c->tables.as<float>();
-        HIPCK(c, launch_bm_scan2(s, sa, gc.scan_lds, scan_version == 3));
+        HIPCK(c, launch_bm_scan2(s, sa, gc.scan_lds, scan_version == 3 ? ((sa.opt & kOptArgminPairs) ? kCombPairs : kCombKeys) : 0));
     } else
         HIPCK(c, launch_bm_scan(s, sa));
     std::memcpy(gc.scan_key, skey, sizeof(skey));
@@ -385,8 +407,12 @@
                                     full_scan ? gc.n_ref_cols : 0u, nHW, P->p, Hb - k - nHW, Wb - k - nHW));
     else
         HIPCK(c, launch_self_trivial(s, gc.refs.as<unsigned>(), R, c->self_idx.as<unsigned>(), c->self_cnt.as<unsigned>()));
-    if (n_slots && scan_version == 3)
-        HIPCK(c, launch_stereo_argmin3(s, c->tables.as<float>(), slots, n_slots, sa.nwg_slot, Wb, Hb, k, P->nDisp, thr,
+    if (merged) {
+        HIPCK(c, launch_stereo_argmin_keys(s, c->tables.as<float>(), sa.edge_off, slots, n_slots, Wb, Hb, k, P->nDisp, thr,
+                                           c->best.as<unsigned>(), c->shape.as<unsigned char>()));
+        c->keys_clean = keys_clean;
+    } else if (n_slots && scan_version == 3)
+        HIPCK(c, launch_stereo_argmin3(s, c->tables.as<float>(), sa.edge_off, slots, n_slots, sa.nwg_slot, Wb, Hb, k, P->nDisp, thr,
                                        c->best.as<unsigned>(), c->shape.as<unsigned char>()));
     else if (n_slots && scan_version == 2)
         HIPCK(c, launch_stereo_argmin2(s, c->tables.as<float>(), slots, n_slots, Wb, Hb, k, P->nDisp, thr,
diff --git a/lfbm5d_amd/csrc/lfbm5d_scan2.hip b/lfbm5d_amd/csrc/lfbm5d_scan2.hip
--- a/lfbm5d_amd/csrc/lfbm5d_scan2.hip
+++ b/lfbm5d_amd/csrc/lfbm5d_scan2.hip
@@ -47,7 +47,6 @@
 constexpr int kS2NL = 1;
 constexpr int kS2NI = 6;
 constexpr int kS2LD = 2;
-
 template <int K, bool STEREO, int NW, int NL>
 __device__ __forceinline__ void scan2_loader(const ScanArgs& a, const Scan2Wg& g, float* lds, int r0, const int lw) {
     static_assert(NL == 1, "one loader wave");
@@ -180,7 +179,7 @@
     lds_barrier();
 }
 
-template <int K, bool STEREO, int NW, bool COMB>
+template <int K, bool STEREO, int NW, int COMB>
 __device__ __forceinline__ void scan2_table(const ScanArgs& a, const Scan2Wg& g, float* lds, const int w, const int r0) {
     typedef S2Geom<K> G;
     constexpr int CW1 = G::CW1, RR1 = G::RR1, RRp1 = G::RRp1;
@@ -228,10 +227,11 @@
     const unsigned NCH = stereo_part_chunks(a.H, a.k, a.nDisp);
     const size_t pstride = COMB ? stereo_part_stride(a.W, a.H, a.k, a.nDisp) : 0;
     const size_t estride = COMB ? stereo_edge_stride(a.W, a.H, a.k, a.nDisp) : 0;
-    const unsigned n_slots = STEREO ? a.n_stereo / (unsigned)ncand : 0;
-    float* part = COMB ? a.tables + ((size_t)g.slot * a.nwg_slot + g.wgj) * pstride * 2 : nullptr;
-    float* edge = COMB ? a.tables + (size_t)n_slots * a.nwg_slot * pstride * 2 + (size_t)(g.slot * ncand + tb) * estride : nullptr;
-    const __amdgpu_buffer_rsrc_t rP = __builtin_amdgcn_make_buffer_rsrc((void*)part, 0, COMB ? (int)(pstride * 8) : 0, kRsrcFlags);
+    float* part = COMB == kCombPairs ? a.tables + ((size_t)g.slot * a.nwg_slot + g.wgj) * pstride * 2 : nullptr;
+    unsigned long long* const keys = COMB == kCombKeys ? reinterpret_cast<unsigned long long*>(a.tables) +
+                                                             ((size_t)g.slot * kStereoKeyArrays + (unsigned)g.wgj % kStereoKeyArrays) * pstride : nullptr;
+    float* edge = COMB ? a.tables + a.edge_off + (size_t)(g.slot * ncand + tb) * estride : nullptr;
+    const __amdgpu_buffer_rsrc_t rP = __builtin_amdgcn_make_buffer_rsrc((void*)part, 0, COMB == kCombPairs ? (int)(pstride * 8) : 0, kRsrcFlags);
     const __amdgpu_buffer_rsrc_t rEd = __builtin_amdgcn_make_buffer_rsrc((void*)edge, 0, (COMB && live) ? (int)(estride * 4) : 0, kRsrcFlags);
     const __amdgpu_buffer_rsrc_t rS = __builtin_amdgcn_make_buffer_rsrc((void*)a.scores, 0, (!STEREO && live) ? (int)a.scores_bytes : 0, kRsrcFlags);
     const int SRq = (int)stereo_table_srq(a.H, a.k, a.nDisp);
@@ -403,6 +403,8 @@
         const int rp = w * kShare + lane;
         const bool rok = lane < kShare && rp < 512;
         auto reduce_chunk = [&](const int cprev) {
+            static_assert(NW <= kShare && (NW - 1) * kShare + NW - 1 < 512, "the order lanes take part in the reduction");
+            if (COMB == kCombKeys && !rok) return;
             const float* src = xch + (cprev & 1) * NW * 512 + (rok ? rp : 0);
             float v[NW];
 #pragma unroll
@@ -415,9 +417,15 @@
 #pragma unroll
             for (int q = NW - 2; q >= 0; q--) bq = v[q] == best ? q : bq;
             const int bo = __builtin_amdgcn_ds_bpermute(bq << 2, ordv);
-            typedef int v2i __attribute__((ext_vector_type(2)));
-            const v2i pr = {__float_as_int(best), bo};
-            __builtin_amdgcn_raw_buffer_store_b64(pr, rP, rok ? (int)(((strip * NCH + cprev) * 512 + rp) * 8) : -1, 0, kPairStoreAux);
+            if (COMB == kCombKeys) {
+                const unsigned long long key = ((unsigned long long)f2ord(best + 0.0f) << 32) | (unsigned)bo;
+                unsigned long long* const kp = reinterpret_cast<unsigned long long*>(reinterpret_cast<char*>(keys) + (unsigned)(((strip * NCH + cprev) * 512 + rp) * 8));
+                (void)__hip_atomic_fetch_min(kp, key, __ATOMIC_RELAXED, __HIP_MEMORY_SCOPE_AGENT);
+            } else {
+                typedef int v2i __attribute__((ext_vector_type(2)));
+                const v2i pr = {__float_as_int(best), bo};
+                __builtin_amdgcn_raw_buffer_store_b64(pr, rP, rok ? (int)(((strip * NCH + cprev) * 512 + rp) * 8) : -1, 0, kPairStoreAux);
+            }
         };
 
 #ifdef LFBM5D_PHASE_TIMING
@@ -563,7 +571,7 @@
     lds_barrier();
 }
 
-template <int K, bool STEREO, int NW, int NL, bool COMB>
+template <int K, bool STEREO, int NW, int NL, int COMB>
 __device__ __forceinline__ void scan2_body(const ScanArgs& a, const Scan2Wg& g, float* lds) {
     typedef S2Geom<K> G;
     const int tid = threadIdx.x;
@@ -584,12 +592,12 @@
     else scan2_table<K, STEREO, NW, COMB>(a, g, lds, w, r0);
 }
 
-template <int K, bool COMB>
+template <int K, int COMB>
 __global__ __launch_bounds__((kS2NW + kS2NL) * 64) void k_bm_scan2(ScanArgs a) {
     extern __shared__ __attribute__((aligned(16))) float lds2[];
     const Scan2Wg& g = a.wgs[blockIdx.x];
     if (g.slot >= 0) scan2_body<K, true, kS2NW, kS2NL, COMB>(a, g, lds2);
-    else scan2_body<K, false, kS2NW, kS2NL, false>(a, g, lds2);
+    else scan2_body<K, false, kS2NW, kS2NL, 0>(a, g, lds2);
 }
 
 struct Argmin2Args { const float* tables; size_t tstride; unsigned st_of_slot[kBigA]; int W, H, k, nDisp, SRq; float thr; unsigned* best; unsigned char* shape; };
@@ -667,7 +675,11 @@
     const size_t ncand = (size_t)(2 * a.nDisp + 1) * (2 * a.nDisp + 1);
     if (version == 1) return (size_t)n_slots * ncand * stereo_table_stride(a.W, a.H, a.k, a.nDisp);
     if (version == 2) return (size_t)n_slots * ncand * stereo_table_stride2(a.W, a.H, a.k, a.nDisp);
-    return (size_t)n_slots * nwg_slot * stereo_part_stride(a.W, a.H, a.k, a.nDisp) * 2 + (size_t)n_slots * ncand * stereo_edge_stride(a.W, a.H, a.k, a.nDisp);
+    return scan_keys_floats(a, n_slots, nwg_slot) + (size_t)n_slots * ncand * stereo_edge_stride(a.W, a.H, a.k, a.nDisp);
+}
+
+size_t scan_keys_floats(const ScanArgs& a, unsigned n_slots, unsigned nwg_slot) {
+    return (size_t)n_slots * (nwg_slot ? nwg_slot : kStereoKeyArrays) * stereo_part_stride(a.W, a.H, a.k, a.nDisp) * 2;
 }
 
 bool scan2_plan(const ScanArgs& a, std::vector<Scan2Wg>& wgs, size_t* lds_bytes, unsigned* nwg_slot) {
@@ -718,6 +730,7 @@
     if (lds_bytes) *lds_bytes = lds;
     const int n1 = 2 * (64 + (int)a.k), n2 = 2 * ((64 + (int)a.k + ch_max + 3) & ~3);
     if (n1 + n2 > 64 * kS2NI || lds > 160 * 1024) return false;
+    if (a.n_stereo && stereo_part_stride(a.W, a.H, a.k, a.nDisp) * 8 > 0x7fffffffull) return false;
     return !wgs.empty();
 }
 
@@ -727,8 +740,9 @@
 }
 
 hipError_t prepare_scan2_kernels() {
-    const void* fns[] = {reinterpret_cast<const void*>(&k_bm_scan2<8, false>), reinterpret_cast<const void*>(&k_bm_scan2<16, false>),
-                         reinterpret_cast<const void*>(&k_bm_scan2<8, true>), reinterpret_cast<const void*>(&k_bm_scan2<16, true>)};
+    const void* fns[] = {reinterpret_cast<const void*>(&k_bm_scan2<8, 0>), reinterpret_cast<const void*>(&k_bm_scan2<16, 0>),
+                         reinterpret_cast<const void*>(&k_bm_scan2<8, kCombKeys>), reinterpret_cast<const void*>(&k_bm_scan2<16, kCombKeys>),
+                         reinterpret_cast<const void*>(&k_bm_scan2<8, kCombPairs>), reinterpret_cast<const void*>(&k_bm_scan2<16, kCombPairs>)};
     for (const void* f : fns) {
         const hipError_t e = hipFuncSetAttribute(f, hipFuncAttributeMaxDynamicSharedMemorySize, 160 * 1024);
         if (e != hipSuccess) return e;
@@ -736,19 +750,26 @@
     return hipSuccess;
 }
 
-hipError_t launch_bm_scan2(hipStream_t s, const ScanArgs& a, size_t lds, bool combined) {
+hipError_t launch_bm_scan2(hipStream_t s, const ScanArgs& a, size_t lds, int form) {
     if (!a.n_wgs) return hipSuccess;
     const dim3 blk((kS2NW + kS2NL) * 64);
-    if (a.k == 8 && combined) hipLaunchKernelGGL((k_bm_scan2<8, true>), dim3(a.n_wgs), blk, lds, s, a);
-    else if (a.k == 8) hipLaunchKernelGGL((k_bm_scan2<8, false>), dim3(a.n_wgs), blk, lds, s, a);
-    else if (a.k == 16 && combined) hipLaunchKernelGGL((k_bm_scan2<16, true>), dim3(a.n_wgs), blk, lds, s, a);
-    else if (a.k == 16) hipLaunchKernelGGL((k_bm_scan2<16, false>), dim3(a.n_wgs), blk, lds, s, a);
-    else return hipErrorInvalidValue;
+    if (a.k != 8 && a.k != 16) return hipErrorInvalidValue;
+    if (form == kCombKeys) {
+        if (a.k == 8) hipLaunchKernelGGL((k_bm_scan2<8, kCombKeys>), dim3(a.n_wgs), blk, lds, s, a);
+        else hipLaunchKernelGGL((k_bm_scan2<16, kCombKeys>), dim3(a.n_wgs), blk, lds, s, a);
+    } else if (form == kCombPairs) {
+        if (a.k == 8) hipLaunchKernelGGL((k_bm_scan2<8, kCombPairs>), dim3(a.n_wgs), blk, lds, s, a);
+        else hipLaunchKernelGGL((k_bm_scan2<16, kCombPairs>), dim3(a.n_wgs), blk, lds, s, a);
+    } else if (form == 0) {
+        if (a.k == 8) hipLaunchKernelGGL((k_bm_scan2<8, 0>), dim3(a.n_wgs), blk, lds, s, a);
+        else hipLaunchKernelGGL((k_bm_scan2<16, 0>), dim3(a.n_wgs), blk, lds, s, a);
+    } else return hipErrorInvalidValue;
     return hipGetLastError();
 }
 
-struct Argmin3Args { const float* tables; unsigned st_of_slot[kBigA]; int W, H, k, nDisp, n_slots, nwg_slot; float thr; unsigned* best; unsigned char* shape; };
-__global__ __launch_bounds__(256) void k_stereo_argmin3(Argmin3Args a) {
+struct Argmin3Args { float* tables; size_t edge_off; unsigned st_of_slot[kBigA]; int W, H, k, nDisp, n_slots, nwg_slot; float thr; unsigned* best; unsigned char* shape; };
+template <bool KEYS>
+__device__ __forceinline__ void stereo_argmin3_body(const Argmin3Args& a) {
     const int W = a.W, H = a.H, nDisp = a.nDisp;
     const int span_c = W - 2 * nDisp - a.k + 1, span_r = H - 2 * nDisp - a.k + 1;
     const int nstrips = (span_c - 1 + 63) / 64;
@@ -770,20 +791,36 @@
         const int p = 2 * (i & 255), c = (i >> 8) % NCH, strip = (i >> 8) / NCH;
         const int l = p >> 3, t = 8 * c + (p & 7);
         const int row = 1 + t - l, col = 1 + 64 * strip + l;
-        if (row + 1 < 0 || row >= span_r || col >= span_c) return;
-        const v4f* src = reinterpret_cast<const v4f*>(a.tables) + ((size_t)slot * a.nwg_slot * pstride >> 1) + i;
         float bv0 = __builtin_inff(), bv1 = __builtin_inff(); int bo0 = 0x7fffffff, bo1 = 0x7fffffff;
-        for (int j0 = 0; j0 < a.nwg_slot; j0 += 16) {
-            v4f w8[16];
-#pragma unroll
-            for (int u = 0; u < 16; u++) {
-                w8[u] = __builtin_nontemporal_load(src + (size_t)min(j0 + u, a.nwg_slot - 1) * (pstride >> 1));
-            }
-#pragma unroll
-            for (int u = 0; u < 16; u++) {
-                const int o0 = __float_as_int(w8[u][1]), o1 = __float_as_int(w8[u][3]);
-                if (w8[u][0] < bv0 || (w8[u][0] == bv0 && o0 < bo0)) { bv0 = w8[u][0]; bo0 = o0; }
-                if (w8[u][2] < bv1 || (w8[u][2] == bv1 && o1 < bo1)) { bv1 = w8[u][2]; bo1 = o1; }
+        if (KEYS) {
+            typedef unsigned long long v2k __attribute__((ext_vector_type(2)));
+            v2k* kp = reinterpret_cast<v2k*>(a.tables) + ((size_t)slot * kStereoKeyArrays * pstride >> 1) + i;
+            v2k kk = __builtin_nontemporal_load(kp);
+            *kp = v2k{~0ull, ~0ull};
+#pragma unroll
+            for (unsigned j = 1; j < kStereoKeyArrays; j++) {
+                const v2k o = __builtin_nontemporal_load(kp + j * (pstride >> 1));
+                kp[j * (pstride >> 1)] = v2k{~0ull, ~0ull};
+                kk[0] = o[0] < kk[0] ? o[0] : kk[0]; kk[1] = o[1] < kk[1] ? o[1] : kk[1];
+            }
+            if (row + 1 < 0 || row >= span_r || col >= span_c) return;
+            bv0 = ord2f((unsigned)(kk[0] >> 32)); bo0 = (int)(unsigned)kk[0];
+            bv1 = ord2f((unsigned)(kk[1] >> 32)); bo1 = (int)(unsigned)kk[1];
+        } else {
+            if (row + 1 < 0 || row >= span_r || col >= span_c) return;
+            const v4f* src = reinterpret_cast<const v4f*>(a.tables) + ((size_t)slot * a.nwg_slot * pstride >> 1) + i;
+            for (int j0 = 0; j0 < a.nwg_slot; j0 += 16) {
+                v4f w8[16];
+#pragma unroll
+                for (int u = 0; u < 16; u++) {
+                    w8[u] = __builtin_nontemporal_load(src + (size_t)min(j0 + u, a.nwg_slot - 1) * (pstride >> 1));
+                }
+#pragma unroll
+                for (int u = 0; u < 16; u++) {
+                    const int o0 = __float_as_int(w8[u][1]), o1 = __float_as_int(w8[u][3]);
+                    if (w8[u][0] < bv0 || (w8[u][0] == bv0 && o0 < bo0)) { bv0 = w8[u][0]; bo0 = o0; }
+                    if (w8[u][2] < bv1 || (w8[u][2] == bv1 && o1 < bo1)) { bv1 = w8[u][2]; bo1 = o1; }
+                }
             }
         }
         if (row >= 0 && !(row == 0 && l == 0)) put(row, col, bv0, bo0);
@@ -793,7 +830,7 @@
         int row, col;
         if (e < span_r) { row = e; col = 0; } else { row = 0; col = 1 + 64 * (e - span_r); }
         const bool ok = e < n_edge && col < span_c;
-        const float* ed = a.tables + (size_t)a.n_slots * a.nwg_slot * pstride * 2 + (size_t)slot * ncand * estride + (ok ? e : 0);
+        const float* ed = a.tables + a.edge_off + (size_t)slot * ncand * estride + (ok ? e : 0);
         float bv = __builtin_inff(); int bo = 0x7fffffff;
         for (int d0 = sub; d0 < ncand; d0 += 16 * 8) {
             float v[8];
@@ -814,18 +851,33 @@
         if (ok && sub == 0) put(row, col, bv, bo);
     }
 }
-
-hipError_t launch_stereo_argmin3(hipStream_t s, const float* tables, const unsigned* st_of_slot, unsigned n_slots, unsigned nwg_slot,
-                                 unsigned W, unsigned H, unsigned k, unsigned nDisp, float thr,
-                                 unsigned* best, unsigned char* shape) {
+__global__ __launch_bounds__(256) void k_stereo_argmin3(Argmin3Args a) { stereo_argmin3_body<false>(a); }
+__global__ __launch_bounds__(256) void k_stereo_argmin_keys(Argmin3Args a) { stereo_argmin3_body<true>(a); }
+
+static hipError_t launch_stereo_argmin3_form(hipStream_t s, bool keys, float* tables, size_t edge_off, const unsigned* st_of_slot, unsigned n_slots,
+                                             unsigned nwg_slot, unsigned W, unsigned H, unsigned k, unsigned nDisp, float thr,
+                                             unsigned* best, unsigned char* shape) {
     Argmin3Args a;
-    a.tables = tables; a.W = (int)W; a.H = (int)H; a.k = (int)k; a.nDisp = (int)nDisp; a.n_slots = (int)n_slots; a.nwg_slot = (int)nwg_slot; a.thr = thr; a.best = best; a.shape = shape;
+    a.tables = tables; a.edge_off = edge_off; a.W = (int)W; a.H = (int)H; a.k = (int)k; a.nDisp = (int)nDisp; a.n_slots = (int)n_slots; a.nwg_slot = (int)nwg_slot; a.thr = thr; a.best = best; a.shape = shape;
     for (unsigned i = 0; i < n_slots && i < (unsigned)kBigA; i++) a.st_of_slot[i] = st_of_slot[i];
     const unsigned span_c = W - 2 * nDisp - k + 1, span_r = H - 2 * nDisp - k + 1;
     const unsigned nstrips = (span_c - 1 + 63) / 64;
     const unsigned n = nstrips * stereo_part_chunks(H, k, nDisp) * 256 + 16 * (span_r + nstrips);
-    hipLaunchKernelGGL(k_stereo_argmin3, dim3((n + 255) / 256, n_slots), dim3(256), 0, s, a);
+    if (keys) hipLaunchKernelGGL(k_stereo_argmin_keys, dim3((n + 255) / 256, n_slots), dim3(256), 0, s, a);
+    else hipLaunchKernelGGL(k_stereo_argmin3, dim3((n + 255) / 256, n_slots), dim3(256), 0, s, a);
     return hipGetLastError();
+}
+
+hipError_t launch_stereo_argmin3(hipStream_t s, const float* tables, size_t edge_off, const unsigned* st_of_slot, unsigned n_slots, unsigned nwg_slot,
+                                 unsigned W, unsigned H, unsigned k, unsigned nDisp, float thr,
+                                 unsigned* best, unsigned char* shape) {
+    return launch_stereo_argmin3_form(s, false, const_cast<float*>(tables), edge_off, st_of_slot, n_slots, nwg_slot, W, H, k, nDisp, thr, best, shape);
+}
+
+hipError_t launch_stereo_argmin_keys(hipStream_t s, float* tables, size_t edge_off, const unsigned* st_of_slot, unsigned n_slots,
+                                     unsigned W, unsigned H, unsigned k, unsigned nDisp, float thr,
+                                     unsigned* best, unsigned char* shape) {
+    return launch_stereo_argmin3_form(s, true, tables, edge_off, st_of_slot, n_slots, 0, W, H, k, nDisp, thr, best, shape);
 }
 
 hipError_t launch_stereo_argmin2(hipStream_t s, const float* tables, const unsigned* st_of_slot, unsigned n_slots,
```

Result: no change. 258.0 SAI-megapixels/s, median of 6 (+0.7%).
